# AnthonyMadia/lodestar

Hardware: AMD Instinct MI355X
Metric: verified signature sets/sec (node) at 8192-set batches (higher is better)
Workload: dtype u32 (28-bit-limb Montgomery Fp, v_mad_u64_u32)

## Files before the change

### lodestar_amd/csrc/bgv_api.cpp

```cpp
#include <hip/hip_runtime.h>
#include <stdio.h>
#include <stdlib.h>
#include <string.h>
#include <sys/mman.h>
#include <sys/random.h>

#include <algorithm>
#include <atomic>
#include <chrono>
#include <condition_variable>
#include <unordered_map>
#include <deque>
#include <map>
#include <memory>
#include <mutex>
#include <shared_mutex>
#include <unordered_set>
#include <thread>
#include <vector>

#include "../../include/blsgpu.h"
#include "bgv_launch.h"
#include "bgv_retry_plan.h"
#include "bls_field.h"
#include "bgv_shuffle.h"

#define BGV_MAX_BATCH_SLOTS 131072
#define BGV_DISPATCHERS 2

static size_t max_batch_slots() {
  static const size_t v = env_size("BGV_MAX_BATCH_SLOTS", BGV_MAX_BATCH_SLOTS, BGV_WAVE);
  return v;
}
#define BGV_COALESCE_US 500
static size_t coalesce_us() {
  static const size_t v = env_size("BGV_COALESCE_US", BGV_COALESCE_US, 0);
  return v;
}
#define BGV_IDLE_COALESCE_US 50
static size_t idle_coalesce_us() {
  static const size_t v = env_size("BGV_IDLE_COALESCE_US", BGV_IDLE_COALESCE_US, 0);
  return v;
}
#define BGV_SPLIT_MIN_SETS 4096
static size_t split_min_env() {
  static const size_t v = env_size("BGV_SPLIT_MIN", BGV_SPLIT_MIN_SETS, 0);
  return v == 1 ? 2 : v;
}
static int dispatchers_per_device() {
  static const int v = (int)env_size("BGV_DISPATCHERS", BGV_DISPATCHERS, 1);
  return v;
}
static int execs_per_device() {
  static const int v = (int)env_size("BGV_EXECS", 2 * BGV_DISPATCHERS, 1);
  return std::max(v, dispatchers_per_device());
}

static size_t retry_hold_max() {
  static const size_t v = env_size("BGV_RETRY_HOLD", 1, 1);
  return v;
}
static int retry_threads_per_device() {
  static const int v = (int)env_size("BGV_RETRY_THREADS", 1, 1);
  return v;
}

extern "C" int bgv_device_count(void) {
  int n = 0;
  if (hipGetDeviceCount(&n) != hipSuccess) return 0;
  return n;
}

namespace {

template <class T>
struct Pinned {
  T* p = nullptr;
  size_t cap = 0;
  hipError_t reserve(size_t n) {
    if (n <= cap) return hipSuccess;
    release();
    n = std::max(n, 2 * cap);
    hipError_t e = hipHostMalloc(reinterpret_cast<void**>(&p), std::max<size_t>(n, 1) * sizeof(T), 0);
    if (e != hipSuccess) {
      p = nullptr;
      return e;
    }
    cap = n;
    return hipSuccess;
  }
  void release() {
    if (p) (void)hipHostFree(p);
    p = nullptr;
    cap = 0;
  }
};

struct Exec {
  hipStream_t main = nullptr;
  hipStream_t close = nullptr;
  hipEvent_t ev0 = nullptr, ev1 = nullptr, ev_prep = nullptr, ev_sets = nullptr;
  hipEvent_t kev[2 * BGV_NKERNELS] = {};
  void* slot_mem = nullptr;
  uint32_t slot_cap = 0;
  void* group_mem = nullptr;
  uint32_t group_cap = 0;
  bgv_dslot* d_slots = nullptr;
  bgv_dgroup* d_groups = nullptr;
  uint32_t* d_idx = nullptr;
  size_t idx_cap = 0;
  uint8_t* d_pkb = nullptr;
  size_t pkb_cap = 0;
  Pinned<bgv_dslot> h_slots;
  Pinned<bgv_dgroup> h_groups;
  Pinned<uint32_t> h_idx;
  Pinned<uint8_t> h_pkb;
  Pinned<int32_t> h_ss, h_ps, h_verdict;
  fp12_t* d_gu1 = nullptr;
  size_t gu1_cap = 0;
  void* d_pscratch = nullptr;
  size_t pscratch_cap = 0;
  uint8_t* d_pout = nullptr;
  size_t pout_cap = 0;
  uint32_t* d_lines = nullptr;
  uint32_t lines_cap = 0;
};

struct FinalScratch {
  uint8_t* din = nullptr;
  void* vals = nullptr;
  void* one = nullptr;
  bgv_dgroup* dg = nullptr;
  int32_t* dst = nullptr;
  int32_t* dv = nullptr;
  size_t cap = 0;
};

static const uint32_t kComHandles = 2 * BGV_MAX_COMMITTEES;
static const size_t kComPoolInit = size_t(1) << 20;
struct ComPool {
  std::mutex mu;
  std::vector<uint32_t> free_handles;
  std::map<uint32_t, uint32_t> free_ranges;
  size_t cap = 0;
  bool alloc(uint32_t n, uint32_t* handle, uint32_t* off) {
    if (free_handles.empty()) return false;
    for (auto it = free_ranges.begin(); it != free_ranges.end(); ++it)
      if (it->second >= n) {
        *off = it->first;
        const uint32_t rest = it->second - n;
        free_ranges.erase(it);
        if (rest) free_ranges.emplace(*off + n, rest);
        *handle = free_handles.back();
        free_handles.pop_back();
        return true;
      }
    return false;
  }
  bool alloc_bulk(uint32_t n, uint32_t nh, std::vector<uint32_t>* handles, uint32_t* off) {
    if (free_handles.size() < nh) return false;
    for (auto it = free_ranges.begin(); it != free_ranges.end(); ++it)
      if (it->second >= n) {
        *off = it->first;
        const uint32_t rest = it->second - n;
        free_ranges.erase(it);
        if (rest) free_ranges.emplace(*off + n, rest);
        handles->assign(free_handles.end() - nh, free_handles.end());
        free_handles.resize(free_handles.size() - nh);
        return true;
      }
    return false;
  }
  void add_range(uint32_t off, uint32_t n) {
    auto nx = free_ranges.lower_bound(off);
    if (nx != free_ranges.begin()) {
      auto pv = std::prev(nx);
      if (pv->first + pv->second == off) {
        off = pv->first;
        n += pv->second;
        free_ranges.erase(pv);
      }
    }
    if (nx != free_ranges.end() && off + n == nx->first) {
      n += nx->second;
      free_ranges.erase(nx);
    }
    free_ranges.emplace(off, n);
  }
};
struct CommitteeRec {
  uint32_t handle = 0, off = 0;
  std::vector<uint32_t> idx;
  bool bad = false;
  std::shared_ptr<ComPool> pool;
  ~CommitteeRec() {
    if (!pool) return;
    std::lock_guard<std::mutex> lk(pool->mu);
    pool->free_handles.push_back(handle);
    pool->add_range(off, (uint32_t)idx.size());
  }
};

struct Call;
struct BatchState {
  std::chrono::steady_clock::time_point tb;
  double t_merge = 0, t_tok = 0, t_sets = 0, t_pass1 = 0, t_post = 0;
  uint32_t nslots = 0, ngroups = 0;
  std::vector<uint32_t> call_gb;
  bool want_gu = false;
  bool uniform = false;
  bool prof = false;
};
struct RetryJob {
  std::vector<Call*> calls;
  Exec* x = nullptr;
  std::shared_ptr<BatchState> st;
};
struct DevSched {
  std::mutex mu;
  std::condition_variable cv;
  std::deque<Exec*> free;
  std::deque<RetryJob> rq;
  bool stop = false;
  std::vector<std::thread> retry_threads;
  std::vector<hipStream_t> retries;
  std::vector<hipStream_t> dstreams;
};

struct Device {
  int id = 0;
  std::unique_ptr<DevSched> sched = std::make_unique<DevSched>();
  FinalScratch final_scratch;
  hipStream_t stream = nullptr;
  bgv_cache_entry* cache = nullptr;
  size_t cache_cap = 0;
  bgv_dcommittee* com_dir = nullptr;
  uint32_t* com_pool = nullptr;
  uint32_t* com_list = nullptr;
  uint32_t* shuf_buf = nullptr;
  size_t shuf_cap = 0;
  std::vector<Exec*> execs;
  std::unique_ptr<std::mutex> compute_mu = std::make_unique<std::mutex>();
};

struct Call : CallPlan {
  const bgv_set* sets = nullptr;
  const bgv_pkbits* pkbits = nullptr;
  std::vector<SetCommittee> setcom;
  std::vector<std::shared_ptr<CommitteeRec>> com_refs;
  int32_t* out = nullptr;
  bgv_stats* stats_out = nullptr;
  bgv_done_fn done = nullptr;
  void* user = nullptr;
  bool owned = false;
  std::chrono::steady_clock::time_point t0;
  int dev = -1;
  bgv_job pjob{};
  int32_t pcode = 0;
  int rc = BGV_OK;
  std::mutex mu;
  std::condition_variable cv;
  bool finished = false;
};

}

struct bgv_ctx {
  std::vector<Device> devs;
  std::atomic<size_t> n_pubkeys{0};
  std::mutex put_mu;
  std::unordered_set<uint32_t> bad_pk;
  std::atomic<bool> closed{false};
  std::mutex rng_mu;
  uint64_t rng_seed = 0, rng_state = 0;
  std::shared_mutex cache_mu;
  std::mutex util_mu;
  std::shared_mutex com_mu;
  std::unordered_map<uint32_t, std::shared_ptr<CommitteeRec>> committees;
  std::vector<std::weak_ptr<CommitteeRec>> retired;
  std::shared_ptr<ComPool> com_pool = std::make_shared<ComPool>();
  std::mutex prof_mu;
  bool profile = false;
  bool fault_inject = false;
  std::atomic<uint32_t> max_slots{BGV_MAX_BATCH_SLOTS};
  std::atomic<uint32_t> coalesce{BGV_COALESCE_US};
  std::atomic<uint32_t> idle_coalesce{BGV_IDLE_COALESCE_US};
  std::atomic<int> running{0};
  std::atomic<uint32_t> split_min{BGV_SPLIT_MIN_SETS};
  int split_inflight = 0;
  bool split_closing = false;
  std::mutex split_mu;
  std::condition_variable split_cv;
  double kernel_ms[BGV_NKERNELS] = {};
  uint64_t kernel_launches = 0;
  std::vector<std::thread> dispatchers;
  std::mutex qmu;
  std::condition_variable qcv;
  std::deque<Call*> queue;
  bool stop = false;
};

#define HIPCHK(x)                               \
  do {                                          \
    hipError_t e_ = (x);                        \
    if (e_ != hipSuccess) return -BGV_E_DEVICE; \
  } while (0)

static uint64_t splitmix64(uint64_t* s) {
  uint64_t z = (*s += 0x9E3779B97F4A7C15ull);
  z = (z ^ (z >> 30)) * 0xBF58476D1CE4E5B9ull;
  z = (z ^ (z >> 27)) * 0x94D049BB133111EBull;
  return z ^ (z >> 31);
}

static void fill_scalars(bgv_ctx* c, uint64_t* out, size_t n) {
  {
    std::lock_guard<std::mutex> lk(c->rng_mu);
    if (c->rng_seed) {
      for (size_t i = 0; i < n; ++i) {
        uint64_t v;
        do v = splitmix64(&c->rng_state);
        while (v == 0);
        out[i] = v;
      }
      return;
    }
  }
  par_ranges(n, [out](size_t lo, size_t hi) {
    size_t got = 0;
    uint8_t* p = reinterpret_cast<uint8_t*>(out + lo);
    while (got < (hi - lo) * 8) {
      const ssize_t r = getrandom(p + got, (hi - lo) * 8 - got, 0);
      if (r > 0) got += (size_t)r;
    }
    for (size_t i = lo; i < hi; ++i)
      if (out[i] == 0) out[i] = 1;
  });
}

template <class T>
static int grow(T** p, size_t* cap, size_t want) {
  if (want <= *cap) return BGV_OK;
  size_t n = std::max(want, *cap * 2);
  if (*p) (void)hipFree(*p);
  *p = nullptr;
  HIPCHK(hipMalloc(reinterpret_cast<void**>(p), n * sizeof(T)));
  *cap = n;
  return BGV_OK;
}

static int exec_reserve_slots(Exec& x, uint32_t slots) {
  if (slots <= x.slot_cap) return BGV_OK;
  uint32_t n = std::max<uint32_t>(slots, x.slot_cap * 2);
  if (x.slot_mem) (void)hipFree(x.slot_mem);
  if (x.d_slots) (void)hipFree(x.d_slots);
  x.slot_mem = nullptr;
  x.d_slots = nullptr;
  HIPCHK(hipMalloc(&x.slot_mem, bgv_slot_mem_bytes(n)));
  HIPCHK(hipMalloc(reinterpret_cast<void**>(&x.d_slots), sizeof(bgv_dslot) * n));
  x.slot_cap = n;
  return BGV_OK;
}

static int exec_reserve_groups(Exec& x, uint32_t groups) {
  if (groups <= x.group_cap) return BGV_OK;
  uint32_t n = std::max<uint32_t>(groups, x.group_cap * 2);
  if (x.group_mem) (void)hipFree(x.group_mem);
  if (x.d_groups) (void)hipFree(x.d_groups);
  x.group_mem = nullptr;
  x.d_groups = nullptr;
  HIPCHK(hipMalloc(&x.group_mem, bgv_group_bytes() * n));
  HIPCHK(hipMalloc(reinterpret_cast<void**>(&x.d_groups), sizeof(bgv_dgroup) * n));
  x.group_cap = n;
  return BGV_OK;
}

static uint32_t lines_keep_pairs(size_t slots) {
  return (uint32_t)((slots + slots / BGV_WAVE + 16383u) & ~(size_t)16383u);
}
static void exec_trim_lines(Exec& x, size_t max_slots) {
  if (x.lines_cap <= lines_keep_pairs(max_slots)) return;
  (void)hipFree(x.d_lines);
  x.d_lines = nullptr;
  x.lines_cap = 0;
}
static int exec_reserve_lines(Exec& x, bgv_dev_batch& b) {
  const uint32_t need = bgv_lines_pairs(b);
  if (need > x.lines_cap) {
    const uint32_t cap = (need + 16383u) & ~16383u;
    if (x.d_lines) (void)hipFree(x.d_lines);
    x.d_lines = nullptr;
    x.lines_cap = 0;
    HIPCHK(hipMalloc(reinterpret_cast<void**>(&x.d_lines), bgv_line_record_bytes() * cap));
    x.lines_cap = cap;
  }
  b.lines = x.d_lines;
  b.lines_cap = x.lines_cap;
  return BGV_OK;
}

static int exec_create(Exec* x) {
  HIPCHK(hipEventCreate(&x->ev0));
  HIPCHK(hipEventCreate(&x->ev1));
  HIPCHK(hipEventCreateWithFlags(&x->ev_sets, hipEventDisableTiming));
  HIPCHK(hipEventCreateWithFlags(&x->ev_prep, hipEventDisableTiming));
  for (auto& e : x->kev) HIPCHK(hipEventCreate(&e));
  return BGV_OK;
}

static void exec_destroy(Exec* x) {
  if (x->main) (void)hipStreamSynchronize(x->main);
  void* ptrs[] = {x->slot_mem, x->group_mem, x->d_slots,    x->d_groups, x->d_idx,
                  x->d_pkb,      x->d_pscratch, x->d_pout, x->d_lines};
  for (void* p : ptrs)
    if (p) (void)hipFree(p);
  x->h_slots.release();
  x->h_groups.release();
  x->h_idx.release();
  x->h_pkb.release();
  x->h_ss.release();
  x->h_ps.release();
  x->h_verdict.release();
  if (x->d_gu1) (void)hipFree(x->d_gu1);
  if (x->ev0) (void)hipEventDestroy(x->ev0);
  if (x->ev1) (void)hipEventDestroy(x->ev1);
  if (x->ev_sets) (void)hipEventDestroy(x->ev_sets);
  if (x->ev_prep) (void)hipEventDestroy(x->ev_prep);
  for (auto& e : x->kev)
    if (e) (void)hipEventDestroy(e);
  if (x->close) (void)hipStreamSynchronize(x->close);
  delete x;
}

static void prof_add(bgv_ctx* c, Exec& x, bool sets, bool groups) {
  std::lock_guard<std::mutex> lk(c->prof_mu);
  if (!c->profile) return;
  for (int k = 0; k < BGV_NKERNELS; ++k) {
    const bool is_set_kernel = k < BGV_NSETKERNELS;
    if ((is_set_kernel && !sets) || (!is_set_kernel && !groups)) continue;
    float km = 0;
    if (hipEventElapsedTime(&km, x.kev[2 * k], x.kev[2 * k + 1]) == hipSuccess) c->kernel_ms[k] += km;
  }
  if (sets) c->kernel_launches++;
}

static bgv_dev_batch make_batch(Device& d, Exec& x, uint32_t nslots, uint32_t ngroups) {
  bgv_dev_batch b;
  memset(&b, 0, sizeof(b));
  b.nslots = nslots;
  b.ngroups = ngroups;
  b.slots = x.d_slots;
  b.groups = x.d_groups;
  b.pk_idx = x.d_idx;
  b.cache_opaque = d.cache;
  b.pk_bytes = x.d_pkb;
  b.com_dir = d.com_dir;
  b.com_pool = d.com_pool;
  bgv_carve(&b, x.slot_mem, x.slot_cap, x.group_mem, x.group_cap);
  return b;
}

static void call_finish(Call* call) {
  for (size_t j = 0; j < call->njobs; ++j) call->out[j] = call->code[j] == 2 ? -BGV_E_DEVICE : call->code[j];
  call->st.wall_ms =
      std::chrono::duration<double, std::milli>(std::chrono::steady_clock::now() - call->t0).count();
  if (call->stats_out) *call->stats_out = call->st;
  if (call->done) call->done(call->user, call->rc);
  if (call->owned) {
    delete call;
    return;
  }
  {
    std::lock_guard<std::mutex> lk(call->mu);
    call->finished = true;
  }
  call->cv.notify_all();
}

static void call_fail(Call* call, int rc) {
  call->rc = rc;
  for (auto& x : call->code)
    if (x == 2) x = -BGV_E_DEVICE;
  call_finish(call);
}

static int host_job_code(bgv_ctx* c, const bgv_job& jb, const bgv_set* sets, int32_t* code,
                         const bgv_pkbits* pkbits = nullptr, Call* call = nullptr) {
  *code = 2;
  if (jb.n_sets == 0) {
    *code = -BGV_E_EMPTY_SET;
    return BGV_OK;
  }
  for (uint32_t k = 0; k < jb.n_sets && *code == 2; ++k) {
    const bgv_set& s = sets[jb.first_set + k];
    if (pkbits && pkbits[jb.first_set + k].committee != BGV_NO_COMMITTEE) {
      const bgv_pkbits& pb = pkbits[jb.first_set + k];
      if (!s.msg || (!s.sig && s.sig_len) || (!pb.bits && pb.n_bits)) return -BGV_E_ARG;
      const auto it = c->committees.find(pb.committee);
      const CommitteeRec* rec = it != c->committees.end() ? it->second.get() : nullptr;
      CommitteeInfo ci{};
      if (rec) ci = CommitteeInfo{rec->handle, (uint32_t)rec->idx.size(), rec->bad};
      SetCommittee sc;
      *code = committee_set_check(rec ? &ci : nullptr, pb, &sc);
      if (*code == 2 && call) {
        call->setcom[jb.first_set + k] = sc;
        if (call->com_refs.empty() || call->com_refs.back().get() != rec) call->com_refs.push_back(it->second);
      }
      continue;
    }
    if (s.n_pk == 0)
      *code = -BGV_E_EMPTY_AGGREGATE;
    else if (!s.msg || (!s.sig && s.sig_len) || (!s.pk_indices && !s.pk_bytes))
      return -BGV_E_ARG;
    else if (s.pk_indices)
      for (uint32_t q = 0; q < s.n_pk; ++q)
        if (s.pk_indices[q] >= c->n_pubkeys || (!c->bad_pk.empty() && c->bad_pk.count(s.pk_indices[q]))) {
          *code = -BGV_E_BAD_INDEX;
          break;
        }
  }
  return BGV_OK;
}

static void advise_huge(void* p, size_t bytes) {
  const uintptr_t a = ((uintptr_t)p + (2u << 20) - 1) & ~(uintptr_t)((2u << 20) - 1);
  const uintptr_t e = ((uintptr_t)p + bytes) & ~(uintptr_t)((2u << 20) - 1);
  if (e > a) (void)madvise(reinterpret_cast<void*>(a), e - a, MADV_HUGEPAGE);
}

static int call_submit(bgv_ctx* c, Call* call, const bgv_job* jobs, size_t njobs, const bgv_set* sets, size_t nsets,
                       int mode, int32_t* out, bgv_stats* stats, bgv_done_fn done, void* user, int dev = -1,
                       const bgv_pkbits* pkbits = nullptr) {
  call->t0 = std::chrono::steady_clock::now();
  call->dev = dev;
  if (c->closed) return -BGV_E_CLOSED;
  if ((njobs && (!jobs || !out)) || (nsets && !sets)) return -BGV_E_ARG;
  if (mode != BGV_MODE_WORKER && mode != BGV_MODE_PER_JOB) return -BGV_E_ARG;
  call->jobs = jobs;
  call->njobs = njobs;
  call->sets = sets;
  call->nsets = nsets;
  call->mode = mode;
  call->out = out;
  call->stats_out = stats;
  call->done = done;
  call->user = user;
  call->code.assign(njobs, 2);
  call->pkbits = pkbits;
  if (pkbits) call->setcom.assign(nsets, SetCommittee{});
  {
    std::shared_lock<std::shared_mutex> clk(c->cache_mu);
    std::shared_lock<std::shared_mutex> mlk(c->com_mu, std::defer_lock);
    if (pkbits) mlk.lock();
    for (size_t j = 0; j < njobs; ++j) {
      if ((size_t)jobs[j].first_set + jobs[j].n_sets > nsets) return -BGV_E_ARG;
      if (host_job_code(c, jobs[j], sets, &call->code[j], pkbits, call) != BGV_OK) return -BGV_E_ARG;
    }
  }
  const auto is_com = [pkbits](size_t i) { return pkbits && pkbits[i].committee != BGV_NO_COMMITTEE; };
  Layout& L = call->L;
  {
    size_t npk = 0;
    for (size_t i = 0; i < nsets; ++i)
      if (is_com(i))
        npk += 1 + pkb_nwords(call->setcom[i].n);
      else if (sets[i].pk_indices)
        npk += sets[i].n_pk;
    const size_t cap = nsets + nsets / 8 + BGV_WAVE;
    L.slots.reserve(cap);
    L.slot_set.reserve(cap);
    L.idx.reserve(npk);
    if (nsets >= (1u << 17)) {
      advise_huge(L.slots.data(), sizeof(bgv_dslot) * cap);
      advise_huge(L.slot_set.data(), 4 * cap);
      advise_huge(L.idx.data(), 4 * npk);
    }
  }
  layout_call(L, call->todo, jobs, njobs, sets, mode, call->code, pkbits ? call->setcom.data() : nullptr);
  call->set_sig.assign(nsets, 0);
  call->set_pk.assign(nsets, 0);
  if (L.slots.empty()) {
    call_finish(call);
    return BGV_OK;
  }
  {
    std::lock_guard<std::mutex> lk(c->qmu);
    if (c->stop) return -BGV_E_CLOSED;
    c->queue.push_back(call);
  }
  if (dev < 0)
    c->qcv.notify_one();
  else
    c->qcv.notify_all();
  return BGV_OK;
}

static double ms_since(std::chrono::steady_clock::time_point t) {
  return std::chrono::duration<double, std::milli>(std::chrono::steady_clock::now() - t).count();
}

static bool needs_retry(const std::vector<Call*>& calls) {
  for (const Call* call : calls)
    if (!call->units.empty()) return true;
  return false;
}

static int run_pass1(bgv_ctx* c, Device& d, Exec& x, std::vector<Call*>& calls, BatchState& bs) {
  const auto tb = std::chrono::steady_clock::now();
  bs.tb = tb;
  double t_merge = 0, t_tok = 0, t_sets = 0, t_pass1 = 0, t_post = 0;
  uint32_t nslots = 0, ngroups = 0;
  size_t nidx = 0, npkb = 0, nuniq = 0, ncom_team = 0, ncom_wave = 0;
  bool any_uniform = false;
  for (Call* call : calls) {
    call->slot_base = nslots;
    nslots += (uint32_t)call->L.slots.size();
    ngroups += (uint32_t)call->L.groups.size();
    nidx += call->L.idx.size();
    npkb += call->L.pkb.size();
    nuniq += call->L.uniq.size();
    ncom_team += call->L.com_team.size();
    ncom_wave += call->L.com_wave.size();
    for (char u : call->L.group_uniform) any_uniform = any_uniform || u;
  }
  const size_t ncom = ncom_team + ncom_wave, nlist = nuniq + ncom;
  const bool bulk = nslots + ngroups > bgv_fold_pairs_max();
  const bool uniform = uniform_enabled() && any_uniform && bulk && !bgv_single_pass_miller();
  HIPCHK(hipSetDevice(d.id));
  int rc;
  if ((rc = exec_reserve_slots(x, nslots)) || (rc = exec_reserve_groups(x, ngroups)) ||
      (rc = grow(&x.d_idx, &x.idx_cap, std::max<size_t>(nidx + nlist, 1))) ||
      (rc = grow(&x.d_pkb, &x.pkb_cap, std::max<size_t>(npkb, 1))))
    return rc;
  HIPCHK(x.h_slots.reserve(nslots));
  HIPCHK(x.h_groups.reserve(std::max<size_t>(ngroups, 1)));
  HIPCHK(x.h_idx.reserve(nidx + nlist));
  HIPCHK(x.h_pkb.reserve(npkb));
  HIPCHK(x.h_ss.reserve(nslots));
  HIPCHK(x.h_ps.reserve(nslots));
  HIPCHK(x.h_verdict.reserve(std::max<size_t>(ngroups, 1)));
  bgv_dslot* slots = x.h_slots.p;
  bgv_dgroup* groups = x.h_groups.p;
  uint32_t max_npk = 0;
  {
    size_t ns = 0, ng = 0, ni = 0, npb = 0;
    for (Call* call : calls) {
      const uint32_t ib = (uint32_t)ni, pb = (uint32_t)(npb / 96), gb = (uint32_t)ng;
      if (ns == 0 && ib == 0 && pb == 0 && gb == 0) {
        const bgv_dslot* src = call->L.slots.data();
        std::atomic<uint32_t> mx{0};
        par_ranges(call->L.slots.size(), [&](size_t lo, size_t hi) {
          memcpy(slots + lo, src + lo, sizeof(bgv_dslot) * (hi - lo));
          uint32_t m = 0;
          for (size_t i = lo; i < hi; ++i)
            if (!(src[i].flags & BGV_SLOT_PK_COMMITTEE)) m = std::max(m, src[i].n_pk);
          uint32_t cur = mx.load();
          while (m > cur && !mx.compare_exchange_weak(cur, m)) {
          }
        });
        max_npk = std::max(max_npk, mx.load());
        ns = call->L.slots.size();
      } else {
        for (const bgv_dslot& s0 : call->L.slots) {
          const bgv_dslot s = rebase_slot(s0, call->slot_base, ib, pb, gb);
          if (!(s.flags & BGV_SLOT_PK_COMMITTEE)) max_npk = std::max(max_npk, s.n_pk);
          slots[ns++] = s;
        }
      }
      for (size_t gi = 0; gi < call->L.groups.size(); ++gi) {
        const bgv_dgroup& g = call->L.groups[gi];
        groups[ng++] = bgv_dgroup{g.first_slot + call->slot_base, g.n_slots, g.mask, 0,
                                  uniform && call->L.group_uniform[gi] ? BGV_GROUP_UNIFORM : 0u};
      }
      if (!call->L.idx.empty()) memcpy(x.h_idx.p + ni, call->L.idx.data(), 4 * call->L.idx.size());
      ni += call->L.idx.size();
      if (!call->L.pkb.empty()) memcpy(x.h_pkb.p + npb, call->L.pkb.data(), call->L.pkb.size());
      npb += call->L.pkb.size();
    }
    uint32_t* u = x.h_idx.p + nidx;
    for (Call* call : calls)
      for (uint32_t v : call->L.uniq) *u++ = v + call->slot_base;
    for (Call* call : calls)
      for (uint32_t v : call->L.com_team) *u++ = v + call->slot_base;
    for (Call* call : calls)
      for (uint32_t v : call->L.com_wave) *u++ = v + call->slot_base;
  }
  std::vector<uint64_t> sc(nslots);
  fill_scalars(c, sc.data(), nslots);
  par_ranges(nslots, [&](size_t lo, size_t hi) {
    for (size_t i = lo; i < hi; ++i) slots[i].scalar = sc[i];
  });

  bool prof;
  {
    std::lock_guard<std::mutex> lk(c->prof_mu);
    prof = c->profile;
  }
  t_merge = ms_since(tb);
  if (c->fault_inject) HIPCHK(hipErrorLaunchFailure);
  HIPCHK(hipMemcpyAsync(x.d_slots, slots, sizeof(bgv_dslot) * nslots, hipMemcpyHostToDevice, x.main));
  HIPCHK(hipMemcpyAsync(x.d_groups, groups, sizeof(bgv_dgroup) * ngroups, hipMemcpyHostToDevice, x.main));
  if (nidx + nlist) HIPCHK(hipMemcpyAsync(x.d_idx, x.h_idx.p, 4 * (nidx + nlist), hipMemcpyHostToDevice, x.main));
  if (npkb) HIPCHK(hipMemcpyAsync(x.d_pkb, x.h_pkb.p, npkb, hipMemcpyHostToDevice, x.main));
  bgv_dev_batch b = make_batch(d, x, nslots, ngroups);
  b.max_npk = max_npk;
  b.uniform = uniform;
  bs.uniform = uniform;
  b.uniq = x.d_idx + nidx;
  b.nuniq = (uint32_t)nuniq;
  b.com = x.d_idx + nidx + nuniq;
  b.ncom_team = (uint32_t)ncom_team;
  b.ncom_wave = (uint32_t)ncom_wave;
  if (int lrc = exec_reserve_lines(x, b)) return lrc;
  bgv_streams S{x.main, prof ? x.kev : nullptr};
  int32_t *ss = x.h_ss.p, *ps = x.h_ps.p, *verdict = x.h_verdict.p;
  {
    const auto tt = std::chrono::steady_clock::now();
    std::unique_lock<std::mutex> tok(*d.compute_mu);
    t_tok = ms_since(tt);
    HIPCHK(hipEventRecord(x.ev0, x.main));
    HIPCHK(bgv_launch_prep(b, S));
    HIPCHK(hipEventRecord(x.ev_prep, x.main));
    HIPCHK(bgv_launch_miller(b, S));
    HIPCHK(hipEventRecord(x.ev_sets, x.main));
    HIPCHK(hipEventSynchronize(x.ev_prep));
    t_sets = ms_since(tt) - t_tok;
  }
  const auto tg = std::chrono::steady_clock::now();
  HIPCHK(bgv_launch_groups(b, S, false));
  HIPCHK(hipEventRecord(x.ev1, x.main));
  HIPCHK(hipMemcpyAsync(ss, b.sig_status, 4ull * nslots, hipMemcpyDeviceToHost, x.main));
  HIPCHK(hipMemcpyAsync(ps, b.pk_status, 4ull * nslots, hipMemcpyDeviceToHost, x.main));
  HIPCHK(hipMemcpyAsync(verdict, b.verdict, 4ull * ngroups, hipMemcpyDeviceToHost, x.main));
  HIPCHK(hipStreamSynchronize(x.main));
  float ms = 0;
  HIPCHK(hipEventElapsedTime(&ms, x.ev0, x.ev1));
  exec_trim_lines(x, c->max_slots.load());
  if (prof) prof_add(c, x, true, true);
  t_pass1 = ms_since(tg);
  const auto tp = std::chrono::steady_clock::now();
  std::vector<uint32_t>& call_gb = bs.call_gb;
  bool& want_gu = bs.want_gu;
  {
    uint32_t gb = 0;
    for (Call* call : calls) {
      call->st.device_ms += ms;
      call->after_pass1(ss + call->slot_base, ps + call->slot_base, verdict + gb);
      call_gb.push_back(gb);
      gb += (uint32_t)call->L.groups.size();
      want_gu = want_gu || call->any_pattern_eligible();
    }
  }
  if (want_gu) {
    if ((rc = grow(&x.d_gu1, &x.gu1_cap, ngroups))) return rc;
    HIPCHK(hipMemcpyAsync(x.d_gu1, b.gu, sizeof(fp12_t) * ngroups, hipMemcpyDeviceToDevice, x.main));
  }
  {
    uint32_t gb = 0, np = 0, maxg = 0;
    for (Call* call : calls) {
      if (call->partial_out) {
        ++np;
        maxg = std::max<uint32_t>(maxg, (uint32_t)call->L.groups.size());
      }
    }
    if (np) {
      if ((rc = grow(reinterpret_cast<uint8_t**>(&x.d_pscratch), &x.pscratch_cap,
                     bgv_fp12_bytes() * (maxg / 32 + 4))) ||
          (rc = grow(&x.d_pout, &x.pout_cap, 576)))
        return rc;
      for (Call* call : calls) {
        const uint32_t ng = (uint32_t)call->L.groups.size();
        if (call->partial_out) {
          HIPCHK(bgv_launch_partial(b, gb, ng, x.d_pscratch, x.d_pout, x.main));
          HIPCHK(hipMemcpyAsync(call->partial_out, x.d_pout, 576, hipMemcpyDeviceToHost, x.main));
          HIPCHK(hipStreamSynchronize(x.main));
        }
        gb += ng;
      }
    }
  }
  HIPCHK(hipStreamSynchronize(x.main));
  t_post = ms_since(tp);
  bs.t_merge = t_merge;
  bs.t_tok = t_tok;
  bs.t_sets = t_sets;
  bs.t_pass1 = t_pass1;
  bs.t_post = t_post;
  bs.nslots = nslots;
  bs.ngroups = ngroups;
  bs.prof = prof;
  if (trace_on() && !needs_retry(calls))
    fprintf(stderr,
            "[bgv] dev %d calls %zu slots %u groups %u | submit..dispatch %.1f | merge %.1f tokwait %.1f sets %.1f "
            "groups %.1f post %.1f total %.1f ms\n",
            d.id, calls.size(), nslots, ngroups,
            std::chrono::duration<double, std::milli>(tb - calls.front()->t0).count(), t_merge, t_tok, t_sets,
            t_pass1, t_post, ms_since(tb));
  return BGV_OK;
}

struct RetryRun {
  RetryJob job;
  int rounds = 0;
  uint32_t nrg = 0;
  double t_build = 0;
  std::chrono::steady_clock::time_point tr;
};

static int retry_launch(Device& d, RetryRun& r, bool* more) {
  Exec& x = *r.job.x;
  std::vector<Call*>& calls = r.job.calls;
  BatchState& bs = *r.job.st;
  const auto th = std::chrono::steady_clock::now();
  std::vector<bgv_dgroup> rg;
  for (size_t k = 0; k < calls.size(); ++k)
    calls[k]->build_parts(rg, bs.want_gu ? (int64_t)bs.call_gb[k] : -1, bs.uniform);
  *more = !rg.empty();
  r.nrg = 0;
  if (rg.empty()) return BGV_OK;
  ++r.rounds;
  const uint32_t nrg = (uint32_t)rg.size();
  std::vector<uint32_t> upk;
  if (bs.uniform)
    for (uint32_t t = 0; t < nrg; ++t)
      if (rg[t].flags & BGV_GROUP_UNIFORM) upk.push_back(t);
  const uint32_t per = (uint32_t)(sizeof(bgv_dgroup) / sizeof(uint32_t));
  const uint32_t nlist = ((uint32_t)upk.size() + per - 1) / per;
  int rc;
  if ((rc = exec_reserve_groups(x, nrg + nlist))) return rc;
  HIPCHK(x.h_groups.reserve(nrg + nlist));
  HIPCHK(x.h_verdict.reserve(nrg));
  memcpy(x.h_groups.p, rg.data(), sizeof(bgv_dgroup) * nrg);
  if (!upk.empty()) memcpy(x.h_groups.p + nrg, upk.data(), 4 * upk.size());
  HIPCHK(hipMemcpyAsync(x.d_groups, x.h_groups.p, sizeof(bgv_dgroup) * (nrg + nlist), hipMemcpyHostToDevice,
                        x.close));
  bgv_dev_batch b = make_batch(d, x, bs.nslots, nrg);
  b.uniform = !upk.empty();
  b.upk = reinterpret_cast<const uint32_t*>(b.groups + nrg);
  b.npk = (uint32_t)upk.size();
  for (const bgv_dgroup& t : rg) b.weighted = b.weighted || (t.flags & BGV_GROUP_WEIGHTED);
  bool pattern = false;
  for (Call* call : calls) pattern = pattern || !call->punits.empty();
  if (pattern) b.gu1 = x.d_gu1;
  r.t_build = ms_since(th);
  bgv_streams SC{x.close, bs.prof ? x.kev : nullptr};
  HIPCHK(hipEventRecord(x.ev0, x.close));
  HIPCHK(bgv_launch_groups(b, SC, true));
  HIPCHK(hipEventRecord(x.ev1, x.close));
  HIPCHK(hipMemcpyAsync(x.h_verdict.p, b.verdict, 4ull * nrg, hipMemcpyDeviceToHost, x.close));
  r.nrg = nrg;
  return BGV_OK;
}

static int retry_complete(bgv_ctx* c, RetryRun& r, double t_wait) {
  Exec& x = *r.job.x;
  float ms = 0;
  HIPCHK(hipEventElapsedTime(&ms, x.ev0, x.ev1));
  if (r.job.st->prof) prof_add(c, x, false, true);
  if (trace_on()) {
    size_t npt = 0;
    for (Call* call : r.job.calls)
      for (const PatternUnit& pu : call->punits) npt += pu.tests.size();
    fprintf(stderr,
            "[bgv]  round %d: %u groups (%zu tests with a reference), host %.2f, launch..verdicts %.2f, device %.2f ms, "
            "since round start %.1f ms\n",
            r.rounds, r.nrg, npt, r.t_build, t_wait, ms, ms_since(r.tr));
  }
  for (Call* call : r.job.calls) {
    call->st.device_ms += ms;
    call->after_round(x.h_verdict.p);
  }
  r.nrg = 0;
  return BGV_OK;
}

static void retry_trace_done(const Device& d, const RetryRun& r) {
  if (!trace_on()) return;
  const BatchState& bs = *r.job.st;
  fprintf(stderr,
          "[bgv] dev %d calls %zu slots %u groups %u | merge %.1f tokwait %.1f sets %.1f groups %.1f post %.1f "
          "retry(%d) %.1f total %.1f ms\n",
          d.id, r.job.calls.size(), bs.nslots, bs.ngroups, bs.t_merge, bs.t_tok, bs.t_sets, bs.t_pass1, bs.t_post,
          r.rounds, ms_since(r.tr), ms_since(bs.tb));
}

static Exec* exec_acquire(Device& d) {
  DevSched& s = *d.sched;
  std::unique_lock<std::mutex> lk(s.mu);
  s.cv.wait(lk, [&s] { return !s.free.empty(); });
  Exec* x = s.free.back();
  s.free.pop_back();
  return x;
}

static void exec_release(Device& d, Exec* x) {
  DevSched& s = *d.sched;
  {
    std::lock_guard<std::mutex> lk(s.mu);
    s.free.push_back(x);
  }
  s.cv.notify_all();
}

static void finish_calls(std::vector<Call*>& calls, int rc) {
  for (Call* call : calls) {
    if (rc != BGV_OK)
      call_fail(call, rc);
    else
      call_finish(call);
  }
}

static void retry_loop(bgv_ctx* c, Device* d, int k) {
  DevSched& s = *d->sched;
  (void)hipSetDevice(d->id);
  hipStream_t st = s.retries[k];
  std::vector<RetryRun> held;
  auto leave = [&](size_t i, int rc) {
    finish_calls(held[i].job.calls, rc);
    exec_release(*d, held[i].job.x);
    c->running.fetch_sub(1);
    held.erase(held.begin() + (std::ptrdiff_t)i);
  };
  for (;;) {
    {
      std::unique_lock<std::mutex> lk(s.mu);
      if (held.empty()) s.cv.wait(lk, [&s] { return s.stop || !s.rq.empty(); });
      if (held.empty() && s.rq.empty()) return;
      while (!s.rq.empty() && held.size() < retry_hold_max()) {
        RetryRun r;
        r.job = std::move(s.rq.front());
        s.rq.pop_front();
        r.job.x->close = st;
        r.tr = std::chrono::steady_clock::now();
        c->running.fetch_add(1);
        held.push_back(std::move(r));
      }
    }
    (void)hipSetDevice(d->id);
    for (size_t i = 0; i < held.size();) {
      bool more = false;
      const int rc = retry_launch(*d, held[i], &more);
      if (rc != BGV_OK) {
        (void)hipStreamSynchronize(st);
        leave(i, rc);
      } else if (!more) {
        retry_trace_done(*d, held[i]);
        leave(i, BGV_OK);
      } else {
        ++i;
      }
    }
    if (held.empty()) continue;
    const auto tl = std::chrono::steady_clock::now();
    const hipError_t e = hipStreamSynchronize(st);
    const double t_wait = ms_since(tl);
    for (size_t i = 0; i < held.size();) {
      const int rc = e == hipSuccess ? retry_complete(c, held[i], t_wait) : -BGV_E_DEVICE;
      if (rc != BGV_OK)
        leave(i, rc);
      else
        ++i;
    }
  }
}

static void dispatcher_loop(bgv_ctx* c, Device* d, hipStream_t stream) {
  (void)hipSetDevice(d->id);
  const int di = (int)(d - c->devs.data());
  auto mine = [di](const Call* q) { return q->dev < 0 || q->dev == di; };
  auto any_mine = [c, &mine] {
    for (Call* q : c->queue)
      if (mine(q)) return true;
    return false;
  };
  for (;;) {
    std::vector<Call*> calls;
    {
      std::unique_lock<std::mutex> lk(c->qmu);
      c->qcv.wait(lk, [c, &any_mine] { return c->stop || any_mine(); });
      if (!any_mine()) return;
      auto queued_slots = [c, &mine] {
        size_t n = 0;
        for (Call* q : c->queue)
          if (mine(q)) n += q->L.slots.size();
        return n;
      };
      const size_t cap = c->max_slots.load();
      const size_t win = c->running.load() > 0 ? c->coalesce.load()
                                               : std::min<size_t>(c->coalesce.load(), c->idle_coalesce.load());
      const auto until = std::chrono::steady_clock::now() + std::chrono::microseconds(win);
      while (!c->stop && queued_slots() < cap &&
             c->qcv.wait_until(lk, until) != std::cv_status::timeout) {
      }
      if (!any_mine()) continue;
      size_t slots = 0;
      for (auto it = c->queue.begin(); it != c->queue.end();) {
        Call* call = *it;
        if (!mine(call)) {
          ++it;
          continue;
        }
        const size_t n = call->L.slots.size();
        if (!calls.empty() && slots + n > cap) break;
        calls.push_back(call);
        slots += n;
        it = c->queue.erase(it);
      }
      if (!c->queue.empty()) c->qcv.notify_all();
    }
    Exec* x = exec_acquire(*d);
    x->main = stream;
    auto bs = std::make_shared<BatchState>();
    int rc;
    {
      std::shared_lock<std::shared_mutex> clk(c->cache_mu);
      c->running.fetch_add(1);
      rc = run_pass1(c, *d, *x, calls, *bs);
      c->running.fetch_sub(1);
    }
    if (rc == BGV_OK && needs_retry(calls)) {
      DevSched& s = *d->sched;
      {
        std::lock_guard<std::mutex> lk(s.mu);
        s.rq.push_back(RetryJob{std::move(calls), x, bs});
      }
      s.cv.notify_all();
      continue;
    }
    finish_calls(calls, rc);
    exec_release(*d, x);
  }
}

extern "C" {

static void ctx_free_devices(bgv_ctx* c) {
  for (Device& d : c->devs) {
    if (!d.stream) continue;
    (void)hipSetDevice(d.id);
    for (Exec* x : d.execs) exec_destroy(x);
    d.execs.clear();
    d.sched->free.clear();
    for (hipStream_t st : d.sched->dstreams) (void)hipStreamDestroy(st);
    d.sched->dstreams.clear();
    for (hipStream_t st : d.sched->retries) (void)hipStreamDestroy(st);
    d.sched->retries.clear();
    if (d.stream) (void)hipStreamSynchronize(d.stream);
    if (d.cache) (void)hipFree(d.cache);
    d.cache = nullptr;
    {
      void* cbufs[] = {d.com_dir, d.com_pool, d.com_list, d.shuf_buf};
      for (void* q : cbufs)
        if (q) (void)hipFree(q);
      d.shuf_buf = nullptr;
      d.shuf_cap = 0;
      d.com_dir = nullptr;
      d.com_pool = nullptr;
      d.com_list = nullptr;
    }
    {
      FinalScratch& fs = d.final_scratch;
      void* bufs[] = {fs.din, fs.vals, fs.one, fs.dg, fs.dst, fs.dv};
      for (void* q : bufs)
        if (q) (void)hipFree(q);
      fs = FinalScratch{};
    }
    if (d.stream) (void)hipStreamDestroy(d.stream);
    d.stream = nullptr;
  }
}

int bgv_init(const int* devices, int ndev, bgv_ctx** out) {
  if (!out) return -BGV_E_ARG;
  *out = nullptr;
  int avail = bgv_device_count();
  if (avail <= 0) return -BGV_E_DEVICE;
  bgv_ctx* c = new bgv_ctx();
  {
    const char* fi = getenv("BGV_FAULT_INJECT");
    c->fault_inject = fi && atoi(fi) > 0;
  }
  c->max_slots = (uint32_t)max_batch_slots();
  c->coalesce = (uint32_t)coalesce_us();
  c->idle_coalesce = (uint32_t)idle_coalesce_us();
  c->split_min = (uint32_t)split_min_env();
  const int n = (devices && ndev > 0) ? ndev : 1;
  c->devs.resize(n);
  for (int i = 0; i < n; ++i) {
    Device& d = c->devs[i];
    d.id = (devices && ndev > 0) ? devices[i] : 0;
    bool ok = d.id >= 0 && d.id < avail && hipSetDevice(d.id) == hipSuccess &&
              hipStreamCreateWithFlags(&d.stream, hipStreamNonBlocking) == hipSuccess;
    int least = 0, greatest = 0;
    ok = ok && hipDeviceGetStreamPriorityRange(&least, &greatest) == hipSuccess;
    for (int k = 0; ok && k < retry_threads_per_device(); ++k) {
      hipStream_t st = nullptr;
      ok = hipStreamCreateWithPriority(&st, hipStreamNonBlocking, greatest) == hipSuccess;
      if (ok) d.sched->retries.push_back(st);
    }
    for (int k = 0; ok && k < dispatchers_per_device(); ++k) {
      hipStream_t st = nullptr;
      ok = hipStreamCreateWithFlags(&st, hipStreamNonBlocking) == hipSuccess;
      if (ok) d.sched->dstreams.push_back(st);
    }
    ok = ok && hipMalloc(reinterpret_cast<void**>(&d.com_dir), sizeof(bgv_dcommittee) * kComHandles) == hipSuccess &&
         hipMalloc(reinterpret_cast<void**>(&d.com_pool), 4 * kComPoolInit) == hipSuccess &&
         hipMalloc(reinterpret_cast<void**>(&d.com_list), 4 * (size_t)kComHandles) == hipSuccess;
    for (int k = 0; ok && k < execs_per_device(); ++k) {
      Exec* x = new Exec();
      d.execs.push_back(x);
      ok = exec_create(x) == BGV_OK;
      if (ok) d.sched->free.push_back(x);
    }
    if (!ok) {
      ctx_free_devices(c);
      delete c;
      (void)hipGetLastError();
      return d.id < 0 || d.id >= avail ? -BGV_E_ARG : -BGV_E_DEVICE;
    }
  }
  c->com_pool->cap = kComPoolInit;
  c->com_pool->free_ranges.emplace(0u, (uint32_t)kComPoolInit);
  for (uint32_t h = kComHandles; h-- > 0;) c->com_pool->free_handles.push_back(h);
  for (Device& d : c->devs) {
    for (hipStream_t st : d.sched->dstreams) c->dispatchers.emplace_back(dispatcher_loop, c, &d, st);
    for (int k = 0; k < (int)d.sched->retries.size(); ++k) d.sched->retry_threads.emplace_back(retry_loop, c, &d, k);
  }
  *out = c;
  return BGV_OK;
}

int bgv_close(bgv_ctx* c) {
  if (!c) return -BGV_E_ARG;
  {
    std::unique_lock<std::mutex> lk(c->split_mu);
    c->split_closing = true;
    c->split_cv.wait(lk, [c] { return c->split_inflight == 0; });
  }
  {
    std::lock_guard<std::mutex> lk(c->qmu);
    c->stop = true;
  }
  c->qcv.notify_all();
  for (auto& w : c->dispatchers)
    if (w.joinable()) w.join();
  c->dispatchers.clear();
  for (Device& d : c->devs) {
    {
      std::lock_guard<std::mutex> lk(d.sched->mu);
      d.sched->stop = true;
    }
    d.sched->cv.notify_all();
    for (auto& t : d.sched->retry_threads)
      if (t.joinable()) t.join();
    d.sched->retry_threads.clear();
  }
  std::unique_lock<std::shared_mutex> lk(c->cache_mu);
  if (c->closed.exchange(true)) return BGV_OK;
  ctx_free_devices(c);
  return BGV_OK;
}

int bgv_destroy(bgv_ctx* c) {
  if (!c) return -BGV_E_ARG;
  bgv_close(c);
  delete c;
  return BGV_OK;
}

int bgv_set_batching(bgv_ctx* c, uint32_t max_batch_slots, uint32_t coalesce_us, uint32_t idle_coalesce_us) {
  if (!c) return -BGV_E_ARG;
  if (max_batch_slots) c->max_slots = std::max<uint32_t>(max_batch_slots, BGV_WAVE);
  if (coalesce_us != UINT32_MAX) c->coalesce = coalesce_us;
  if (idle_coalesce_us != UINT32_MAX) c->idle_coalesce = idle_coalesce_us;
  return BGV_OK;
}

int bgv_set_rng_seed(bgv_ctx* c, uint64_t seed) {
  if (!c) return -BGV_E_ARG;
  std::lock_guard<std::mutex> lk(c->rng_mu);
  c->rng_seed = seed;
  c->rng_state = seed;
  return BGV_OK;
}

size_t bgv_pubkeys_count(const bgv_ctx* c) { return c ? c->n_pubkeys.load() : 0; }

static int cache_reserve(bgv_ctx* c, size_t need) {
  const size_t esz = bgv_cache_entry_bytes();
  for (Device& d : c->devs) {
    HIPCHK(hipSetDevice(d.id));
    if (need <= d.cache_cap) continue;
    size_t cap = std::max(need, d.cache_cap * 2);
    void* p = nullptr;
    HIPCHK(hipMalloc(&p, esz * cap));
    if (d.cache) {
      HIPCHK(hipMemcpyAsync(p, d.cache, esz * c->n_pubkeys, hipMemcpyDeviceToDevice, d.stream));
      HIPCHK(hipStreamSynchronize(d.stream));
      HIPCHK(hipFree(d.cache));
    }
    d.cache = static_cast<bgv_cache_entry*>(p);
    d.cache_cap = cap;
  }
  return BGV_OK;
}

static int committee_totals(bgv_ctx* c, const std::vector<uint32_t>& handles) {
  if (handles.empty()) return BGV_OK;
  for (Device& d : c->devs) {
    HIPCHK(hipSetDevice(d.id));
    HIPCHK(hipMemcpyAsync(d.com_list, handles.data(), 4 * handles.size(), hipMemcpyHostToDevice, d.stream));
    HIPCHK(bgv_launch_committee_totals(d.com_dir, d.com_list, (uint32_t)handles.size(), d.com_pool, d.cache, d.stream));
    HIPCHK(hipStreamSynchronize(d.stream));
  }
  return BGV_OK;
}

static int committees_refresh(bgv_ctx* c, uint32_t first, size_t n) {
  std::vector<uint32_t> handles;
  {
    std::unique_lock<std::shared_mutex> lk(c->com_mu);
    std::vector<std::shared_ptr<CommitteeRec>> recs;
    for (auto& kv : c->committees) recs.push_back(kv.second);
    for (auto& w : c->retired)
      if (auto sp = w.lock()) recs.push_back(std::move(sp));
    for (auto& sp : recs) {
      CommitteeRec& r = *sp;
      bool touched = false, bad = false;
      for (uint32_t i : r.idx) {
        touched = touched || (i >= first && (size_t)i < (size_t)first + n);
        bad = bad || (!c->bad_pk.empty() && c->bad_pk.count(i));
      }
      if (!touched) continue;
      r.bad = bad;
      handles.push_back(r.handle);
    }
  }
  return committee_totals(c, handles);
}

static int com_pool_grow(bgv_ctx* c, size_t need) {
  ComPool& P = *c->com_pool;
  const size_t old = P.cap, cap = std::max(2 * old, old + need);
  if (cap > (size_t)UINT32_MAX) return -BGV_E_NOMEM;
  for (Device& d : c->devs) {
    HIPCHK(hipSetDevice(d.id));
    uint32_t* p = nullptr;
    HIPCHK(hipMalloc(reinterpret_cast<void**>(&p), 4 * cap));
    HIPCHK(hipMemcpyAsync(p, d.com_pool, 4 * old, hipMemcpyDeviceToDevice, d.stream));
    HIPCHK(hipStreamSynchronize(d.stream));
    HIPCHK(hipFree(d.com_pool));
    d.com_pool = p;
  }
  std::lock_guard<std::mutex> lk(P.mu);
  P.add_range((uint32_t)old, (uint32_t)(cap - old));
  P.cap = cap;
  return BGV_OK;
}

int bgv_committee_put(bgv_ctx* c, uint32_t id, const uint32_t* indices, size_t n) {
  if (!c || id >= BGV_MAX_COMMITTEES || !indices || n < 1 || n > 65536) return -BGV_E_ARG;
  std::lock_guard<std::mutex> plk(c->put_mu);
  auto rec = std::make_shared<CommitteeRec>();
  auto checks = [&]() -> int {
    if (c->closed) return -BGV_E_CLOSED;
    {
      std::shared_lock<std::shared_mutex> lk(c->com_mu);
      if (c->committees.count(id)) return -BGV_E_ARG;
    }
    for (size_t i = 0; i < n; ++i)
      if (indices[i] >= c->n_pubkeys || (!c->bad_pk.empty() && c->bad_pk.count(indices[i]))) return -BGV_E_BAD_INDEX;
    return BGV_OK;
  };
  auto take = [&]() -> bool {
    std::lock_guard<std::mutex> lk(c->com_pool->mu);
    if (!c->com_pool->alloc((uint32_t)n, &rec->handle, &rec->off)) return false;
    rec->pool = c->com_pool;
    return true;
  };
  auto upload = [&]() -> int {
    rec->idx.assign(indices, indices + n);
    const bgv_dcommittee head{rec->off, (uint32_t)n, {}};
    std::lock_guard<std::mutex> ulk(c->util_mu);
    for (Device& d : c->devs) {
      HIPCHK(hipSetDevice(d.id));
      HIPCHK(hipMemcpyAsync(d.com_pool + rec->off, indices, 4 * n, hipMemcpyHostToDevice, d.stream));
      HIPCHK(hipMemcpyAsync(d.com_dir + rec->handle, &head, sizeof(head), hipMemcpyHostToDevice, d.stream));
      HIPCHK(hipStreamSynchronize(d.stream));
    }
    const int rc = committee_totals(c, {rec->handle});
    if (rc) return rc;
    std::unique_lock<std::shared_mutex> lk(c->com_mu);
    c->committees.emplace(id, rec);
    return BGV_OK;
  };
  {
    std::shared_lock<std::shared_mutex> clk(c->cache_mu);
    if (int rc = checks()) return rc;
    if (take()) return upload();
    std::lock_guard<std::mutex> lk(c->com_pool->mu);
    if (c->com_pool->free_handles.empty()) return -BGV_E_NOMEM;
  }
  std::unique_lock<std::shared_mutex> clk(c->cache_mu);
  if (int rc = checks()) return rc;
  {
    std::lock_guard<std::mutex> ulk(c->util_mu);
    if (int rc = com_pool_grow(c, n)) return rc;
  }
  if (!take()) return -BGV_E_NOMEM;
  return upload();
}

int bgv_committee_drop(bgv_ctx* c, uint32_t id) {
  if (!c) return -BGV_E_ARG;
  std::lock_guard<std::mutex> plk(c->put_mu);
  if (c->closed) return -BGV_E_CLOSED;
  std::shared_ptr<CommitteeRec> rec;
  std::unique_lock<std::shared_mutex> lk(c->com_mu);
  auto it = c->committees.find(id);
  if (it == c->committees.end()) return -BGV_E_BAD_INDEX;
  rec = std::move(it->second);
  c->committees.erase(it);
  c->retired.erase(std::remove_if(c->retired.begin(), c->retired.end(),
                                  [](const std::weak_ptr<CommitteeRec>& w) { return w.expired(); }),
                   c->retired.end());
  c->retired.push_back(rec);
  return BGV_OK;
}

int bgv_shuffling_put(bgv_ctx* c, uint32_t first_id, const uint8_t seed[32], const uint32_t* active, size_t n_active,
                      uint32_t slots, uint32_t committees_per_slot, uint32_t rounds, uint32_t* out_shuffling) {
  if (!c || !seed || !active || n_active < 1 || n_active > BGV_SHUFFLE_MAX_N || !slots || !committees_per_slot ||
      rounds > BGV_SHUFFLE_MAX_ROUNDS)
    return -BGV_E_ARG;
  const uint64_t count64 = (uint64_t)slots * committees_per_slot;
  if (first_id > BGV_MAX_COMMITTEES || count64 > BGV_MAX_COMMITTEES - first_id) return -BGV_E_ARG;
  const uint32_t n = (uint32_t)n_active, count = (uint32_t)count64, m = shuf_nonempty(n, count);
  if (shuf_longest(n, count) > 65536) return -BGV_E_ARG;
  std::lock_guard<std::mutex> plk(c->put_mu);
  std::vector<std::shared_ptr<CommitteeRec>> recs;
  std::vector<uint32_t> ks, handles;
  uint32_t base = 0;
  auto checks = [&]() -> int {
    if (c->closed) return -BGV_E_CLOSED;
    {
      std::shared_lock<std::shared_mutex> lk(c->com_mu);
      for (uint32_t k = 0; k < count; ++k)
        if (c->committees.count(first_id + k)) return -BGV_E_ARG;
    }
    const size_t npk = c->n_pubkeys;
    const bool marks = !c->bad_pk.empty();
    for (size_t i = 0; i < n; ++i)
      if (active[i] >= npk || (marks && c->bad_pk.count(active[i]))) return -BGV_E_BAD_INDEX;
    return BGV_OK;
  };
  auto take = [&]() -> bool {
    std::lock_guard<std::mutex> lk(c->com_pool->mu);
    if (!c->com_pool->alloc_bulk(n, m, &handles, &base)) return false;
    for (uint32_t j = 0; j < m; ++j) {
      uint32_t lo, hi;
      ks.push_back(shuf_nonempty_k(n, count, j, &lo, &hi));
      auto rec = std::make_shared<CommitteeRec>();
      rec->handle = handles[j];
      rec->off = base + lo;
      rec->idx.resize(hi - lo);
      rec->pool = c->com_pool;
      recs.push_back(std::move(rec));
    }
    return true;
  };
  auto run = [&]() -> int {
    std::vector<uint32_t> shuf(n);
    {
      std::lock_guard<std::mutex> ulk(c->util_mu);
      const size_t words = bgv_shuffle_scratch_words(n, rounds);
      bool first = true;
      for (Device& d : c->devs) {
        HIPCHK(hipSetDevice(d.id));
        if (d.shuf_cap < words) {
          uint32_t* p = nullptr;
          HIPCHK(hipMalloc(reinterpret_cast<void**>(&p), 4 * words));
          if (d.shuf_buf) (void)hipFree(d.shuf_buf);
          d.shuf_buf = p;
          d.shuf_cap = words;
        }
        HIPCHK(hipMemcpyAsync(d.shuf_buf, active, 4 * (size_t)n, hipMemcpyHostToDevice, d.stream));
        HIPCHK(hipMemcpyAsync(d.com_list, handles.data(), 4 * (size_t)m, hipMemcpyHostToDevice, d.stream));
        HIPCHK(bgv_launch_shuffle(seed, n, rounds, d.shuf_buf, d.com_pool + base, d.stream));
        HIPCHK(bgv_launch_shuffle_dir(d.com_dir, d.com_list, m, base, n, count, d.stream));
        HIPCHK(bgv_launch_committee_totals(d.com_dir, d.com_list, m, d.com_pool, d.cache, d.stream));
        if (first)
          HIPCHK(hipMemcpyAsync(shuf.data(), d.com_pool + base, 4 * (size_t)n, hipMemcpyDeviceToHost, d.stream));
        first = false;
        HIPCHK(hipStreamSynchronize(d.stream));
      }
    }
    for (uint32_t j = 0; j < m; ++j) {
      CommitteeRec& r = *recs[j];
      std::copy_n(shuf.begin() + (r.off - base), r.idx.size(), r.idx.begin());
    }
    if (out_shuffling) memcpy(out_shuffling, shuf.data(), 4 * (size_t)n);
    std::unique_lock<std::shared_mutex> lk(c->com_mu);
    for (uint32_t j = 0; j < m; ++j) c->committees.emplace(first_id + ks[j], recs[j]);
    return BGV_OK;
  };
  {
    std::shared_lock<std::shared_mutex> clk(c->cache_mu);
    if (int rc = checks()) return rc;
    if (take()) return run();
    std::lock_guard<std::mutex> lk(c->com_pool->mu);
    if (c->com_pool->free_handles.size() < m) return -BGV_E_NOMEM;
  }
  std::unique_lock<std::shared_mutex> clk(c->cache_mu);
  if (int rc = checks()) return rc;
  {
    std::lock_guard<std::mutex> ulk(c->util_mu);
    if (int rc = com_pool_grow(c, n)) return rc;
  }
  if (!take()) return -BGV_E_NOMEM;
  return run();
}

int bgv_committee_drop_range(bgv_ctx* c, uint32_t first_id, uint32_t count) {
  if (!c || first_id > BGV_MAX_COMMITTEES || count > BGV_MAX_COMMITTEES - first_id) return -BGV_E_ARG;
  std::lock_guard<std::mutex> plk(c->put_mu);
  if (c->closed) return -BGV_E_CLOSED;
  std::vector<std::shared_ptr<CommitteeRec>> recs;
  std::unique_lock<std::shared_mutex> lk(c->com_mu);
  c->retired.erase(std::remove_if(c->retired.begin(), c->retired.end(),
                                  [](const std::weak_ptr<CommitteeRec>& w) { return w.expired(); }),
                   c->retired.end());
  for (uint32_t id = first_id; id < first_id + count; ++id) {
    auto it = c->committees.find(id);
    if (it == c->committees.end()) continue;
    c->retired.push_back(it->second);
    recs.push_back(std::move(it->second));
    c->committees.erase(it);
  }
  return (int)recs.size();
}

int bgv_pubkeys_put(bgv_ctx* c, uint32_t first, const uint8_t* keys, size_t n, int fmt) {
  if (!c || (n && !keys) || (fmt != BGV_PK_COMPRESSED && fmt != BGV_PK_UNCOMPRESSED)) return -BGV_E_ARG;
  std::lock_guard<std::mutex> plk(c->put_mu);
  const size_t esz = bgv_cache_entry_bytes();
  std::vector<void*> staged(c->devs.size(), nullptr);
  std::vector<int32_t> status(n, 0);
  auto free_staged = [&] {
    for (size_t di = 0; di < staged.size(); ++di)
      if (staged[di]) {
        (void)hipSetDevice(c->devs[di].id);
        (void)hipFree(staged[di]);
      }
  };
  {
    std::shared_lock<std::shared_mutex> clk(c->cache_mu);
    if (c->closed) return -BGV_E_CLOSED;
    if ((size_t)first > c->n_pubkeys) return -BGV_E_ARG;
    if (n == 0) return BGV_OK;
    std::lock_guard<std::mutex> ulk(c->util_mu);
    for (size_t di = 0; di < c->devs.size(); ++di) {
      Device& d = c->devs[di];
      if (hipSetDevice(d.id) != hipSuccess || hipMalloc(&staged[di], esz * n) != hipSuccess ||
          hipMemsetAsync(staged[di], 0, esz * n, d.stream) != hipSuccess) {
        free_staged();
        return -BGV_E_DEVICE;
      }
      const size_t chunk = 1 << 20;
      uint8_t* dk = nullptr;
      int32_t* dst = nullptr;
      int rc = BGV_OK;
      if (hipMalloc(reinterpret_cast<void**>(&dk), (size_t)fmt * std::min(n, chunk) + 1) != hipSuccess ||
          hipMalloc(reinterpret_cast<void**>(&dst), 4 * std::min(n, chunk) + 4) != hipSuccess)
        rc = -BGV_E_DEVICE;
      for (size_t off = 0; rc == BGV_OK && off < n; off += chunk) {
        const size_t m = std::min(chunk, n - off);
        bgv_cache_entry* out =
            reinterpret_cast<bgv_cache_entry*>(static_cast<uint8_t*>(staged[di]) + esz * off);
        if (hipMemcpyAsync(dk, keys + (size_t)fmt * off, (size_t)fmt * m, hipMemcpyHostToDevice, d.stream) !=
                hipSuccess ||
            bgv_launch_cache_put(dk, (uint32_t)m, fmt, out, dst, d.stream) != hipSuccess ||
            (di == 0 && hipMemcpyAsync(status.data() + off, dst, 4 * m, hipMemcpyDeviceToHost, d.stream) !=
                            hipSuccess) ||
            hipStreamSynchronize(d.stream) != hipSuccess)
          rc = -BGV_E_DEVICE;
      }
      if (dk) (void)hipFree(dk);
      if (dst) (void)hipFree(dst);
      if (rc) {
        free_staged();
        return rc;
      }
    }
  }
  int first_err = BGV_OK;
  std::vector<uint32_t> bad;
  for (size_t i = 0; i < n; ++i)
    if (status[i]) {
      if (first_err == BGV_OK) first_err = status[i];
      bad.push_back(first + (uint32_t)i);
    }
  const size_t need = (size_t)first + n;
  auto copy_in = [&]() -> int {
    for (size_t di = 0; di < c->devs.size(); ++di) {
      Device& d = c->devs[di];
      HIPCHK(hipSetDevice(d.id));
      HIPCHK(hipMemcpyAsync(reinterpret_cast<uint8_t*>(d.cache) + esz * first, staged[di], esz * n,
                            hipMemcpyDeviceToDevice, d.stream));
      HIPCHK(hipStreamSynchronize(d.stream));
    }
    return BGV_OK;
  };
  int rc = BGV_OK;
  bool done = false;
  {
    std::shared_lock<std::shared_mutex> clk(c->cache_mu);
    if (c->closed) {
      rc = -BGV_E_CLOSED;
      done = true;
    } else if (first == c->n_pubkeys && bad.empty()) {
      bool fits = true;
      for (const Device& d : c->devs) fits = fits && need <= d.cache_cap;
      if (fits) {
        std::lock_guard<std::mutex> ulk(c->util_mu);
        rc = copy_in();
        if (rc == BGV_OK) c->n_pubkeys.store(need);
        done = true;
      }
    }
  }
  if (!done) {
    std::unique_lock<std::shared_mutex> clk(c->cache_mu);
    if (c->closed) {
      rc = -BGV_E_CLOSED;
    } else {
      std::lock_guard<std::mutex> ulk(c->util_mu);
      rc = cache_reserve(c, need);
      const uint32_t old_n = (uint32_t)c->n_pubkeys.load();
      for (size_t di = 0; rc == BGV_OK && di < c->devs.size(); ++di) {
        Device& d = c->devs[di];
        if (hipSetDevice(d.id) != hipSuccess) rc = -BGV_E_DEVICE;
        for (uint32_t i : bad)
          if (rc == BGV_OK && i < old_n &&
              hipMemcpyAsync(static_cast<uint8_t*>(staged[di]) + esz * (i - first),
                             reinterpret_cast<const uint8_t*>(d.cache) + esz * i, esz, hipMemcpyDeviceToDevice,
                             d.stream) != hipSuccess)
            rc = -BGV_E_DEVICE;
      }
      if (rc == BGV_OK) rc = copy_in();
      if (rc == BGV_OK) {
        for (uint32_t i = first; i < need; ++i) c->bad_pk.erase(i);
        for (uint32_t i : bad) c->bad_pk.insert(i);
        c->n_pubkeys.store(std::max(c->n_pubkeys.load(), need));
        if (first < old_n) rc = committees_refresh(c, first, n);
      }
    }
  }
  free_staged();
  if (rc) return rc;
  return first_err ? -first_err : BGV_OK;
}

static void fp12_one_bytes(uint8_t out[576]) {
  memset(out, 0, 576);
  out[47] = 1;
}

static int partial_submit(bgv_ctx* c, Call* call, const bgv_set* sets, size_t nsets, uint8_t* out576,
                          int32_t* out_codes, int dev, const bgv_pkbits* pkbits = nullptr) {
  out_codes[0] = out_codes[1] = 0;
  fp12_one_bytes(out576);
  call->partial_out = out576;
  call->partial_codes = out_codes;
  call->pjob = bgv_job{0, (uint32_t)nsets, 0};
  return call_submit(c, call, &call->pjob, 1, sets, nsets, BGV_MODE_PER_JOB, &call->pcode, nullptr, nullptr, nullptr,
                     dev, pkbits);
}

static int call_wait(Call* call) {
  std::unique_lock<std::mutex> lk(call->mu);
  call->cv.wait(lk, [call] { return call->finished; });
  return call->rc;
}

static int partial_finish(Call* call, int rc, int32_t* out_codes) {
  if (rc == BGV_OK) rc = call_wait(call);
  if (rc == BGV_OK && call->pcode < 0 && call->pcode != -BGV_E_DEVICE) out_codes[0] = call->pcode;
  return rc;
}

static size_t split_min_sets(const bgv_ctx* c) {
  return c->split_min.load();
}

static void stats_add(bgv_stats* a, const bgv_stats& b) {
  a->batch_retries += b.batch_retries;
  a->batch_sigs_success += b.batch_sigs_success;
  a->device_groups += b.device_groups;
  a->sets_verified += b.sets_verified;
  a->device_ms = std::max(a->device_ms, b.device_ms);
}

static bool split_wanted(const bgv_ctx* c, size_t nsets) {
  return c->devs.size() > 1 && split_min_sets(c) > 0 && nsets >= split_min_sets(c);
}

static bool split_enter(bgv_ctx* c) {
  std::lock_guard<std::mutex> lk(c->split_mu);
  if (c->split_closing) return false;
  ++c->split_inflight;
  return true;
}

static void split_leave(bgv_ctx* c) {
  std::lock_guard<std::mutex> lk(c->split_mu);
  --c->split_inflight;
  c->split_cv.notify_all();
}

static int verify_split(bgv_ctx* c, const bgv_job* jobs, size_t njobs, const bgv_set* sets, size_t nsets,
                        const bgv_pkbits* pkbits, int mode, int32_t* out, bgv_stats* stats) {
  const auto t0 = std::chrono::steady_clock::now();
  const size_t K = c->devs.size(), big = split_min_sets(c);
  struct Shard {
    Call call;
    size_t job;
    uint8_t part[576];
    int32_t codes[2] = {0, 0};
    int rc = BGV_OK;
  };
  struct Child {
    Call call;
    std::vector<bgv_job> jobs;
    std::vector<int32_t> out;
    bgv_stats st{};
    size_t j0 = 0;
    int rc = BGV_OK;
  };
  std::vector<std::unique_ptr<Shard>> shards;
  std::vector<std::unique_ptr<Child>> kids;
  std::vector<size_t> small;
  size_t small_sets = 0;
  std::vector<int32_t> pre(njobs, 2);
  {
    std::shared_lock<std::shared_mutex> clk(c->cache_mu);
    std::shared_lock<std::shared_mutex> mlk(c->com_mu, std::defer_lock);
    if (pkbits) mlk.lock();
    for (size_t j = 0; j < njobs; ++j) {
      if ((size_t)jobs[j].first_set + jobs[j].n_sets > nsets) return -BGV_E_ARG;
      if (jobs[j].n_sets >= big && host_job_code(c, jobs[j], sets, &pre[j], pkbits) != BGV_OK) return -BGV_E_ARG;
    }
  }
  for (size_t j = 0; j < njobs; ++j) {
    if (jobs[j].n_sets >= big) continue;
    small.push_back(j);
    small_sets += jobs[j].n_sets;
  }
  int rc = BGV_OK;
  {
    size_t i = 0, acc = 0;
    for (size_t d = 0; d < K && i < small.size(); ++d) {
      const size_t target = (small_sets * (d + 1) + K - 1) / K;
      auto kid = std::make_unique<Child>();
      kid->j0 = i;
      while (i < small.size() && (acc < target || kid->jobs.empty())) {
        kid->jobs.push_back(jobs[small[i]]);
        acc += jobs[small[i]].n_sets;
        ++i;
      }
      if (d == K - 1)
        while (i < small.size()) {
          kid->jobs.push_back(jobs[small[i]]);
          ++i;
        }
      kid->out.assign(kid->jobs.size(), 0);
      kid->rc = call_submit(c, &kid->call, kid->jobs.data(), kid->jobs.size(), sets, nsets, mode, kid->out.data(),
                            &kid->st, nullptr, nullptr, (int)d, pkbits);
      if (kid->rc != BGV_OK && rc == BGV_OK) rc = kid->rc;
      kids.push_back(std::move(kid));
    }
  }
  for (size_t j = 0; j < njobs; ++j) {
    const uint32_t n = jobs[j].n_sets;
    if (n < big || pre[j] != 2) continue;
    for (size_t d = 0; d < K; ++d) {
      const size_t lo = n * d / K, hi = n * (d + 1) / K;
      if (hi <= lo) continue;
      auto sh = std::make_unique<Shard>();
      sh->job = j;
      sh->rc = partial_submit(c, &sh->call, sets + jobs[j].first_set + lo, hi - lo, sh->part, sh->codes, (int)d,
                              pkbits ? pkbits + jobs[j].first_set + lo : nullptr);
      if (sh->rc != BGV_OK && rc == BGV_OK) rc = sh->rc;
      shards.push_back(std::move(sh));
    }
  }
  for (auto& k : kids)
    if (k->rc == BGV_OK) {
      k->rc = call_wait(&k->call);
      if (k->rc != BGV_OK && rc == BGV_OK) rc = k->rc;
    }
  for (auto& sh : shards)
    if (sh->rc == BGV_OK) {
      sh->rc = partial_finish(&sh->call, BGV_OK, sh->codes);
      if (sh->rc != BGV_OK && rc == BGV_OK) rc = sh->rc;
    }
  if (rc != BGV_OK) return rc;
  bgv_stats st{};
  for (auto& k : kids) {
    for (size_t q = 0; q < k->jobs.size(); ++q) out[small[k->j0 + q]] = k->out[q];
    stats_add(&st, k->st);
  }
  for (size_t j = 0; j < njobs; ++j) {
    if (jobs[j].n_sets < big) continue;
    if (pre[j] != 2) {
      out[j] = pre[j];
      continue;
    }
    int32_t code = 0;
    bool decided = false;
    std::vector<uint8_t> parts;
    for (auto& sh : shards)
      if (sh->job == j && sh->codes[0] && !decided) {
        code = sh->codes[0];
        decided = true;
      }
    for (auto& sh : shards)
      if (sh->job == j && sh->codes[1] && !decided) {
        code = sh->codes[1] == 1 ? -BGV_BLST_PK_IS_INFINITY : sh->codes[1];
        decided = true;
      }
    if (!decided) {
      for (auto& sh : shards)
        if (sh->job == j) parts.insert(parts.end(), sh->part, sh->part + 576);
      int32_t v = 0;
      const int frc = bgv_final_verify(c, parts.data(), parts.size() / 576, &v);
      if (frc != BGV_OK) return frc;
      code = v ? 1 : 0;
    }
    out[j] = code;
    st.sets_verified += jobs[j].n_sets;
    st.device_groups += 1;
  }
  st.wall_ms = std::chrono::duration<double, std::milli>(std::chrono::steady_clock::now() - t0).count();
  if (stats) *stats = st;
  return BGV_OK;
}

int bgv_set_split(bgv_ctx* c, uint32_t min_sets) {
  if (!c) return -BGV_E_ARG;
  c->split_min = min_sets == 1 ? 2 : min_sets;
  return BGV_OK;
}

int bgv_verify(bgv_ctx* c, const bgv_job* jobs, size_t njobs, const bgv_set* sets, size_t nsets, int mode,
               int32_t* out, bgv_stats* stats) {
  return bgv_verify_bits(c, jobs, njobs, sets, nsets, nullptr, mode, out, stats);
}

int bgv_verify_async(bgv_ctx* c, const bgv_job* jobs, size_t njobs, const bgv_set* sets, size_t nsets, int mode,
                     int32_t* out, bgv_stats* stats, bgv_done_fn done, void* user) {
  return bgv_verify_bits_async(c, jobs, njobs, sets, nsets, nullptr, mode, out, stats, done, user);
}

int bgv_verify_bits(bgv_ctx* c, const bgv_job* jobs, size_t njobs, const bgv_set* sets, size_t nsets,
                    const bgv_pkbits* pkbits, int mode, int32_t* out, bgv_stats* stats) {
  if (!c) return -BGV_E_ARG;
  if (split_wanted(c, nsets)) {
    if (c->closed) return -BGV_E_CLOSED;
    if ((njobs && (!jobs || !out)) || (nsets && !sets)) return -BGV_E_ARG;
    if (mode != BGV_MODE_WORKER && mode != BGV_MODE_PER_JOB) return -BGV_E_ARG;
    if (!split_enter(c)) return -BGV_E_CLOSED;
    const int rc = verify_split(c, jobs, njobs, sets, nsets, pkbits, mode, out, stats);
    split_leave(c);
    return rc;
  }
  Call* call = new Call();
  int rc = call_submit(c, call, jobs, njobs, sets, nsets, mode, out, stats, nullptr, nullptr, -1, pkbits);
  if (rc == BGV_OK) {
    std::unique_lock<std::mutex> lk(call->mu);
    call->cv.wait(lk, [call] { return call->finished; });
    rc = call->rc;
  }
  delete call;
  return rc;
}

int bgv_verify_bits_async(bgv_ctx* c, const bgv_job* jobs, size_t njobs, const bgv_set* sets, size_t nsets,
                          const bgv_pkbits* pkbits, int mode, int32_t* out, bgv_stats* stats, bgv_done_fn done,
                          void* user) {
  if (!c) return -BGV_E_ARG;
  if (split_wanted(c, nsets)) {
    if (c->closed) return -BGV_E_CLOSED;
    if ((njobs && (!jobs || !out)) || (nsets && !sets)) return -BGV_E_ARG;
    if (mode != BGV_MODE_WORKER && mode != BGV_MODE_PER_JOB) return -BGV_E_ARG;
    if (!split_enter(c)) return -BGV_E_CLOSED;
    std::thread([=] {
      const int rc = verify_split(c, jobs, njobs, sets, nsets, pkbits, mode, out, stats);
      if (done) done(user, rc);
      split_leave(c);
    }).detach();
    return BGV_OK;
  }
  Call* call = new Call();
  call->owned = true;
  int rc = call_submit(c, call, jobs, njobs, sets, nsets, mode, out, stats, done, user, -1, pkbits);
  if (rc != BGV_OK) delete call;
  return rc;
}

int bgv_verify_partial(bgv_ctx* c, const bgv_set* sets, size_t nsets, uint8_t out576[576], int32_t out_codes[2]) {
  if (!c || !out576 || !out_codes || (nsets && !sets)) return -BGV_E_ARG;
  out_codes[0] = out_codes[1] = 0;
  fp12_one_bytes(out576);
  if (nsets == 0) return c->closed ? -BGV_E_CLOSED : BGV_OK;
  Call* call = new Call();
  const int rc = partial_finish(call, partial_submit(c, call, sets, nsets, out576, out_codes, -1), out_codes);
  delete call;
  return rc;
}

int bgv_final_verify(bgv_ctx* c, const uint8_t* partials, size_t n, int32_t* out_verdict) {
  if (!c || !out_verdict || (n && !partials) || n > (1u << 20)) return -BGV_E_ARG;
  std::shared_lock<std::shared_mutex> clk(c->cache_mu);
  if (c->closed) return -BGV_E_CLOSED;
  std::lock_guard<std::mutex> lk(c->util_mu);
  Device& d = c->devs[0];
  HIPCHK(hipSetDevice(d.id));
  const size_t m = std::max<size_t>(n, 1);
  std::vector<uint8_t> in(576 * m);
  if (n) memcpy(in.data(), partials, 576 * n);
  else fp12_one_bytes(in.data());
  FinalScratch& fs = d.final_scratch;
  if (m > fs.cap) {
    void* bufs[] = {fs.din, fs.vals, fs.one, fs.dg, fs.dst, fs.dv};
    for (void* q : bufs)
      if (q) (void)hipFree(q);
    fs = FinalScratch{};
    const size_t cap = std::max<size_t>(m, 8);
    HIPCHK(hipMalloc(reinterpret_cast<void**>(&fs.din), 576 * cap));
    HIPCHK(hipMalloc(&fs.vals, bgv_fp12_bytes() * cap));
    HIPCHK(hipMalloc(&fs.one, bgv_fp12_bytes()));
    HIPCHK(hipMalloc(reinterpret_cast<void**>(&fs.dg), sizeof(bgv_dgroup)));
    HIPCHK(hipMalloc(reinterpret_cast<void**>(&fs.dst), 4 * cap));
    HIPCHK(hipMalloc(reinterpret_cast<void**>(&fs.dv), 4));
    fs.cap = cap;
  }
  const bgv_dgroup g{0, (uint32_t)m, BGV_ALL_SLOTS};
  HIPCHK(hipMemcpyAsync(fs.din, in.data(), 576 * m, hipMemcpyHostToDevice, d.stream));
  HIPCHK(hipMemcpyAsync(fs.dg, &g, sizeof(g), hipMemcpyHostToDevice, d.stream));
  HIPCHK(bgv_launch_final_verify(fs.din, (uint32_t)m, fs.vals, fs.one, fs.dg, fs.dst, fs.dv, d.stream));
  std::vector<int32_t> st(m);
  int32_t v = 0;
  HIPCHK(hipMemcpyAsync(st.data(), fs.dst, 4 * m, hipMemcpyDeviceToHost, d.stream));
  HIPCHK(hipMemcpyAsync(&v, fs.dv, 4, hipMemcpyDeviceToHost, d.stream));
  HIPCHK(hipStreamSynchronize(d.stream));
  for (int32_t x : st)
    if (x) return -BGV_E_ARG;
  *out_verdict = v;
  return BGV_OK;
}

int bgv_debug_prepare(bgv_ctx* c, const bgv_set* sets, size_t nsets, int path, uint64_t seed, uint8_t* out_h192,
                      uint8_t* out_f576, int32_t* out_status) {
  if (!c || (nsets && (!sets || !out_h192 || !out_f576 || !out_status)) ||
      (path != BGV_PATH_BULK && path != BGV_PATH_LATENCY))
    return -BGV_E_ARG;
  if (nsets == 0) return BGV_OK;
  std::shared_lock<std::shared_mutex> clk(c->cache_mu);
  if (c->closed) return -BGV_E_CLOSED;
  std::vector<bgv_dslot> slots;
  std::vector<bgv_dgroup> groups;
  std::vector<uint32_t> idx;
  uint64_t state = seed;
  uint32_t max_npk = 0;
  for (size_t i = 0; i < nsets; ++i) {
    const bgv_set& st = sets[i];
    if (!st.pk_indices || st.n_pk == 0 || !st.msg || (st.sig_len && !st.sig)) return -BGV_E_ARG;
    for (uint32_t q = 0; q < st.n_pk; ++q)
      if (st.pk_indices[q] >= c->n_pubkeys || c->bad_pk.count(st.pk_indices[q])) return -BGV_E_BAD_INDEX;
    bgv_dslot s;
    memset(&s, 0, sizeof(s));
    s.flags = BGV_SLOT_PK_CACHED;
    s.n_pk = st.n_pk;
    s.sig_len = st.sig_len;
    s.pk_off = (uint32_t)idx.size();
    idx.insert(idx.end(), st.pk_indices, st.pk_indices + st.n_pk);
    memcpy(s.msg, st.msg, 32);
    if (st.sig_len == 96) memcpy(s.sig, st.sig, 96);
    s.group = (uint32_t)(i / BGV_WAVE);
    s.hsrc = (uint32_t)i;
    do s.scalar = splitmix64(&state);
    while (s.scalar == 0);
    max_npk = std::max(max_npk, st.n_pk);
    slots.push_back(s);
  }
  while (slots.size() % BGV_WAVE) {
    bgv_dslot s;
    memset(&s, 0, sizeof(s));
    s.flags = BGV_SLOT_PAD;
    s.hsrc = (uint32_t)slots.size();
    slots.push_back(s);
  }
  for (size_t g = 0; g * BGV_WAVE < nsets; ++g)
    groups.push_back(bgv_dgroup{(uint32_t)(g * BGV_WAVE), (uint32_t)std::min<size_t>(BGV_WAVE, nsets - g * BGV_WAVE),
                                BGV_ALL_SLOTS});
  const uint32_t nslots = (uint32_t)slots.size(), ngroups = (uint32_t)groups.size();
  std::lock_guard<std::mutex> lk(c->util_mu);
  Device& d = c->devs[0];
  HIPCHK(hipSetDevice(d.id));
  Exec* x = new Exec();
  uint8_t *dh = nullptr, *df = nullptr;
  int rc = exec_create(x);
  hipStream_t dstream = nullptr;
  if (!rc && hipStreamCreateWithFlags(&dstream, hipStreamNonBlocking) != hipSuccess) rc = -BGV_E_DEVICE;
  x->main = dstream;
  if (!rc) rc = exec_reserve_slots(*x, nslots);
  if (!rc) rc = exec_reserve_groups(*x, ngroups);
  if (!rc) rc = grow(&x->d_idx, &x->idx_cap, idx.size());
  if (!rc && (hipMalloc(reinterpret_cast<void**>(&dh), 192ull * nslots) != hipSuccess ||
              hipMalloc(reinterpret_cast<void**>(&df), 576ull * nslots) != hipSuccess))
    rc = -BGV_E_DEVICE;
  std::vector<int32_t> ss(nslots), ps(nslots);
  if (!rc) {
    bgv_dev_batch b = make_batch(d, *x, nslots, ngroups);
    b.max_npk = max_npk;
    b.path = path;
    rc = exec_reserve_lines(*x, b);
    bgv_streams S{x->main, nullptr};
    const bool ok = rc == BGV_OK &&
        hipMemcpyAsync(x->d_slots, slots.data(), sizeof(bgv_dslot) * nslots, hipMemcpyHostToDevice, x->main) ==
            hipSuccess &&
        hipMemcpyAsync(x->d_groups, groups.data(), sizeof(bgv_dgroup) * ngroups, hipMemcpyHostToDevice, x->main) ==
            hipSuccess &&
        hipMemcpyAsync(x->d_idx, idx.data(), 4 * idx.size(), hipMemcpyHostToDevice, x->main) == hipSuccess &&
        bgv_launch_sets(b, S) == hipSuccess && bgv_launch_debug_out(b, dh, df, x->main) == hipSuccess &&
        hipMemcpyAsync(out_h192, dh, 192 * nsets, hipMemcpyDeviceToHost, x->main) == hipSuccess &&
        hipMemcpyAsync(out_f576, df, 576 * nsets, hipMemcpyDeviceToHost, x->main) == hipSuccess &&
        hipMemcpyAsync(ss.data(), b.sig_status, 4ull * nslots, hipMemcpyDeviceToHost, x->main) == hipSuccess &&
        hipMemcpyAsync(ps.data(), b.pk_status, 4ull * nslots, hipMemcpyDeviceToHost, x->main) == hipSuccess &&
        hipStreamSynchronize(x->main) == hipSuccess;
    if (!ok) rc = -BGV_E_DEVICE;
  }
  if (dh) (void)hipFree(dh);
  if (df) (void)hipFree(df);
  exec_destroy(x);
  if (dstream) (void)hipStreamDestroy(dstream);
  if (rc) return rc;
  for (size_t i = 0; i < nsets; ++i) {
    out_status[2 * i] = ss[i];
    out_status[2 * i + 1] = ps[i];
  }
  return BGV_OK;
}

int bgv_debug_uniform(bgv_ctx* c, const bgv_set* sets, size_t nsets, uint64_t seed, const uint64_t* test_masks,
                      const uint32_t* test_weighted, size_t ntests, uint8_t* out_first576, uint8_t* out_pk576,
                      uint8_t* out_sig576) {
  if (!c || nsets < 2 || nsets > BGV_WAVE || !sets || !out_first576 || ntests > BGV_WAVE ||
      (ntests && (!test_masks || !test_weighted || !out_pk576 || !out_sig576)))
    return -BGV_E_ARG;
  std::shared_lock<std::shared_mutex> clk(c->cache_mu);
  if (c->closed) return -BGV_E_CLOSED;
  std::vector<bgv_dslot> slots;
  std::vector<uint32_t> idx;
  uint64_t state = seed;
  uint32_t max_npk = 0;
  for (size_t i = 0; i < nsets; ++i) {
    const bgv_set& st = sets[i];
    if (!st.pk_indices || st.n_pk == 0 || !st.msg || st.sig_len != 96 || !st.sig ||
        memcmp(st.msg, sets[0].msg, 32) != 0)
      return -BGV_E_ARG;
    for (uint32_t q = 0; q < st.n_pk; ++q)
      if (st.pk_indices[q] >= c->n_pubkeys || c->bad_pk.count(st.pk_indices[q])) return -BGV_E_BAD_INDEX;
    bgv_dslot s;
    memset(&s, 0, sizeof(s));
    s.flags = BGV_SLOT_PK_CACHED;
    s.n_pk = st.n_pk;
    s.sig_len = st.sig_len;
    s.pk_off = (uint32_t)idx.size();
    idx.insert(idx.end(), st.pk_indices, st.pk_indices + st.n_pk);
    memcpy(s.msg, st.msg, 32);
    memcpy(s.sig, st.sig, 96);
    s.group = 0;
    s.hsrc = 0;
    do s.scalar = splitmix64(&state);
    while (s.scalar == 0);
    max_npk = std::max(max_npk, st.n_pk);
    slots.push_back(s);
  }
  while (slots.size() % BGV_WAVE) {
    bgv_dslot s;
    memset(&s, 0, sizeof(s));
    s.flags = BGV_SLOT_PAD;
    s.hsrc = (uint32_t)slots.size();
    slots.push_back(s);
  }
  const uint32_t nslots = (uint32_t)slots.size(), nt = (uint32_t)ntests;
  const bgv_dgroup first{0u, (uint32_t)nsets, BGV_ALL_SLOTS, 0u, BGV_GROUP_UNIFORM};
  const uint32_t per = (uint32_t)(sizeof(bgv_dgroup) / sizeof(uint32_t));
  const uint32_t nlist = (nt + per - 1) / per;
  std::vector<bgv_dgroup> tg(nt + nlist);
  bool weighted = false;
  for (uint32_t t = 0; t < nt; ++t) {
    tg[t] = bgv_dgroup{0u, (uint32_t)nsets, test_masks[t], 0u,
                       BGV_GROUP_UNIFORM | (test_weighted[t] ? BGV_GROUP_WEIGHTED : 0u)};
    weighted = weighted || test_weighted[t];
    reinterpret_cast<uint32_t*>(tg.data() + nt)[t] = t;
  }
  std::lock_guard<std::mutex> lk(c->util_mu);
  Device& d = c->devs[0];
  HIPCHK(hipSetDevice(d.id));
  Exec* x = new Exec();
  uint8_t* dout = nullptr;
  int rc = exec_create(x);
  hipStream_t dstream = nullptr;
  if (!rc && hipStreamCreateWithFlags(&dstream, hipStreamNonBlocking) != hipSuccess) rc = -BGV_E_DEVICE;
  x->main = dstream;
  if (!rc) rc = exec_reserve_slots(*x, nslots);
  if (!rc) rc = exec_reserve_groups(*x, std::max<uint32_t>(1, nt + nlist));
  if (!rc) rc = grow(&x->d_idx, &x->idx_cap, idx.size());
  if (!rc && hipMalloc(reinterpret_cast<void**>(&dout), 576ull * (1 + 2 * nt)) != hipSuccess) rc = -BGV_E_DEVICE;
  if (!rc) {
    bgv_dev_batch b = make_batch(d, *x, nslots, 1);
    b.max_npk = max_npk;
    b.path = BGV_PATH_BULK;
    b.uniform = true;
    rc = exec_reserve_lines(*x, b);
    bgv_streams S{x->main, nullptr};
    bool ok = rc == BGV_OK &&
        hipMemcpyAsync(x->d_slots, slots.data(), sizeof(bgv_dslot) * nslots, hipMemcpyHostToDevice, x->main) ==
            hipSuccess &&
        hipMemcpyAsync(x->d_groups, &first, sizeof(bgv_dgroup), hipMemcpyHostToDevice, x->main) == hipSuccess &&
        hipMemcpyAsync(x->d_idx, idx.data(), 4 * idx.size(), hipMemcpyHostToDevice, x->main) == hipSuccess &&
        bgv_launch_sets(b, S) == hipSuccess &&
        bgv_launch_fp12_bytes(b.gpkp, 1, dout, x->main) == hipSuccess;
    if (ok && nt) {
      bgv_dev_batch t = make_batch(d, *x, nslots, nt);
      t.max_npk = max_npk;
      t.path = BGV_PATH_BULK;
      t.uniform = true;
      t.upk = reinterpret_cast<const uint32_t*>(t.groups + nt);
      t.npk = nt;
      t.weighted = weighted;
      ok = hipMemcpyAsync(x->d_groups, tg.data(), sizeof(bgv_dgroup) * tg.size(), hipMemcpyHostToDevice, x->main) ==
               hipSuccess &&
           bgv_launch_gpairs(t, x->main) == hipSuccess &&
           bgv_launch_fp12_bytes(t.gpkp, nt, dout + 576, x->main) == hipSuccess &&
           bgv_launch_fp12_bytes(t.gpair, nt, dout + 576ull * (1 + nt), x->main) == hipSuccess &&
           hipMemcpyAsync(out_pk576, dout + 576, 576ull * nt, hipMemcpyDeviceToHost, x->main) == hipSuccess &&
           hipMemcpyAsync(out_sig576, dout + 576ull * (1 + nt), 576ull * nt, hipMemcpyDeviceToHost, x->main) ==
               hipSuccess;
    }
    ok = ok && hipMemcpyAsync(out_first576, dout, 576, hipMemcpyDeviceToHost, x->main) == hipSuccess &&
         hipStreamSynchronize(x->main) == hipSuccess;
    if (!ok) rc = -BGV_E_DEVICE;
  }
  if (dout) (void)hipFree(dout);
  exec_destroy(x);
  if (dstream) (void)hipStreamDestroy(dstream);
  return rc;
}

int bgv_aggregate_pubkeys(bgv_ctx* c, const uint32_t* idx, size_t n, uint8_t out96[96]) {
  if (!c || !out96 || (n && !idx)) return -BGV_E_ARG;
  if (n == 0) return -BGV_E_EMPTY_AGGREGATE;
  std::shared_lock<std::shared_mutex> clk(c->cache_mu);
  if (c->closed) return -BGV_E_CLOSED;
  for (size_t i = 0; i < n; ++i)
    if (idx[i] >= c->n_pubkeys || c->bad_pk.count(idx[i])) return -BGV_E_BAD_INDEX;
  std::lock_guard<std::mutex> lk(c->util_mu);
  Device& d = c->devs[0];
  HIPCHK(hipSetDevice(d.id));
  bgv_dslot s;
  memset(&s, 0, sizeof(s));
  s.flags = BGV_SLOT_PK_CACHED;
  s.n_pk = (uint32_t)n;
  uint32_t* di = nullptr;
  uint8_t* dout = nullptr;
  bgv_dslot* ds = nullptr;
  void* dagg = nullptr;
  HIPCHK(hipMalloc(reinterpret_cast<void**>(&di), 4 * n));
  HIPCHK(hipMalloc(reinterpret_cast<void**>(&dout), 96));
  HIPCHK(hipMalloc(reinterpret_cast<void**>(&ds), sizeof(bgv_dslot)));
  HIPCHK(hipMalloc(&dagg, bgv_g1_point_bytes()));
  HIPCHK(hipMemcpyAsync(di, idx, 4 * n, hipMemcpyHostToDevice, d.stream));
  HIPCHK(hipMemcpyAsync(ds, &s, sizeof(s), hipMemcpyHostToDevice, d.stream));
  HIPCHK(bgv_launch_aggregate(ds, di, (uint32_t)n, d.cache, dagg, dout, d.stream));
  HIPCHK(hipMemcpyAsync(out96, dout, 96, hipMemcpyDeviceToHost, d.stream));
  HIPCHK(hipStreamSynchronize(d.stream));
  void* bufs[] = {di, dout, ds, dagg};
  for (void* p : bufs) (void)hipFree(p);
  return BGV_OK;
}

int bgv_aggregate_committee_bits(bgv_ctx* c, uint32_t id, const uint8_t* bits, uint32_t n_bits, uint8_t out96[96]) {
  if (!c || !out96 || (n_bits && !bits)) return -BGV_E_ARG;
  std::shared_lock<std::shared_mutex> clk(c->cache_mu);
  if (c->closed) return -BGV_E_CLOSED;
  const uint8_t zero[96] = {0};
  bgv_set st{};
  st.sig_len = 96;
  st.msg = zero;
  st.sig = zero;
  const bgv_pkbits pb{id, n_bits, bits};
  const bgv_job jb{0, 1, 0};
  Call call;
  call.setcom.assign(1, SetCommittee{});
  int32_t code = 2;
  {
    std::shared_lock<std::shared_mutex> mlk(c->com_mu);
    if (host_job_code(c, jb, &st, &code, &pb, &call) != BGV_OK) return -BGV_E_ARG;
  }
  if (code != 2) return code;
  Layout L;
  std::vector<size_t> todo;
  layout_call(L, todo, &jb, 1, &st, BGV_MODE_PER_JOB, {2}, call.setcom.data());
  const uint32_t list = 0;
  std::lock_guard<std::mutex> lk(c->util_mu);
  Device& d = c->devs[0];
  HIPCHK(hipSetDevice(d.id));
  uint32_t* di = nullptr;
  uint8_t* dout = nullptr;
  bgv_dslot* ds = nullptr;
  void* dagg = nullptr;
  const bool ok =
      hipMalloc(reinterpret_cast<void**>(&di), 4 * (L.idx.size() + 1)) == hipSuccess &&
      hipMalloc(reinterpret_cast<void**>(&dout), 96) == hipSuccess &&
      hipMalloc(reinterpret_cast<void**>(&ds), sizeof(bgv_dslot)) == hipSuccess &&
      hipMalloc(&dagg, bgv_g1_point_bytes()) == hipSuccess &&
      hipMemcpyAsync(di, L.idx.data(), 4 * L.idx.size(), hipMemcpyHostToDevice, d.stream) == hipSuccess &&
      hipMemcpyAsync(di + L.idx.size(), &list, 4, hipMemcpyHostToDevice, d.stream) == hipSuccess &&
      hipMemcpyAsync(ds, L.slots.data(), sizeof(bgv_dslot), hipMemcpyHostToDevice, d.stream) == hipSuccess &&
      bgv_launch_aggregate_bits(ds, di, di + L.idx.size(), !L.com_team.empty(), d.com_dir, d.com_pool, d.cache, dagg,
                                dout, d.stream) == hipSuccess &&
      hipMemcpyAsync(out96, dout, 96, hipMemcpyDeviceToHost, d.stream) == hipSuccess;
  const bool done = hipStreamSynchronize(d.stream) == hipSuccess;
  void* bufs[] = {di, dout, ds, dagg};
  for (void* p : bufs)
    if (p) (void)hipFree(p);
  return ok && done ? BGV_OK : -BGV_E_DEVICE;
}

int bgv_hash_to_g2(bgv_ctx* c, const uint8_t* msgs, const uint32_t* lens, size_t n, uint8_t* out192) {
  if (!c || (n && (!lens || !out192))) return -BGV_E_ARG;
  std::shared_lock<std::shared_mutex> clk(c->cache_mu);
  if (c->closed) return -BGV_E_CLOSED;
  if (n == 0) return BGV_OK;
  std::vector<uint32_t> offs(n);
  size_t tot = 0;
  for (size_t i = 0; i < n; ++i) {
    if (lens[i] > 1024) return -BGV_E_ARG;
    offs[i] = (uint32_t)tot;
    tot += lens[i];
  }
  if (tot && !msgs) return -BGV_E_ARG;
  std::lock_guard<std::mutex> lk(c->util_mu);
  Device& d = c->devs[0];
  HIPCHK(hipSetDevice(d.id));
  uint8_t *dm = nullptr, *dout = nullptr;
  uint32_t *doff = nullptr, *dlen = nullptr;
  HIPCHK(hipMalloc(reinterpret_cast<void**>(&dm), tot + 1));
  HIPCHK(hipMalloc(reinterpret_cast<void**>(&doff), 4 * n));
  HIPCHK(hipMalloc(reinterpret_cast<void**>(&dlen), 4 * n));
  HIPCHK(hipMalloc(reinterpret_cast<void**>(&dout), 192 * n));
  if (tot) HIPCHK(hipMemcpyAsync(dm, msgs, tot, hipMemcpyHostToDevice, d.stream));
  HIPCHK(hipMemcpyAsync(doff, offs.data(), 4 * n, hipMemcpyHostToDevice, d.stream));
  HIPCHK(hipMemcpyAsync(dlen, lens, 4 * n, hipMemcpyHostToDevice, d.stream));
  HIPCHK(bgv_launch_hash(dm, doff, dlen, (uint32_t)n, dout, d.stream));
  HIPCHK(hipMemcpyAsync(out192, dout, 192 * n, hipMemcpyDeviceToHost, d.stream));
  HIPCHK(hipStreamSynchronize(d.stream));
  (void)hipFree(dm);
  (void)hipFree(doff);
  (void)hipFree(dlen);
  (void)hipFree(dout);
  return BGV_OK;
}

int bgv_pubkeys_validate(bgv_ctx* c, const uint8_t* keys48, size_t n, int32_t* out_status, uint8_t* out96) {
  if (!c || (n && (!keys48 || !out_status))) return -BGV_E_ARG;
  std::shared_lock<std::shared_mutex> clk(c->cache_mu);
  if (c->closed) return -BGV_E_CLOSED;
  if (n == 0) return BGV_OK;
  std::lock_guard<std::mutex> lk(c->util_mu);
  Device& d = c->devs[0];
  HIPCHK(hipSetDevice(d.id));
  uint8_t *dk = nullptr, *dout = nullptr;
  int32_t* dst = nullptr;
  HIPCHK(hipMalloc(reinterpret_cast<void**>(&dk), 48 * n));
  HIPCHK(hipMalloc(reinterpret_cast<void**>(&dout), 96 * n));
  HIPCHK(hipMalloc(reinterpret_cast<void**>(&dst), 4 * n));
  HIPCHK(hipMemcpyAsync(dk, keys48, 48 * n, hipMemcpyHostToDevice, d.stream));
  HIPCHK(bgv_launch_pk_validate(dk, (uint32_t)n, dst, dout, d.stream));
  HIPCHK(hipMemcpyAsync(out_status, dst, 4 * n, hipMemcpyDeviceToHost, d.stream));
  if (out96) HIPCHK(hipMemcpyAsync(out96, dout, 96 * n, hipMemcpyDeviceToHost, d.stream));
  HIPCHK(hipStreamSynchronize(d.stream));
  (void)hipFree(dk);
  (void)hipFree(dout);
  (void)hipFree(dst);
  for (size_t i = 0; i < n; ++i) out_status[i] = -out_status[i];
  return BGV_OK;
}

int bgv_aggregate_signatures(bgv_ctx* c, const uint8_t* sigs96, const uint32_t* lens, const uint32_t* counts,
                             size_t naggs, uint8_t* out96, int32_t* out_status) {
  if (!c || (naggs && (!counts || !out96 || !out_status))) return -BGV_E_ARG;
  std::shared_lock<std::shared_mutex> clk(c->cache_mu);
  if (c->closed) return -BGV_E_CLOSED;
  if (naggs == 0) return BGV_OK;
  std::vector<uint32_t> first(naggs);
  size_t n = 0;
  for (size_t a = 0; a < naggs; ++a) {
    first[a] = (uint32_t)n;
    n += counts[a];
  }
  if (n && (!sigs96 || !lens)) return -BGV_E_ARG;
  std::vector<int32_t> st(n);
  std::lock_guard<std::mutex> lk(c->util_mu);
  Device& d = c->devs[0];
  HIPCHK(hipSetDevice(d.id));
  uint8_t *ds = nullptr, *dout = nullptr;
  uint32_t *dl = nullptr, *df = nullptr, *dc = nullptr;
  int32_t* dst = nullptr;
  void* pts = nullptr;
  HIPCHK(hipMalloc(reinterpret_cast<void**>(&ds), 96 * n + 1));
  HIPCHK(hipMalloc(reinterpret_cast<void**>(&dl), 4 * n + 4));
  HIPCHK(hipMalloc(reinterpret_cast<void**>(&dst), 4 * n + 4));
  HIPCHK(hipMalloc(&pts, bgv_g2_point_bytes() * n + 1));
  HIPCHK(hipMalloc(reinterpret_cast<void**>(&df), 4 * naggs));
  HIPCHK(hipMalloc(reinterpret_cast<void**>(&dc), 4 * naggs));
  HIPCHK(hipMalloc(reinterpret_cast<void**>(&dout), 96 * naggs));
  if (n) {
    HIPCHK(hipMemcpyAsync(ds, sigs96, 96 * n, hipMemcpyHostToDevice, d.stream));
    HIPCHK(hipMemcpyAsync(dl, lens, 4 * n, hipMemcpyHostToDevice, d.stream));
  }
  HIPCHK(hipMemcpyAsync(df, first.data(), 4 * naggs, hipMemcpyHostToDevice, d.stream));
  HIPCHK(hipMemcpyAsync(dc, counts, 4 * naggs, hipMemcpyHostToDevice, d.stream));
  HIPCHK(bgv_launch_sig_aggregate(ds, dl, (uint32_t)n, df, dc, (uint32_t)naggs, pts, dst, dout, d.stream));
  if (n) HIPCHK(hipMemcpyAsync(st.data(), dst, 4 * n, hipMemcpyDeviceToHost, d.stream));
  HIPCHK(hipMemcpyAsync(out96, dout, 96 * naggs, hipMemcpyDeviceToHost, d.stream));
  HIPCHK(hipStreamSynchronize(d.stream));
  void* bufs[] = {ds, dl, dst, pts, df, dc, dout};
  for (void* b : bufs) (void)hipFree(b);
  for (size_t a = 0; a < naggs; ++a) {
    int32_t code = counts[a] ? BGV_OK : -BGV_E_EMPTY_AGGREGATE;
    for (uint32_t k = 0; k < counts[a] && code == BGV_OK; ++k)
      if (st[first[a] + k] != BGV_OK) code = -st[first[a] + k];
    out_status[a] = code;
    if (code != BGV_OK) memset(out96 + 96 * a, 0, 96);
  }
  return BGV_OK;
}

int bgv_deposits_verify(bgv_ctx* c, const uint8_t* keys48, const uint8_t* msgs32, const uint8_t* sigs96, size_t n,
                        int32_t* out_valid) {
  if (!c || (n && (!keys48 || !msgs32 || !sigs96 || !out_valid))) return -BGV_E_ARG;
  if (n == 0) return BGV_OK;
  std::vector<int32_t> ks(n);
  std::vector<uint8_t> pk96(96 * n);
  int rc = bgv_pubkeys_validate(c, keys48, n, ks.data(), pk96.data());
  if (rc) return rc;
  std::vector<bgv_set> sets;
  std::vector<bgv_job> jobs;
  std::vector<size_t> which;
  for (size_t i = 0; i < n; ++i) {
    out_valid[i] = 0;
    if (ks[i] != BGV_OK) continue;
    bgv_set st{};
    st.n_pk = 1;
    st.sig_len = 96;
    st.pk_bytes = pk96.data() + 96 * i;
    st.msg = msgs32 + 32 * i;
    st.sig = sigs96 + 96 * i;
    jobs.push_back(bgv_job{(uint32_t)sets.size(), 1, 0});
    sets.push_back(st);
    which.push_back(i);
  }
  if (jobs.empty()) return BGV_OK;
  std::vector<int32_t> codes(jobs.size());
  rc = bgv_verify(c, jobs.data(), jobs.size(), sets.data(), sets.size(), BGV_MODE_PER_JOB, codes.data(), nullptr);
  if (rc) return rc;
  for (size_t k = 0; k < which.size(); ++k) out_valid[which[k]] = codes[k] == 1 ? 1 : 0;
  return BGV_OK;
}

int bgv_keygen(bgv_ctx* c, const uint8_t* sks, size_t n, int64_t cache_first, uint8_t* out48) {
  if (!c || (n && !sks)) return -BGV_E_ARG;
  std::lock_guard<std::mutex> plk(c->put_mu);
  std::unique_lock<std::shared_mutex> clk(c->cache_mu);
  if (c->closed) return -BGV_E_CLOSED;
  if (cache_first > (int64_t)c->n_pubkeys) return -BGV_E_ARG;
  if (n == 0) return BGV_OK;
  if (cache_first >= 0) {
    int rc = cache_reserve(c, (size_t)cache_first + n);
    if (rc) return rc;
  }
  const size_t esz = bgv_cache_entry_bytes();
  for (size_t di = 0; di < c->devs.size(); ++di) {
    Device& d = c->devs[di];
    if (cache_first < 0 && di > 0) break;
    HIPCHK(hipSetDevice(d.id));
    uint8_t *dsk = nullptr, *dout = nullptr;
    HIPCHK(hipMalloc(reinterpret_cast<void**>(&dsk), 32 * n));
    HIPCHK(hipMalloc(reinterpret_cast<void**>(&dout), 48 * n));
    HIPCHK(hipMemcpyAsync(dsk, sks, 32 * n, hipMemcpyHostToDevice, d.stream));
    bgv_cache_entry* dst =
        cache_first >= 0 ? reinterpret_cast<bgv_cache_entry*>(reinterpret_cast<uint8_t*>(d.cache) + esz * cache_first)
                         : nullptr;
    HIPCHK(bgv_launch_keygen(dsk, (uint32_t)n, dst, dout, d.stream));
    if (out48 && di == 0) HIPCHK(hipMemcpyAsync(out48, dout, 48 * n, hipMemcpyDeviceToHost, d.stream));
    HIPCHK(hipStreamSynchronize(d.stream));
    (void)hipFree(dsk);
    (void)hipFree(dout);
  }
  if (cache_first >= 0) {
    const size_t old_n = c->n_pubkeys.load();
    for (size_t i = 0; i < n; ++i) c->bad_pk.erase((uint32_t)(cache_first + i));
    c->n_pubkeys.store(std::max(old_n, (size_t)cache_first + n));
    if ((size_t)cache_first < old_n) return committees_refresh(c, (uint32_t)cache_first, n);
  }
  return BGV_OK;
}

int bgv_sign(bgv_ctx* c, const uint8_t* sks, const uint8_t* msgs, size_t n, uint8_t* out96) {
  if (!c || (n && (!sks || !msgs || !out96))) return -BGV_E_ARG;
  std::shared_lock<std::shared_mutex> clk(c->cache_mu);
  if (c->closed) return -BGV_E_CLOSED;
  if (n == 0) return BGV_OK;
  std::lock_guard<std::mutex> lk(c->util_mu);
  Device& d = c->devs[0];
  HIPCHK(hipSetDevice(d.id));
  uint8_t *dsk = nullptr, *dm = nullptr, *dout = nullptr;
  HIPCHK(hipMalloc(reinterpret_cast<void**>(&dsk), 32 * n));
  HIPCHK(hipMalloc(reinterpret_cast<void**>(&dm), 32 * n));
  HIPCHK(hipMalloc(reinterpret_cast<void**>(&dout), 96 * n));
  HIPCHK(hipMemcpyAsync(dsk, sks, 32 * n, hipMemcpyHostToDevice, d.stream));
  HIPCHK(hipMemcpyAsync(dm, msgs, 32 * n, hipMemcpyHostToDevice, d.stream));
  HIPCHK(bgv_launch_sign(dsk, dm, (uint32_t)n, dout, d.stream));
  HIPCHK(hipMemcpyAsync(out96, dout, 96 * n, hipMemcpyDeviceToHost, d.stream));
  HIPCHK(hipStreamSynchronize(d.stream));
  (void)hipFree(dsk);
  (void)hipFree(dm);
  (void)hipFree(dout);
  return BGV_OK;
}

int bgv_profile(bgv_ctx* c, int enable, double* kernel_ms, const char** names, int n, uint64_t* launches) {
  if (!c) return -BGV_E_ARG;
  std::lock_guard<std::mutex> lk(c->prof_mu);
  for (int k = 0; k < n && k < BGV_NKERNELS; ++k) {
    if (kernel_ms) kernel_ms[k] = c->kernel_ms[k];
    if (names) names[k] = BGV_KERNEL_NAMES[k];
  }
  if (launches) *launches = c->kernel_launches;
  if (enable >= 0) {
    c->profile = enable != 0;
    for (double& v : c->kernel_ms) v = 0;
    c->kernel_launches = 0;
  }
  return BGV_NKERNELS;
}

const char* bgv_strerror(int code) {
  if (code < 0) code = -code;
  switch (code) {
    case BGV_OK: return "BLST_SUCCESS";
    case BGV_BLST_BAD_ENCODING: return "BLST_BAD_ENCODING";
    case BGV_BLST_POINT_NOT_ON_CURVE: return "BLST_POINT_NOT_ON_CURVE";
    case BGV_BLST_POINT_NOT_IN_GROUP: return "BLST_POINT_NOT_IN_GROUP";
    case BGV_BLST_AGGR_TYPE_MISMATCH: return "BLST_AGGR_TYPE_MISMATCH";
    case BGV_BLST_VERIFY_FAIL: return "BLST_VERIFY_FAIL";
    case BGV_BLST_PK_IS_INFINITY: return "BLST_PK_IS_INFINITY";
    case BGV_BLST_BAD_SCALAR: return "BLST_BAD_SCALAR";
    case BGV_BLST_INVALID_SIZE: return "BLST_INVALID_SIZE";
    case BGV_E_EMPTY_AGGREGATE: return "EMPTY_AGGREGATE_ARRAY";
    case BGV_E_EMPTY_SET: return "Empty signature set";
    case BGV_E_BAD_INDEX: return "BGV_E_BAD_INDEX: validator index not in the device pubkey cache";
    case BGV_E_ARG: return "BGV_E_ARG: invalid argument";
    case BGV_E_DEVICE: return "BGV_E_DEVICE: HIP device error";
    case BGV_E_NOMEM: return "BGV_E_NOMEM";
    case BGV_E_CLOSED: return "QUEUE_ABORTED";
    default: return "BGV_E_UNKNOWN";
  }
}

}
```

### lodestar_amd/csrc/bgv_device.h

```cpp
#pragma once
#include <stdlib.h>
#include "bgv_layout.h"
#define BGV_KERNEL_SIDE 1
#include "bls_hash.h"
#include "bls_pairing.h"
#include "bls_team.h"

#ifndef BGV_WPE
#define BGV_WPE 1
#endif
#ifndef BGV_WPE_PREP
#define BGV_WPE_PREP 1
#endif
#ifndef BGV_PK_TREE_MIN
#define BGV_PK_TREE_MIN 16
#endif
#ifndef BGV_PK_TEAM_MAX
#define BGV_PK_TEAM_MAX 256
#endif
#define BGV_KATTR __launch_bounds__(64) __attribute__((amdgpu_waves_per_eu(BGV_WPE, BGV_WPE)))
#define BGV_KATTR_PREP __launch_bounds__(64) __attribute__((amdgpu_waves_per_eu(BGV_WPE_PREP, BGV_WPE_PREP)))

template <int M>
__device__ __forceinline__ uint32_t lane_xor(uint32_t v) {
  if constexpr (M == 32)
    return (uint32_t)__builtin_amdgcn_ds_bpermute((int)((threadIdx.x ^ 32u) << 2), (int)v);
  else
    return (uint32_t)__builtin_amdgcn_ds_swizzle((int)v, 0x1f | (M << 10));
}

template <int M, class P>
__device__ __forceinline__ P point_xor(const P& p) {
  constexpr int W = (int)(sizeof(P) / 4);
  P r;
  const uint32_t* a = reinterpret_cast<const uint32_t*>(&p);
  uint32_t* o = reinterpret_cast<uint32_t*>(&r);
  BGV_UNROLL for (int i = 0; i < W; ++i) o[i] = lane_xor<M>(a[i]);
  return r;
}



__device__ __forceinline__ bool grp_has(const bgv_dgroup& g, uint32_t k) {
  return k < g.n_slots && (k >= 64 || ((g.mask >> k) & 1));
}

__device__ __forceinline__ bool slot_live(const bgv_dslot& d, int32_t ss, int32_t ps) {
  return !(d.flags & BGV_SLOT_PAD) && (ss == BGV_ST_OK || ss == BGV_ST_INFINITY) && ps == BGV_ST_OK;
}

#include "bgv_launch.h"

static inline unsigned nblk(uint32_t n, unsigned t) { return (n + t - 1) / t; }

#define BGV_PREP_WIDE_MAX 340
#define BGV_MILLER_WIDE_MAX 1024

static inline uint32_t bgv_latency_max() {
  static const uint32_t v = [] {
    const char* e = getenv("BGV_LATENCY_MAX");
    return e ? (uint32_t)strtoul(e, nullptr, 10) : 16384u;
  }();
  return v;
}

static inline bool bgv_use_latency(const bgv_dev_batch& b, uint32_t pairs) {
  return b.path == BGV_PATH_LATENCY || (b.path == BGV_PATH_AUTO && pairs <= bgv_latency_max());
}

#define BGV_MARK(i) \
  if (s.kev) (void)hipEventRecord(s.kev[i], s.main)
```

### lodestar_amd/csrc/bgv_host_layout.h

```cpp
#pragma once
#include <stdint.h>
#include <stdlib.h>
#include <string.h>

#include <algorithm>
#include <memory>
#include <thread>
#include <unordered_map>
#include <utility>
#include <vector>

#include "../../include/blsgpu.h"
#include "bgv_layout.h"
#include "bgv_pk_bits.h"

namespace {

inline size_t env_size(const char* name, size_t dflt, size_t lo) {
  const char* e = getenv(name);
  long n = e ? atol(e) : 0;
  return n >= (long)lo ? (size_t)n : dflt;
}
#define BGV_GROUP_SLOTS 64
inline uint32_t group_slots() {
  static const uint32_t v = [] {
    size_t n = env_size("BGV_GROUP_SLOTS", BGV_GROUP_SLOTS, 1);
    uint32_t p = 1;
    while (p * 2 <= n && p * 2 <= BGV_WAVE) p *= 2;
    return p;
  }();
  return v;
}
inline bool uniform_enabled() {
  static const bool v = [] {
    const char* e = getenv("BGV_UNIFORM");
    return !(e && atoi(e) == 0);
  }();
  return v;
}
#define BGV_UNIFORM_MIN_JOBS 1024
static const size_t kUniformAlignMin = 32;

template <class F>
inline void par_ranges(size_t n, F fn) {
  const size_t kMin = size_t(1) << 17;
  const unsigned nt = n >= kMin ? std::min<unsigned>(8u, std::max(1u, std::thread::hardware_concurrency())) : 1u;
  if (nt <= 1) {
    fn(size_t(0), n);
    return;
  }
  std::vector<std::thread> th;
  for (unsigned t = 1; t < nt; ++t) th.emplace_back(fn, n * t / nt, n * (t + 1) / nt);
  fn(size_t(0), n / nt);
  for (auto& t : th) t.join();
}

template <class T>
struct uninit_alloc : std::allocator<T> {
  template <class U>
  struct rebind {
    using other = uninit_alloc<U>;
  };
  uninit_alloc() = default;
  template <class U>
  uninit_alloc(const uninit_alloc<U>&) {}
  template <class U>
  void construct(U* p) noexcept {
    ::new (static_cast<void*>(p)) U;
  }
  template <class U, class... A>
  void construct(U* p, A&&... a) {
    ::new (static_cast<void*>(p)) U(std::forward<A>(a)...);
  }
};

struct CommitteeInfo {
  uint32_t handle;
  uint32_t n;
  bool bad;
};
struct SetCommittee {
  uint32_t handle = BGV_NO_COMMITTEE;
  uint32_t n = 0;
  uint32_t k = 0;
  const uint8_t* bits = nullptr;
};
inline int32_t committee_set_check(const CommitteeInfo* ci, const bgv_pkbits& pb, SetCommittee* out) {
  if (!ci) return -BGV_E_BAD_INDEX;
  if (pb.n_bits != ci->n) return -BGV_E_ARG;
  const uint32_t nbytes = (pb.n_bits + 7u) / 8u;
  if ((pb.n_bits & 7u) && (pb.bits[nbytes - 1] >> (pb.n_bits & 7u))) return -BGV_E_ARG;
  uint32_t k = 0;
  for (uint32_t i = 0; i < nbytes; ++i) k += (uint32_t)__builtin_popcount(pb.bits[i]);
  if (k == 0) return -BGV_E_EMPTY_AGGREGATE;
  if (ci->bad) return -BGV_E_BAD_INDEX;
  *out = SetCommittee{ci->handle, ci->n, k, pb.bits};
  return 2;
}

struct Layout {
  std::vector<bgv_dslot, uninit_alloc<bgv_dslot>> slots;
  std::vector<bgv_dgroup> groups;
  std::vector<int32_t> slot_set;
  std::vector<std::vector<uint32_t>> job_groups;
  std::vector<uint32_t> job_first_slot;
  std::vector<char> group_shared;
  std::vector<char> group_uniform;
  std::vector<uint32_t> idx;
  std::vector<uint8_t> pkb;
  std::vector<uint32_t> uniq;
  std::vector<uint32_t> com_team, com_wave;
};

inline bgv_dslot rebase_slot(bgv_dslot s, uint32_t slot_base, uint32_t ib, uint32_t pb, uint32_t gb) {
  s.hsrc += slot_base;
  if (s.flags & (BGV_SLOT_PK_CACHED | BGV_SLOT_PK_COMMITTEE)) s.pk_off += ib;
  if (s.flags & BGV_SLOT_PK_BYTES) s.pk_off += pb;
  if (!(s.flags & BGV_SLOT_PAD)) s.group += gb;
  return s;
}

struct RootIndex {
  std::unordered_map<uint64_t, uint32_t> first;
  template <class MsgOf>
  uint32_t source(uint32_t self, const uint8_t* msg, const uint8_t* prev_msg, uint32_t prev_src, MsgOf msg_of) {
    if (prev_msg && memcmp(prev_msg, msg, 32) == 0) return prev_src;
    uint64_t key;
    memcpy(&key, msg, 8);
    auto it = first.find(key);
    if (it == first.end()) it = first.emplace(key, self).first;
    return it->second != self && memcmp(msg_of(it->second), msg, 32) == 0 ? it->second : self;
  }
};

struct Builder {
  Layout& L;
  bool open = false;
  uint32_t open_group = 0;
  int open_job = -1;
  RootIndex roots;
  explicit Builder(Layout& l) : L(l) {}

  void close_group() { open = false; }
  void new_group() {
    uint32_t first = (uint32_t)L.slots.size();
    const uint32_t gs = group_slots();
    uint32_t aligned = (first + gs - 1) / gs * gs;
    while (L.slots.size() < aligned) pad();
    L.groups.push_back(bgv_dgroup{aligned, 0, BGV_ALL_SLOTS});
    L.group_shared.push_back(0);
    L.group_uniform.push_back(1);
    open_group = (uint32_t)L.groups.size() - 1;
    open = true;
    open_job = -1;
  }
  void pad() {
    bgv_dslot s;
    memset(&s, 0, sizeof(s));
    s.flags = BGV_SLOT_PAD;
    s.hsrc = (uint32_t)L.slots.size();
    L.slots.push_back(s);
    L.slot_set.push_back(-1);
  }
  void pad_to_wave() {
    while (L.slots.size() % BGV_WAVE) pad();
  }
  void add(int job, uint32_t set_index, const bgv_set& st, bool first_of_job, const SetCommittee* sc = nullptr) {
    if (!open || L.groups[open_group].n_slots == group_slots()) new_group();
    bgv_dgroup& g = L.groups[open_group];
    if (open_job >= 0 && open_job != job) L.group_shared[open_group] = 1;
    open_job = job;
    std::vector<uint32_t>& jg = L.job_groups[job];
    if (jg.empty() || jg.back() != open_group) jg.push_back(open_group);
    if (first_of_job) L.job_first_slot[job] = (uint32_t)L.slots.size();
    bgv_dslot s;
    memset(&s, 0, sizeof(s));
    s.n_pk = st.n_pk;
    s.sig_len = st.sig_len;
    s.group = open_group;
    if (sc && sc->handle != BGV_NO_COMMITTEE) {
      const bool comp = pkb_use_complement(sc->n, sc->k);
      s.flags = BGV_SLOT_PK_COMMITTEE | (comp ? BGV_SLOT_PK_COMPLEMENT : 0u);
      s.n_pk = sc->k;
      s.pk_off = (uint32_t)L.idx.size();
      L.idx.push_back(sc->handle);
      const uint32_t nbytes = (sc->n + 7u) / 8u;
      for (uint32_t w = 0; w < pkb_nwords(sc->n); ++w) {
        uint32_t v = 0;
        for (uint32_t q = 0; q < 4 && 4 * w + q < nbytes; ++q) v |= (uint32_t)sc->bits[4 * w + q] << (8 * q);
        L.idx.push_back(v);
      }
      (pkb_terms(sc->n, sc->k, comp) <= BGV_PK_TEAM_MAX ? L.com_team : L.com_wave).push_back((uint32_t)L.slots.size());
    } else if (st.pk_indices) {
      s.flags = BGV_SLOT_PK_CACHED;
      s.pk_off = (uint32_t)L.idx.size();
      L.idx.insert(L.idx.end(), st.pk_indices, st.pk_indices + st.n_pk);
    } else {
      s.flags = BGV_SLOT_PK_BYTES;
      s.pk_off = (uint32_t)(L.pkb.size() / 96);
      L.pkb.insert(L.pkb.end(), st.pk_bytes, st.pk_bytes + 96ull * st.n_pk);
    }
    memcpy(s.msg, st.msg, 32);
    if (st.sig_len == 96) memcpy(s.sig, st.sig, 96);
    const uint32_t self = (uint32_t)L.slots.size();
    const bgv_dslot* prev = self > 0 && !(L.slots[self - 1].flags & BGV_SLOT_PAD) ? &L.slots[self - 1] : nullptr;
    s.hsrc = roots.source(self, st.msg, prev ? prev->msg : nullptr, prev ? prev->hsrc : 0,
                          [&](uint32_t i) { return L.slots[i].msg; });
    if (s.hsrc == self) L.uniq.push_back(self);
    if (g.n_slots > 0 && L.slots[g.first_slot].hsrc != s.hsrc) L.group_uniform[open_group] = 0;
    L.slots.push_back(s);
    L.slot_set.push_back((int32_t)set_index);
    g.n_slots++;
  }
};

inline bool layout_one_job_fast(Layout& L, const bgv_job& jb, const bgv_set* sets, const SetCommittee* sc = nullptr) {
  const uint32_t n = jb.n_sets, gs = group_slots();
  const bgv_set* S = sets + jb.first_set;
  if (n < (1u << 17)) return false;
  for (uint32_t i = 0; i < n; ++i)
    if (!S[i].pk_indices || (sc && sc[jb.first_set + i].handle != BGV_NO_COMMITTEE)) return false;
  std::vector<uint32_t> hsrc(n), pk_off(n);
  RootIndex roots;
  uint32_t npk = 0;
  for (uint32_t i = 0; i < n; ++i) {
    pk_off[i] = npk;
    npk += S[i].n_pk;
    hsrc[i] = roots.source(i, S[i].msg, i > 0 ? S[i - 1].msg : nullptr, i > 0 ? hsrc[i - 1] : 0,
                           [&](uint32_t q) { return S[q].msg; });
    if (hsrc[i] == i) L.uniq.push_back(i);
  }
  const uint32_t nslots = (n + BGV_WAVE - 1) / BGV_WAVE * BGV_WAVE, ng = (n + gs - 1) / gs;
  L.slots.resize(nslots);
  L.slot_set.resize(nslots);
  L.idx.resize(npk);
  par_ranges(nslots, [&](size_t lo, size_t hi) {
    for (size_t i = lo; i < hi; ++i) {
      bgv_dslot& s = L.slots[i];
      memset(&s, 0, sizeof(s));
      if (i >= n) {
        s.flags = BGV_SLOT_PAD;
        s.hsrc = (uint32_t)i;
        L.slot_set[i] = -1;
        continue;
      }
      const bgv_set& st = S[i];
      s.n_pk = st.n_pk;
      s.sig_len = st.sig_len;
      s.group = (uint32_t)(i / gs);
      s.flags = BGV_SLOT_PK_CACHED;
      s.pk_off = pk_off[i];
      memcpy(L.idx.data() + pk_off[i], st.pk_indices, 4ull * st.n_pk);
      memcpy(s.msg, st.msg, 32);
      if (st.sig_len == 96) memcpy(s.sig, st.sig, 96);
      s.hsrc = hsrc[i];
      L.slot_set[i] = (int32_t)(jb.first_set + i);
    }
  });
  L.groups.resize(ng);
  L.group_shared.assign(ng, 0);
  L.group_uniform.assign(ng, 1);
  for (uint32_t g = 0; g < ng; ++g) {
    const uint32_t f = g * gs, m = std::min(gs, n - f);
    L.groups[g] = bgv_dgroup{f, m, BGV_ALL_SLOTS};
    for (uint32_t k = 1; k < m; ++k)
      if (hsrc[f + k] != hsrc[f]) {
        L.group_uniform[g] = 0;
        break;
      }
  }
  L.job_groups[0].resize(ng);
  for (uint32_t g = 0; g < ng; ++g) L.job_groups[0][g] = g;
  L.job_first_slot[0] = 0;
  return true;
}

inline void layout_call(Layout& L, std::vector<size_t>& todo, const bgv_job* jobs, size_t njobs, const bgv_set* sets,
                        int mode, const std::vector<int32_t>& code, const SetCommittee* sc = nullptr) {
  auto shared_job = [&](size_t j) { return mode == BGV_MODE_WORKER && jobs[j].batchable; };
  L.job_groups.resize(njobs);
  L.job_first_slot.assign(njobs, 0);
  Builder B(L);
  for (size_t j = 0; j < njobs; ++j)
    if (code[j] == 2) todo.push_back(j);
  const bool fast = njobs == 1 && todo.size() == 1 && !shared_job(0) && layout_one_job_fast(L, jobs[0], sets, sc);
  auto add_job = [&](size_t j) {
    for (uint32_t k = 0; k < jobs[j].n_sets; ++k)
      B.add((int)j, jobs[j].first_set + k, sets[jobs[j].first_set + k], k == 0,
            sc ? sc + jobs[j].first_set + k : nullptr);
  };
  for (size_t j : todo) {
    if (shared_job(j) || fast) continue;
    B.close_group();
    add_job(j);
    B.close_group();
  }
  B.close_group();
  std::vector<size_t> shared_order;
  std::vector<size_t> breaks;
  size_t n_one = 0;
  for (size_t j : todo)
    if (shared_job(j) && jobs[j].n_sets == 1) ++n_one;
  if (uniform_enabled() && n_one >= BGV_UNIFORM_MIN_JOBS) {
    std::unordered_map<uint64_t, uint32_t> bucket_of;
    bucket_of.reserve(2 * n_one);
    std::vector<std::vector<size_t>> buckets;
    std::vector<const uint8_t*> broot;
    bool grouped = false;
    uint32_t last = UINT32_MAX;
    for (size_t j : todo) {
      if (!shared_job(j) || jobs[j].n_sets != 1) continue;
      const uint8_t* m = sets[jobs[j].first_set].msg;
      uint64_t key;
      memcpy(&key, m, 8);
      auto it = bucket_of.find(key);
      uint32_t b;
      if (it != bucket_of.end() && memcmp(broot[it->second], m, 32) == 0) {
        b = it->second;
      } else {
        b = (uint32_t)buckets.size();
        buckets.emplace_back();
        broot.push_back(m);
        if (it == bucket_of.end()) bucket_of.emplace(key, b);
      }
      grouped = grouped || (b != last && !buckets[b].empty());
      last = b;
      buckets[b].push_back(j);
    }
    if (grouped) {
      for (const auto& bk : buckets)
        if (bk.size() >= kUniformAlignMin) {
          breaks.push_back(shared_order.size());
          shared_order.insert(shared_order.end(), bk.begin(), bk.end());
        }
      breaks.push_back(shared_order.size());
      for (const auto& bk : buckets)
        if (bk.size() < kUniformAlignMin) shared_order.insert(shared_order.end(), bk.begin(), bk.end());
      for (size_t j : todo)
        if (shared_job(j) && jobs[j].n_sets != 1) shared_order.push_back(j);
    }
  }
  if (shared_order.empty())
    for (size_t j : todo)
      if (shared_job(j)) shared_order.push_back(j);
  size_t bi = 0;
  for (size_t q = 0; q < shared_order.size(); ++q) {
    if (bi < breaks.size() && breaks[bi] == q) B.close_group();
    while (bi < breaks.size() && breaks[bi] <= q) ++bi;
    add_job(shared_order[q]);
  }
  B.pad_to_wave();
  for (size_t j : todo)
    if (L.job_groups[j].size() > 1 && shared_job(j))
      for (uint32_t g : L.job_groups[j]) L.group_uniform[g] = 0;
}

}
```

### lodestar_amd/csrc/bgv_k_prep.hip

```cpp
#include "bgv_k_lat.h"
#include "bgv_pk_bits.h"
#include "bgv_team_dev.h"
#include "bgv_tcurve.h"
#include "bgv_tg1.h"
#include "bgv_tround_dev.h"

static __constant__ uint8_t kTcProg[TCP_TABLE_BYTES] = TCP_TABLE_INIT;
static __constant__ uint8_t kTg1Prog[TG1_TABLE_BYTES] = TG1_TABLE_INIT;

struct tc_dev_engine {
  const uint8_t* prog;
  fp_t* S;
  int c;
  bool bad;
  __device__ void run(int off) {
    int pos = off;
    const int nr = prog[pos++];
    for (int r = 0; r < nr; ++r) {
      const int T = prog[pos], M = prog[pos + 1];
      pos += 2;
      const int rb = tmp_rec_bytes(T, M);
      int out;
      const fp_t v = tmp_lane_any(S, prog + pos + c * rb, T, M, &out);
      S[out] = v;
      __syncthreads();
      pos += BGV_TEAM * rb;
    }
  }
  __device__ void copy(int dst, int src) {
    if (c < 6 && dst != src) S[TCP_BANK(dst) + c] = S[TCP_BANK(src) + c];
    __syncthreads();
  }
  __device__ void neg_y(int b) {
    if (c == 2 || c == 3) S[TCP_BANK(b) + c] = fp_neg(S[TCP_BANK(b) + c]);
    __syncthreads();
  }
  __device__ void check_add() {
    if (c == 0) {
      const auto z2 = [&](int s) { return fp_is_zero(S[s]) && fp_is_zero(S[s + 1]); };
      bad = bad || z2(TC_CHK_A) || z2(TC_CHK_B);
    }
  }
};

#ifndef BGV_WPE_AGG
#define BGV_WPE_AGG 2
#endif

static_assert(sizeof(g1_jac) == sizeof(bgv_dcommittee::total), "bgv_dcommittee keeps a Jacobian G1 point");
template <int T>
__device__ __forceinline__ g1_jac pk_bits_sum(bool act, uint32_t l, const uint32_t* __restrict__ words,
                                              const uint32_t* __restrict__ members, uint32_t n, bool comp,
                                              const g1_aff* __restrict__ cache) {
  g1_jac acc = jac_infinity<fp_t>();
  if (act) {
    pkb_cursor c = pkb_begin(l);
    uint32_t pos;
    if (pkb_next(c, words, n, comp, T, &pos)) {
      acc = jac_from_aff(cache[members[pos]]);
      bool have = pkb_next(c, words, n, comp, T, &pos);
      g1_aff cur = cache[members[have ? pos : 0]];
      while (have) {
        uint32_t pn;
        const bool hn = pkb_next(c, words, n, comp, T, &pn);
        const g1_aff nxt = cache[members[hn ? pn : pos]];
        acc = jac_add_aff(acc, cur);
        cur = nxt;
        pos = hn ? pn : pos;
        have = hn;
      }
    }
  }
  if constexpr (T == 64) {
    acc = jac_add(acc, point_xor<32>(acc));
    acc = jac_add(acc, point_xor<16>(acc));
  }
  acc = jac_add(acc, point_xor<8>(acc));
  acc = jac_add(acc, point_xor<4>(acc));
  acc = jac_add(acc, point_xor<2>(acc));
  acc = jac_add(acc, point_xor<1>(acc));
  return acc;
}

template <int T>
__device__ __forceinline__ void pk_bits_slot(bool act, uint32_t s, uint32_t l, const bgv_dslot* __restrict__ slots,
                                             const uint32_t* __restrict__ pk_idx,
                                             const bgv_dcommittee* __restrict__ dir,
                                             const uint32_t* __restrict__ pool, const g1_aff* __restrict__ cache,
                                             g1_jac* __restrict__ pk_agg, bool writer) {
  const uint32_t* words = nullptr;
  const uint32_t* members = nullptr;
  const bgv_dcommittee* cm = nullptr;
  uint32_t n = 0;
  bool comp = false;
  if (act) {
    const bgv_dslot& d = slots[s];
    cm = dir + pk_idx[d.pk_off];
    words = pk_idx + d.pk_off + 1;
    members = pool + cm->off;
    n = cm->n;
    comp = (d.flags & BGV_SLOT_PK_COMPLEMENT) != 0;
  }
  g1_jac acc = pk_bits_sum<T>(act, l, words, members, n, comp, cache);
  if (act && writer) {
    if (comp) acc = jac_add(*reinterpret_cast<const g1_jac*>(cm->total), jac_neg(acc));
    pk_agg[s] = acc;
  }
}

extern "C" {

__device__ __forceinline__ void pk_aggw_body(const bgv_dslot* __restrict__ slots, uint32_t s,
                                             const uint32_t* __restrict__ pk_idx, const g1_aff* __restrict__ cache,
                                             g1_jac* __restrict__ pk_agg) {
  const bgv_dslot& d = slots[s];
  if ((d.flags & BGV_SLOT_PAD) || !(d.flags & BGV_SLOT_PK_CACHED) || d.n_pk <= BGV_PK_TEAM_MAX) return;
  const uint32_t l = threadIdx.x;
  g1_jac acc = jac_infinity<fp_t>();
  for (uint32_t k = l; k < d.n_pk; k += 64) acc = jac_add_aff(acc, cache[pk_idx[d.pk_off + k]]);
  acc = jac_add(acc, point_xor<32>(acc));
  acc = jac_add(acc, point_xor<16>(acc));
  acc = jac_add(acc, point_xor<8>(acc));
  acc = jac_add(acc, point_xor<4>(acc));
  acc = jac_add(acc, point_xor<2>(acc));
  acc = jac_add(acc, point_xor<1>(acc));
  if (l == 0) pk_agg[s] = acc;
}

__device__ __forceinline__ void pk_agg16_body(const bgv_dslot* __restrict__ slots, uint32_t nslots, uint32_t blk,
                                              const uint32_t* __restrict__ pk_idx, const g1_aff* __restrict__ cache,
                                              g1_jac* __restrict__ pk_agg) {
  const uint32_t s = blk * (64 / 16) + threadIdx.x / 16;
  const uint32_t l = threadIdx.x % 16;
  const bgv_dslot* d = s < nslots ? &slots[s] : nullptr;
  const bool act = d && !(d->flags & BGV_SLOT_PAD) && (d->flags & BGV_SLOT_PK_CACHED) &&
                   d->n_pk >= BGV_PK_TREE_MIN && d->n_pk <= BGV_PK_TEAM_MAX;
  g1_jac acc = jac_infinity<fp_t>();
  if (act) {
    const uint32_t* idx = pk_idx + d->pk_off;
    const uint32_t n = d->n_pk;
    acc = jac_from_aff(cache[idx[l]]);
    uint32_t k = l + 16;
    g1_aff cur = cache[idx[k < n ? k : l]];
    for (; k < n; k += 16) {
      const uint32_t kn = k + 16 < n ? k + 16 : k;
      const g1_aff nxt = cache[idx[kn]];
      acc = jac_add_aff(acc, cur);
      cur = nxt;
    }
  }
  acc = jac_add(acc, point_xor<8>(acc));
  acc = jac_add(acc, point_xor<4>(acc));
  acc = jac_add(acc, point_xor<2>(acc));
  acc = jac_add(acc, point_xor<1>(acc));
  if (act && l == 0) pk_agg[s] = acc;
}

__device__ __forceinline__ void pk_agg_one(const bgv_dslot* __restrict__ slots, uint32_t s,
                                           const uint32_t* __restrict__ pk_idx, const g1_aff* __restrict__ cache,
                                           g1_jac* __restrict__ pk_agg) {
  const bgv_dslot& d = slots[s];
  if ((d.flags & BGV_SLOT_PAD) || !(d.flags & BGV_SLOT_PK_CACHED) || d.n_pk < BGV_PK_TREE_MIN) return;
  if (d.n_pk > BGV_PK_TEAM_MAX) {
    pk_aggw_body(slots, s, pk_idx, cache, pk_agg);
    return;
  }
  const uint32_t l = threadIdx.x % 16;
  const uint32_t* idx = pk_idx + d.pk_off;
  const uint32_t n = d.n_pk;
  g1_jac acc = jac_from_aff(cache[idx[l]]);
  for (uint32_t k = l + 16; k < n; k += 16) acc = jac_add_aff(acc, cache[idx[k]]);
  acc = jac_add(acc, point_xor<8>(acc));
  acc = jac_add(acc, point_xor<4>(acc));
  acc = jac_add(acc, point_xor<2>(acc));
  acc = jac_add(acc, point_xor<1>(acc));
  if (threadIdx.x == 0) pk_agg[s] = acc;
}

#ifndef BGV_WPE_BITS
#define BGV_WPE_BITS 1
#endif
__global__ void __launch_bounds__(64) __attribute__((amdgpu_waves_per_eu(BGV_WPE_BITS, BGV_WPE_BITS)))
k_pk_agg_bits(const bgv_dslot* __restrict__ slots, const uint32_t* __restrict__ com, uint32_t nteam, uint32_t nwave,
              const uint32_t* __restrict__ pk_idx, const bgv_dcommittee* __restrict__ dir,
              const uint32_t* __restrict__ pool, const g1_aff* __restrict__ cache, g1_jac* __restrict__ pk_agg) {
  const uint32_t nb_team = (nteam + 3) / 4;
  if (blockIdx.x < nb_team) {
    const uint32_t q = blockIdx.x * 4 + threadIdx.x / 16, l = threadIdx.x % 16;
    const bool act = q < nteam;
    pk_bits_slot<16>(act, act ? com[q] : 0u, l, slots, pk_idx, dir, pool, cache, pk_agg, l == 0);
  } else {
    const uint32_t q = nteam + (blockIdx.x - nb_team);
    const bool act = q < nteam + nwave;
    pk_bits_slot<64>(act, act ? com[q] : 0u, threadIdx.x, slots, pk_idx, dir, pool, cache, pk_agg, threadIdx.x == 0);
  }
}

#define BGV_PK_ONE_WAVE_MIN 49
__device__ __noinline__ void pk_bits_one(const bgv_dslot* __restrict__ slots, uint32_t s,
                                            const uint32_t* __restrict__ pk_idx,
                                            const bgv_dcommittee* __restrict__ dir,
                                            const uint32_t* __restrict__ pool, const g1_aff* __restrict__ cache,
                                            g1_jac* __restrict__ pk_agg) {
  const bgv_dslot& d = slots[s];
  if ((d.flags & BGV_SLOT_PAD) || !(d.flags & BGV_SLOT_PK_COMMITTEE)) return;
  const uint32_t n = dir[pk_idx[d.pk_off]].n;
  if (pkb_terms(n, d.n_pk, (d.flags & BGV_SLOT_PK_COMPLEMENT) != 0) < BGV_PK_ONE_WAVE_MIN)
    pk_bits_slot<16>(true, s, threadIdx.x % 16, slots, pk_idx, dir, pool, cache, pk_agg, threadIdx.x == 0);
  else
    pk_bits_slot<64>(true, s, threadIdx.x, slots, pk_idx, dir, pool, cache, pk_agg, threadIdx.x == 0);
}

__global__ void __launch_bounds__(64) k_committee_total(bgv_dcommittee* __restrict__ dir,
                                                        const uint32_t* __restrict__ handles, uint32_t nh,
                                                        const uint32_t* __restrict__ pool,
                                                        const g1_aff* __restrict__ cache) {
  if (blockIdx.x >= nh) return;
  bgv_dcommittee* cm = dir + handles[blockIdx.x];
  const g1_jac acc = pk_bits_sum<64>(true, threadIdx.x, nullptr, pool + cm->off, cm->n, false, cache);
  if (threadIdx.x == 0) *reinterpret_cast<g1_jac*>(cm->total) = acc;
}

__global__ void __launch_bounds__(64) k_pk_agg(const bgv_dslot* __restrict__ slots, uint32_t nslots,
                                               const uint32_t* __restrict__ pk_idx,
                                               const g1_aff* __restrict__ cache, g1_jac* __restrict__ pk_agg) {
  if (blockIdx.x < nslots) pk_aggw_body(slots, blockIdx.x, pk_idx, cache, pk_agg);
}

__global__ void BGV_KATTR_PREP k_prep_a(const bgv_dslot* __restrict__ slots, uint32_t nslots, g2_jac* __restrict__ h,
                                        fp12_t* __restrict__ f, int32_t* __restrict__ sig_status,
                                        const uint32_t* __restrict__ pk_idx, const g1_aff* __restrict__ cache,
                                        const uint8_t* __restrict__ pk_bytes, g1_jac* __restrict__ rpk,
                                        int32_t* __restrict__ pk_status, g1_jac* __restrict__ pk_agg) {
  const uint32_t s = blockIdx.x * blockDim.x + threadIdx.x;
  if (s >= nslots) return;
  if (blockIdx.y == 0)
    task_map_t<bgv_pow_lane>(s, 0, slots, h + s, true);
  else if (blockIdx.y == 1)
    task_map_t<bgv_pow_lane>(s, 1, slots, split_q1(f, s), true);
  else if (blockIdx.y == 2)
    task_sig_decode_t<bgv_pow_lane>(s, slots, split_sig(f, s), sig_status, true);
  else
    task_pk(s, slots, pk_idx, cache, pk_bytes, rpk, pk_status, pk_agg);
}

__global__ void __launch_bounds__(64) k_prep_team(const bgv_dslot* __restrict__ slots, uint32_t nslots,
                                                  g2_jac* __restrict__ h, fp12_t* __restrict__ f,
                                                  g2_jac* __restrict__ rsig, int32_t* __restrict__ sig_status) {
  if (blockIdx.y == 2) {
    const uint32_t s = blockIdx.x * blockDim.x + threadIdx.x;
    if (s >= nslots || (slots[s].flags & BGV_SLOT_PAD) || sig_status[s] != BGV_ST_OK) return;
    if (!g2_in_subgroup(jac_from_aff(*split_sig(f, s)))) sig_status[s] = BGV_POINT_NOT_IN_GROUP;
    return;
  }
  __shared__ uint8_t prog[TCP_TABLE_BYTES];
  __shared__ fp_t Sall[BGV_FINAL_TEAMS][TCP_NSLOT];
  __shared__ int flags[BGV_FINAL_TEAMS];
  for (int i = threadIdx.x; i < TCP_TABLE_BYTES; i += 64) prog[i] = kTcProg[i];
  const int team = threadIdx.x / BGV_TEAM, c = threadIdx.x % BGV_TEAM;
  const uint32_t u = blockIdx.x * BGV_FINAL_TEAMS + team;
  const uint32_t uu = u < nslots ? u : nslots - 1;
  const bgv_dslot& d = slots[uu];
  const bool real = u < nslots && !(d.flags & BGV_SLOT_PAD);
  fp_t* S = Sall[team];
  if (c == 6) {
    S[TCP_S_ONE] = fp_one();
  } else if (c >= 7 && c < 11) {
    const fp2_t cx = BGV_PSI_CX, cy = BGV_PSI_CY;
    const fp2_t& v = c < 9 ? cx : cy;
    S[c < 9 ? TCP_S_PSI_CX + (c - 7) : TCP_S_PSI_CY + (c - 9)] = (c & 1) ? v.c0 : v.c1;
  } else if (c == 11) {
    S[TCP_S_PSI2_CX] = fp_t{BGV_PSI2_CX};
  } else if (c == 12) {
    S[TCP_S_PSI2_CY] = fp_t{BGV_PSI2_CY};
  }
  for (int i = c; i < TC_ISO_NCONST; i += BGV_TEAM) S[TCP_S_ISO + i] = tc_iso_const(i);
  tc_dev_engine e{prog, S, c, false};
  if (blockIdx.y == 0) {
    if (c < 6) {
      S[TCP_BANK(1) + c] = reinterpret_cast<const fp_t*>(h + uu)[c];
      S[TCP_BANK(2) + c] = reinterpret_cast<const fp_t*>(split_q1(f, uu))[c];
    }
    __syncthreads();
    tc_clear_cofactor(e);
    if (c == 0) flags[team] = e.bad ? 1 : 0;
    __syncthreads();
    if (real) {
      if (!flags[team]) {
        if (c < 6) reinterpret_cast<fp_t*>(h + uu)[c] = S[TCP_BANK(3) + c];
      } else if (c == 0) {
        h[uu] = g2_clear_cofactor(jac_add(iso_map_g2_jac(h[uu]), iso_map_g2_jac(*split_q1(f, uu))));
      }
    }
  } else {
    const bool ok = sig_status[uu] == BGV_ST_OK;
    if (c < 4)
      S[TCP_BANK(1) + c] = reinterpret_cast<const fp_t*>(split_sig(f, uu))[c];
    else if (c < 6)
      S[TCP_BANK(1) + c] = c == 4 ? fp_one() : fp_zero();
    __syncthreads();
    tc_mul_glv(e, d.scalar);
    if (real && ok && c < 6) reinterpret_cast<fp_t*>(rsig + uu)[c] = S[TCP_BANK(4) + c];
  }
}

struct tc_wide_engine : tr_wide_engine {
  __device__ void copy(int dst, int src) {
    if (q == 0 && c < 6 && dst != src) S[TCP_BANK(dst) + c] = S[TCP_BANK(src) + c];
    __syncthreads();
  }
  __device__ void neg_y(int b) {
    if (q == 0 && (c == 2 || c == 3)) S[TCP_BANK(b) + c] = fp_neg(S[TCP_BANK(b) + c]);
    __syncthreads();
  }
  __device__ void check_add() {
    if (q == 0 && c == 0) {
      const auto z2 = [&](int s) { return fp_is_zero(S[s]) && fp_is_zero(S[s + 1]); };
      bad = bad || z2(TC_CHK_A) || z2(TC_CHK_B);
    }
  }
};

struct tg1_wide_engine : tr_wide_engine {
  __device__ void copy(int dst, int src) {
    if (q == 0 && c < 3 && dst != src) S[TG1_BANK(dst) + c] = S[TG1_BANK(src) + c];
    __syncthreads();
  }
};

__global__ void __launch_bounds__(64) k_prep_wide(const bgv_dslot* __restrict__ slots, uint32_t nslots,
                                                  g2_jac* __restrict__ h, fp12_t* __restrict__ f,
                                                  g2_jac* __restrict__ rsig, int32_t* __restrict__ sig_status,
                                                  const uint32_t* __restrict__ pk_idx,
                                                  const g1_aff* __restrict__ cache, const uint8_t* __restrict__ pk_bytes,
                                                  g1_jac* __restrict__ rpk, int32_t* __restrict__ pk_status,
                                                  g1_jac* __restrict__ pk_agg,
                                                  const bgv_dcommittee* __restrict__ com_dir,
                                                  const uint32_t* __restrict__ com_pool) {
  static_assert(TG1_TABLE_BYTES <= TCP_TABLE_BYTES && TG1_NSLOT <= TCP_NSLOT, "plane 3 reuses the G2 buffers");
  __shared__ uint8_t prog[TCP_TABLE_BYTES];
  __shared__ fp_t S[TCP_NSLOT];
  __shared__ fp_t RP[64];
  __shared__ int flag;
  if (blockIdx.y == 3) {
    const uint32_t s = blockIdx.x;
    if (pk_agg) pk_agg_one(slots, s, pk_idx, cache, pk_agg);
    if (pk_agg) pk_bits_one(slots, s, pk_idx, com_dir, com_pool, cache, pk_agg);
    if (threadIdx.x == 0) {
      g1_jac acc;
      const bool go = task_pk_sum(s, slots, pk_idx, cache, pk_bytes, pk_status, pk_agg, &acc);
      flag = go ? 1 : 0;
      if (go) {
        S[TG1_BANK(1)] = acc.x;
        S[TG1_BANK(1) + 1] = acc.y;
        S[TG1_BANK(1) + 2] = acc.z;
      }
      S[TG1_S_ONE] = fp_one();
      S[TG1_S_BETA] = fp_t{BGV_BETA_MX2};
    }
    for (int i = threadIdx.x; i < TG1_TABLE_BYTES; i += 64) prog[i] = kTg1Prog[i];
    __syncthreads();
    if (!flag) return;
    const int lane = threadIdx.x;
    tg1_wide_engine e{{prog, S, RP, tr_wide_lane_c(lane), tr_wide_lane_q(lane), false}};
    tg1_mul_glv(e, slots[s].scalar);
    if (lane < 3) reinterpret_cast<fp_t*>(rpk + s)[lane] = S[TG1_BANK(4) + lane];
    if (lane == 0) pk_status[s] = BGV_ST_OK;
    return;
  }
  const uint32_t uu = blockIdx.x;
  const int lane = threadIdx.x, c = lane % BGV_TEAM, q = lane / BGV_TEAM;
  const bgv_dslot& d = slots[uu];
  const bool real = !(d.flags & BGV_SLOT_PAD);
  if (blockIdx.y == 2 && (!real || sig_status[uu] != BGV_ST_OK)) return;
  for (int i = lane; i < TCP_TABLE_BYTES; i += 64) prog[i] = kTcProg[i];
  if (q == 0) {
    if (c == 6) {
      S[TCP_S_ONE] = fp_one();
    } else if (c >= 7 && c < 11) {
      const fp2_t cx = BGV_PSI_CX, cy = BGV_PSI_CY;
      const fp2_t& v = c < 9 ? cx : cy;
      S[c < 9 ? TCP_S_PSI_CX + (c - 7) : TCP_S_PSI_CY + (c - 9)] = (c & 1) ? v.c0 : v.c1;
    } else if (c == 11) {
      S[TCP_S_PSI2_CX] = fp_t{BGV_PSI2_CX};
    } else if (c == 12) {
      S[TCP_S_PSI2_CY] = fp_t{BGV_PSI2_CY};
    }
  }
  for (int i = lane; i < TC_ISO_NCONST; i += 64) S[TCP_S_ISO + i] = tc_iso_const(i);
  tc_wide_engine e{{prog, S, RP, tr_wide_lane_c(lane), tr_wide_lane_q(lane), false}};
  if (blockIdx.y == 0) {
    if (q == 0 && c < 6) {
      S[TCP_BANK(1) + c] = reinterpret_cast<const fp_t*>(h + uu)[c];
      S[TCP_BANK(2) + c] = reinterpret_cast<const fp_t*>(split_q1(f, uu))[c];
    }
    __syncthreads();
    tc_clear_cofactor(e);
    if (lane == 0) flag = e.bad ? 1 : 0;
    __syncthreads();
    if (real) {
      if (!flag) {
        if (q == 0 && c < 6) reinterpret_cast<fp_t*>(h + uu)[c] = S[TCP_BANK(3) + c];
      } else if (lane == 0) {
        h[uu] = g2_clear_cofactor(jac_add(iso_map_g2_jac(h[uu]), iso_map_g2_jac(*split_q1(f, uu))));
      }
    }
  } else if (blockIdx.y == 1) {
    const bool ok = sig_status[uu] == BGV_ST_OK;
    if (q == 0) {
      if (c < 4)
        S[TCP_BANK(1) + c] = reinterpret_cast<const fp_t*>(split_sig(f, uu))[c];
      else if (c < 6)
        S[TCP_BANK(1) + c] = c == 4 ? fp_one() : fp_zero();
    }
    __syncthreads();
    tc_mul_glv(e, d.scalar);
    if (real && ok && q == 0 && c < 6) reinterpret_cast<fp_t*>(rsig + uu)[c] = S[TCP_BANK(4) + c];
  } else {
    if (q == 0 && c < 6) {
      const fp_t v = c < 4 ? reinterpret_cast<const fp_t*>(split_sig(f, uu))[c] : (c == 4 ? fp_one() : fp_zero());
      S[TCP_BANK(0) + c] = v;
      S[TCP_BANK(4) + c] = v;
    }
    __syncthreads();
    const int a = tc_to_jac(e, tc_mul_x_abs(e));
    if (lane == 0) {
      const g2_jac p = jac_from_aff(*split_sig(f, uu));
      bool in;
      if (e.bad) {
        in = g2_in_subgroup(p);
      } else {
        const fp_t* B = S + TCP_BANK(a);
        const g2_jac xp = {{B[0], B[1]}, {B[2], B[3]}, {B[4], B[5]}};
        in = jac_eq(g2_psi(p), jac_neg(xp));
      }
      if (!in) sig_status[uu] = BGV_POINT_NOT_IN_GROUP;
    }
  }
}

__global__ void __launch_bounds__(64) __attribute__((amdgpu_waves_per_eu(BGV_WPE_AGG, BGV_WPE_AGG)))
k_pk_agg16(const bgv_dslot* __restrict__ slots, uint32_t nslots, const uint32_t* __restrict__ pk_idx,
           const g1_aff* __restrict__ cache, g1_jac* __restrict__ pk_agg) {
  pk_agg16_body(slots, nslots, blockIdx.x, pk_idx, cache, pk_agg);
}

__global__ void k_pk_sum_out(const bgv_dslot* __restrict__ slot, const uint32_t* __restrict__ idx,
                             const g1_aff* __restrict__ cache, const g1_jac* __restrict__ pk_agg,
                             uint8_t* __restrict__ out96) {
  if (blockIdx.x != 0 || threadIdx.x != 0) return;
  int32_t st = BGV_OK;
  const g1_jac acc = pk_sum(slot[0], idx, cache, nullptr, pk_agg, 0, &st);
  g1_aff a;
  const bool fin = jac_to_aff(&a, acc);
  uint8_t b[96];
  g1_serialize(b, a, !fin);
  for (int i = 0; i < 96; ++i) out96[i] = b[i];
}

}

hipError_t bgv_launch_prep(const bgv_dev_batch& b, const bgv_streams& s) {
  const uint32_t n = b.nslots;
  if (n == 0) return hipSuccess;
  BGV_MARK(0);
  const bool tree = b.max_npk >= BGV_PK_TREE_MIN;
  const uint32_t ncom = b.ncom_team + b.ncom_wave;
  const bool agg = tree || ncom > 0;
  const bool wide = bgv_use_latency(b, n + b.ngroups) && n <= BGV_PREP_WIDE_MAX;
  if (wide) {
    const g1_aff* cache = reinterpret_cast<const g1_aff*>(b.cache_opaque);
    const hipError_t e = bgv_launch_prep_wave(b, s.main);
    if (e != hipSuccess) return e;
    hipLaunchKernelGGL(k_prep_wide, dim3(n, 4), dim3(64), 0, s.main, b.slots, n, b.h, b.f, b.rsig, b.sig_status,
                       b.pk_idx, cache, b.pk_bytes, b.rpk, b.pk_status, agg ? b.pk_agg : nullptr, b.com_dir, b.com_pool);
    BGV_MARK(1);
    return hipGetLastError();
  }
  if (ncom)
    hipLaunchKernelGGL(k_pk_agg_bits, dim3(nblk(b.ncom_team, 4) + b.ncom_wave), dim3(64), 0, s.main, b.slots, b.com,
                       b.ncom_team, b.ncom_wave, b.pk_idx, b.com_dir, b.com_pool,
                       reinterpret_cast<const g1_aff*>(b.cache_opaque), b.pk_agg);
  if (tree)
    hipLaunchKernelGGL(k_pk_agg16, dim3(nblk(n, 4)), dim3(64), 0, s.main, b.slots, n, b.pk_idx,
                       reinterpret_cast<const g1_aff*>(b.cache_opaque), b.pk_agg);
  if (b.max_npk > BGV_PK_TEAM_MAX)
    hipLaunchKernelGGL(k_pk_agg, dim3(n), dim3(64), 0, s.main, b.slots, n, b.pk_idx,
                       reinterpret_cast<const g1_aff*>(b.cache_opaque), b.pk_agg);
  if (bgv_use_latency(b, n + b.ngroups)) {
    hipLaunchKernelGGL(k_prep_a, dim3(nblk(n, 64), 4), dim3(64), 0, s.main, b.slots, n, b.h, b.f, b.sig_status,
                       b.pk_idx, reinterpret_cast<const g1_aff*>(b.cache_opaque), b.pk_bytes, b.rpk, b.pk_status,
                       agg ? b.pk_agg : nullptr);
    hipLaunchKernelGGL(k_prep_team, dim3(nblk(n, BGV_FINAL_TEAMS), 3), dim3(64), 0, s.main, b.slots, n, b.h, b.f,
                       b.rsig, b.sig_status);
  } else {
    const hipError_t e = bgv_launch_prep_bulk(b, s, agg);
    if (e != hipSuccess) return e;
  }
  BGV_MARK(1);
  return hipGetLastError();
}

hipError_t bgv_launch_aggregate(const bgv_dslot* slot, const uint32_t* idx, uint32_t n, const bgv_cache_entry* cache,
                                void* agg, uint8_t* out96, hipStream_t st) {
  const g1_aff* c = reinterpret_cast<const g1_aff*>(cache);
  g1_jac* a = reinterpret_cast<g1_jac*>(agg);
  const bool tree = n >= BGV_PK_TREE_MIN;
  if (tree && n <= BGV_PK_TEAM_MAX) hipLaunchKernelGGL(k_pk_agg16, dim3(1), dim3(64), 0, st, slot, 1u, idx, c, a);
  if (tree && n > BGV_PK_TEAM_MAX) hipLaunchKernelGGL(k_pk_agg, dim3(1), dim3(64), 0, st, slot, 1u, idx, c, a);
  hipLaunchKernelGGL(k_pk_sum_out, dim3(1), dim3(64), 0, st, slot, idx, c, tree ? a : nullptr, out96);
  return hipGetLastError();
}

hipError_t bgv_launch_aggregate_bits(const bgv_dslot* slot, const uint32_t* idx, const uint32_t* list, bool team,
                                     const bgv_dcommittee* dir, const uint32_t* pool, const bgv_cache_entry* cache,
                                     void* agg, uint8_t* out96, hipStream_t st) {
  const g1_aff* c = reinterpret_cast<const g1_aff*>(cache);
  g1_jac* a = reinterpret_cast<g1_jac*>(agg);
  hipLaunchKernelGGL(k_pk_agg_bits, dim3(1), dim3(64), 0, st, slot, list, team ? 1u : 0u, team ? 0u : 1u, idx, dir, pool,
                     c, a);
  hipLaunchKernelGGL(k_pk_sum_out, dim3(1), dim3(64), 0, st, slot, idx, c, a, out96);
  return hipGetLastError();
}

hipError_t bgv_launch_committee_totals(bgv_dcommittee* dir, const uint32_t* handles, uint32_t nh, const uint32_t* pool,
                                       const bgv_cache_entry* cache, hipStream_t st) {
  if (nh == 0) return hipSuccess;
  hipLaunchKernelGGL(k_committee_total, dim3(nh), dim3(64), 0, st, dir, handles, nh, pool,
                     reinterpret_cast<const g1_aff*>(cache));
  return hipGetLastError();
}
```

### lodestar_amd/csrc/bgv_k_prep_bulk.hip

```cpp
#ifndef BGV_LZ2_CLASSIC
#define BGV_LZ2_WIDE 1
#define BGV_LZ2_WIDE_STRICT 1
#endif
#include "bgv_k_tasks.h"

#ifndef BGV_WPE_BULK
#define BGV_WPE_BULK 1
#endif
#define BGV_KATTR_BULK __launch_bounds__(64) __attribute__((amdgpu_waves_per_eu(BGV_WPE_BULK, BGV_WPE_BULK)))

extern "C" {

__global__ void BGV_KATTR_BULK k_prep(const bgv_dslot* __restrict__ slots, uint32_t nslots, g2_jac* __restrict__ rsig,
                                      int32_t* __restrict__ sig_status, g2_jac* __restrict__ h,
                                      const uint32_t* __restrict__ pk_idx, const g1_aff* __restrict__ cache,
                                      const uint8_t* __restrict__ pk_bytes, g1_jac* __restrict__ rpk,
                                      int32_t* __restrict__ pk_status, const g1_jac* __restrict__ pk_agg,
                                      const uint32_t* __restrict__ uniq, uint32_t nuniq, uint32_t task0) {
  const uint32_t s = blockIdx.x * blockDim.x + threadIdx.x;
  const uint32_t task = blockIdx.y + task0;
  if (task == 0) {
    if (uniq) {
      if (s < nuniq) task_hash(uniq[s], slots, h);
    } else if (s < nslots) {
      task_hash(s, slots, h);
    }
    return;
  }
  if (s >= nslots) return;
  if (task == 1)
    task_sig(s, slots, rsig, sig_status);
  else
    task_pk(s, slots, pk_idx, cache, pk_bytes, rpk, pk_status, pk_agg);
}

}

hipError_t bgv_launch_prep_bulk(const bgv_dev_batch& b, const bgv_streams& s, bool tree) {
  static const bool split = [] {
    const char* e = getenv("BGV_PREP_SPLIT");
    return e && atoi(e) > 0;
  }();
  for (uint32_t t0 = 0; t0 < 3; t0 += split ? 1 : 3) {
    hipLaunchKernelGGL(k_prep, dim3(nblk(b.nslots, 64), split ? 1 : 3), dim3(64), 0, s.main, b.slots, b.nslots, b.rsig,
                       b.sig_status, b.h, b.pk_idx, reinterpret_cast<const g1_aff*>(b.cache_opaque), b.pk_bytes, b.rpk,
                       b.pk_status, tree ? b.pk_agg : nullptr, b.uniq, b.nuniq, t0);
  }
  return hipGetLastError();
}
```

### lodestar_amd/csrc/bgv_k_tasks.h

```cpp
#pragma once
#include "bgv_device.h"

static __device__ __noinline__ void task_sig(uint32_t s, const bgv_dslot* __restrict__ slots, g2_jac* __restrict__ rsig,
                                      int32_t* __restrict__ sig_status) {
  const bgv_dslot& d = slots[s];
  int32_t st = BGV_ST_OK;
  if (d.flags & BGV_SLOT_PAD) {
    st = BGV_ST_INFINITY;
  } else if (d.sig_len != 96) {
    st = BGV_INVALID_SIZE;
  } else {
    uint8_t b[96];
    for (int i = 0; i < 96; ++i) b[i] = d.sig[i];
    g2_aff a;
    bool inf;
    st = g2_decompress(&a, &inf, b);
    if (st == BGV_OK) {
      if (inf) {
        st = BGV_ST_INFINITY;
      } else {
        const g2_jac j = jac_from_aff(a);
        if (!g2_in_subgroup(j))
          st = BGV_POINT_NOT_IN_GROUP;
        else
          rsig[s] = jac_mul_glv(j, d.scalar);
      }
    }
  }
  sig_status[s] = st;
}

static __device__ __noinline__ void task_hash(uint32_t s, const bgv_dslot* __restrict__ slots, g2_jac* __restrict__ h) {
  const bgv_dslot& d = slots[s];
  if (d.flags & BGV_SLOT_PAD) return;
  uint8_t msg[32];
  for (int i = 0; i < 32; ++i) msg[i] = d.msg[i];
  h[s] = hash_to_g2(msg, 32);
}

__device__ __noinline__ static g1_jac pk_sum(const bgv_dslot& d, const uint32_t* __restrict__ pk_idx,
                                      const g1_aff* __restrict__ cache, const uint8_t* __restrict__ pk_bytes,
                                      const g1_jac* __restrict__ pk_agg, uint32_t s, int32_t* st) {
  if (d.flags & BGV_SLOT_PK_COMMITTEE) return pk_agg[s];
  g1_jac acc = jac_infinity<fp_t>();
  const bool cached = (d.flags & BGV_SLOT_PK_CACHED) != 0;
  const bool tree = pk_agg != nullptr && cached && d.n_pk >= BGV_PK_TREE_MIN;
  if (tree) return pk_agg[s];
  for (uint32_t k = 0; k < d.n_pk; ++k) {
    g1_aff a;
    if (cached) {
      a = cache[pk_idx[d.pk_off + k]];
    } else {
      uint8_t b[96];
      const uint8_t* src = pk_bytes + 96ull * (d.pk_off + k);
      for (int i = 0; i < 96; ++i) b[i] = src[i];
      bool inf;
      const int rc = g1_deserialize(&a, &inf, b);
      if (rc != BGV_OK) {
        *st = rc;
        break;
      }
      if (inf) continue;
    }
    acc = jac_add_aff(acc, a);
  }
  return acc;
}

static __device__ __noinline__ bool task_pk_sum(uint32_t s, const bgv_dslot* __restrict__ slots,
                                                const uint32_t* __restrict__ pk_idx, const g1_aff* __restrict__ cache,
                                                const uint8_t* __restrict__ pk_bytes, int32_t* __restrict__ pk_status,
                                                const g1_jac* __restrict__ pk_agg, g1_jac* acc) {
  const bgv_dslot& d = slots[s];
  if (d.flags & BGV_SLOT_PAD) {
    pk_status[s] = BGV_ST_INFINITY;
    return false;
  }
  int32_t st = BGV_ST_OK;
  const g1_jac a = pk_sum(d, pk_idx, cache, pk_bytes, pk_agg, s, &st);
  if (st != BGV_OK || jac_is_inf(a)) {
    pk_status[s] = st != BGV_OK ? st : BGV_ST_INFINITY;
    return false;
  }
  *acc = a;
  return true;
}

static __device__ __noinline__ void task_pk(uint32_t s, const bgv_dslot* __restrict__ slots,
                                     const uint32_t* __restrict__ pk_idx, const g1_aff* __restrict__ cache,
                                     const uint8_t* __restrict__ pk_bytes, g1_jac* __restrict__ rpk,
                                     int32_t* __restrict__ pk_status, const g1_jac* __restrict__ pk_agg) {
  const bgv_dslot& d = slots[s];
  int32_t st = BGV_ST_OK;
  if (d.flags & BGV_SLOT_PAD) {
    pk_status[s] = BGV_ST_INFINITY;
    return;
  }
  const g1_jac acc = pk_sum(d, pk_idx, cache, pk_bytes, pk_agg, s, &st);
  if (st == BGV_OK) {
    const g1_jac rp = jac_mul_glv(acc, d.scalar);
    if (jac_is_inf(rp))
      st = BGV_ST_INFINITY;
    else
      rpk[s] = rp;
  }
  pk_status[s] = st;
}
```

### lodestar_amd/csrc/bgv_launch.h

```cpp
#pragma once
#include <hip/hip_runtime.h>
#include <stddef.h>
#include <stdint.h>

#include "bgv_layout.h"

struct fp12_t;
template <class F>
struct jac_t;
template <class F>
struct aff_t;
struct fp_t;
struct fp2_t;

struct bgv_cache_entry;

#define BGV_PATH_AUTO 0
#ifndef BGV_PATH_BULK
#define BGV_PATH_BULK 1
#define BGV_PATH_LATENCY 2
#endif

struct bgv_dev_batch {
  uint32_t nslots, ngroups;
  uint32_t max_npk;
  bool uniform;
  int path;
  const uint32_t* uniq;
  uint32_t nuniq;
  const bgv_dslot* slots;
  const bgv_dgroup* groups;
  const uint32_t* pk_idx;
  const bgv_cache_entry* cache_opaque;
  const uint8_t* pk_bytes;
  const uint32_t* com;
  uint32_t ncom_team, ncom_wave;
  const bgv_dcommittee* com_dir;
  const uint32_t* com_pool;
  jac_t<fp2_t>* rsig;
  jac_t<fp2_t>* h;
  jac_t<fp_t>* rpk;
  fp12_t* f;
  fp12_t* fsig;
  jac_t<fp_t>* pk_agg;
  int32_t* sig_status;
  int32_t* pk_status;
  jac_t<fp2_t>* gsum;
  fp12_t* gpair;
  jac_t<fp_t>* gpk;
  fp12_t* gpkp;
  const uint32_t* upk;
  uint32_t npk;
  bool weighted;
  fp12_t* gprod;
  fp12_t* gu;
  const fp12_t* gu1;
  int32_t* verdict;
  uint32_t* lines;
  uint32_t lines_cap;
#ifdef BGV_KERNEL_SIDE
  const aff_t<fp_t>* cache_ptr() const { return reinterpret_cast<const aff_t<fp_t>*>(cache_opaque); }
#endif
};

#define BGV_NKERNELS 3
#define BGV_NSETKERNELS 2
static const char* const BGV_KERNEL_NAMES[BGV_NKERNELS] = {"k_prep", "k_miller", "k_final"};
struct bgv_streams {
  hipStream_t main;
  hipEvent_t* kev;
};
hipError_t bgv_launch_sets(const bgv_dev_batch& b, const bgv_streams& s);
bool bgv_sig_pairs(const bgv_dev_batch& b);
hipError_t bgv_launch_prep(const bgv_dev_batch& b, const bgv_streams& s);
hipError_t bgv_launch_prep_bulk(const bgv_dev_batch& b, const bgv_streams& s, bool tree);
hipError_t bgv_launch_prep_wave(const bgv_dev_batch& b, hipStream_t st);
hipError_t bgv_launch_miller(const bgv_dev_batch& b, const bgv_streams& s);
hipError_t bgv_launch_miller_bulk(const bgv_dev_batch& b, uint32_t ngroups, hipStream_t st);
uint32_t bgv_lines_pairs(const bgv_dev_batch& b);
bool bgv_single_pass_miller();
size_t bgv_line_record_bytes();
hipError_t bgv_launch_groups(const bgv_dev_batch& b, const bgv_streams& s, bool pairs);
uint32_t bgv_fold_pairs_max();
hipError_t bgv_launch_gpairs(const bgv_dev_batch& b, hipStream_t st);
size_t bgv_slot_bytes();
size_t bgv_slot_mem_bytes(uint32_t cap_slots);
size_t bgv_group_bytes();
size_t bgv_cache_entry_bytes();
void bgv_carve(bgv_dev_batch* b, void* slot_mem, uint32_t cap_slots, void* group_mem, uint32_t cap_groups);
hipError_t bgv_launch_cache_put(const uint8_t* keys, uint32_t n, int fmt, bgv_cache_entry* cache, int32_t* status,
                                hipStream_t st);
hipError_t bgv_launch_aggregate(const bgv_dslot* slot, const uint32_t* idx, uint32_t n, const bgv_cache_entry* cache,
                                void* agg, uint8_t* out96, hipStream_t st);
hipError_t bgv_launch_aggregate_bits(const bgv_dslot* slot, const uint32_t* idx, const uint32_t* list, bool team,
                                     const bgv_dcommittee* dir, const uint32_t* pool, const bgv_cache_entry* cache,
                                     void* agg, uint8_t* out96, hipStream_t st);
hipError_t bgv_launch_committee_totals(bgv_dcommittee* dir, const uint32_t* handles, uint32_t nh, const uint32_t* pool,
                                       const bgv_cache_entry* cache, hipStream_t st);
size_t bgv_shuffle_scratch_words(uint32_t n, uint32_t rounds);
hipError_t bgv_launch_shuffle(const uint8_t seed[32], uint32_t n, uint32_t rounds, uint32_t* scratch, uint32_t* out,
                              hipStream_t st);
hipError_t bgv_launch_shuffle_dir(bgv_dcommittee* dir, const uint32_t* handles, uint32_t nh, uint32_t base, uint32_t n,
                                  uint32_t count, hipStream_t st);
size_t bgv_g1_point_bytes();
hipError_t bgv_launch_debug_out(const bgv_dev_batch& b, uint8_t* out_h192, uint8_t* out_f576, hipStream_t st);
hipError_t bgv_launch_hash(const uint8_t* msgs, const uint32_t* offs, const uint32_t* lens, uint32_t n,
                           uint8_t* out192, hipStream_t st);
hipError_t bgv_launch_keygen(const uint8_t* sks, uint32_t n, bgv_cache_entry* cache, uint8_t* out48, hipStream_t st);
hipError_t bgv_launch_sign(const uint8_t* sks, const uint8_t* msgs, uint32_t n, uint8_t* out96, hipStream_t st);
hipError_t bgv_launch_pk_validate(const uint8_t* keys48, uint32_t n, int32_t* status, uint8_t* out96,
                                  hipStream_t st);
hipError_t bgv_launch_sig_aggregate(const uint8_t* sigs96, const uint32_t* lens, uint32_t n, const uint32_t* first,
                                    const uint32_t* count, uint32_t naggs, void* pts, int32_t* status,
                                    uint8_t* out96, hipStream_t st);
size_t bgv_g2_point_bytes();
size_t bgv_fp12_bytes();
hipError_t bgv_launch_fp12_bytes(const fp12_t* in, uint32_t n, uint8_t* out576, hipStream_t st);
hipError_t bgv_launch_partial(const bgv_dev_batch& b, uint32_t g0, uint32_t ng, void* scratch, uint8_t* out576,
                              hipStream_t st);
hipError_t bgv_launch_final_verify(const uint8_t* in, uint32_t n, void* vals, void* one, const bgv_dgroup* group,
                                   int32_t* status, int32_t* verdict, hipStream_t st);
```

Before: 2.726 million.

## Add opt-in zero-copy prep path and parallel chunked host merge

Adds an opt-in mode (BGV_INPLACE) where the bulk prep kernel reads slots, groups, indices and key bytes directly from pinned host memory through mapped device pointers. In that mode the kernel copies those records into device buffers itself, which removes the separate host-to-device memcpys. The host-side merge of per-call layouts is refactored into a plan plus a chunked multi-threaded merge, and random scalars are now written straight into slot records. Slot records are staged through LDS with vector loads, which adds shared-memory use and extra syncs to the prep kernel. The in-place path is off by default, so the default behaviour changes mostly through the merge refactor and the kernel staging.

```diff
diff --git a/lodestar_amd/csrc/bgv_api.cpp b/lodestar_amd/csrc/bgv_api.cpp
--- a/lodestar_amd/csrc/bgv_api.cpp
+++ b/lodestar_amd/csrc/bgv_api.cpp
@@ -47,6 +47,13 @@
   static const size_t v = env_size("BGV_SPLIT_MIN", BGV_SPLIT_MIN_SETS, 0);
   return v == 1 ? 2 : v;
 }
+static bool inplace_enabled() {
+  static const bool v = [] {
+    const char* e = getenv("BGV_INPLACE");
+    return e && atoi(e) > 0;
+  }();
+  return v;
+}
 static int dispatchers_per_device() {
   static const int v = (int)env_size("BGV_DISPATCHERS", BGV_DISPATCHERS, 1);
   return v;
@@ -76,14 +83,19 @@
 template <class T>
 struct Pinned {
   T* p = nullptr;
+  T* dev = nullptr;
   size_t cap = 0;
   hipError_t reserve(size_t n) {
     if (n <= cap) return hipSuccess;
     release();
     n = std::max(n, 2 * cap);
     hipError_t e = hipHostMalloc(reinterpret_cast<void**>(&p), std::max<size_t>(n, 1) * sizeof(T), 0);
+    if (e == hipSuccess) {
+      e = hipHostGetDevicePointer(reinterpret_cast<void**>(&dev), p, 0);
+      if (e != hipSuccess) (void)hipHostFree(p);
+    }
     if (e != hipSuccess) {
-      p = nullptr;
+      p = dev = nullptr;
       return e;
     }
     cap = n;
@@ -91,7 +103,7 @@
   }
   void release() {
     if (p) (void)hipHostFree(p);
-    p = nullptr;
+    p = dev = nullptr;
     cap = 0;
   }
 };
@@ -205,6 +217,7 @@
 struct BatchState {
   std::chrono::steady_clock::time_point tb;
   double t_merge = 0, t_tok = 0, t_sets = 0, t_pass1 = 0, t_post = 0;
+  size_t h2d_bytes = 0;
   uint32_t nslots = 0, ngroups = 0;
   std::vector<uint32_t> call_gb;
   bool want_gu = false;
@@ -313,7 +326,7 @@
   return z ^ (z >> 31);
 }
 
-static void fill_scalars(bgv_ctx* c, uint64_t* out, size_t n) {
+static void fill_scalars(bgv_ctx* c, bgv_dslot* slots, size_t n) {
   {
     std::lock_guard<std::mutex> lk(c->rng_mu);
     if (c->rng_seed) {
@@ -321,20 +334,24 @@
         uint64_t v;
         do v = splitmix64(&c->rng_state);
         while (v == 0);
-        out[i] = v;
+        slots[i].scalar = v;
       }
       return;
     }
   }
-  par_ranges(n, [out](size_t lo, size_t hi) {
-    size_t got = 0;
-    uint8_t* p = reinterpret_cast<uint8_t*>(out + lo);
-    while (got < (hi - lo) * 8) {
-      const ssize_t r = getrandom(p + got, (hi - lo) * 8 - got, 0);
-      if (r > 0) got += (size_t)r;
-    }
-    for (size_t i = lo; i < hi; ++i)
-      if (out[i] == 0) out[i] = 1;
+  par_ranges(n, [slots](size_t lo, size_t hi) {
+    uint64_t buf[512];
+    for (size_t at = lo; at < hi;) {
+      const size_t m = std::min<size_t>(hi - at, sizeof(buf) / sizeof(buf[0]));
+      size_t got = 0;
+      uint8_t* p = reinterpret_cast<uint8_t*>(buf);
+      while (got < m * 8) {
+        const ssize_t r = getrandom(p + got, m * 8 - got, 0);
+        if (r > 0) got += (size_t)r;
+      }
+      for (size_t i = 0; i < m; ++i) slots[at + i].scalar = buf[i] ? buf[i] : 1;
+      at += m;
+    }
   });
 }
 
@@ -609,21 +626,14 @@
   const auto tb = std::chrono::steady_clock::now();
   bs.tb = tb;
   double t_merge = 0, t_tok = 0, t_sets = 0, t_pass1 = 0, t_post = 0;
-  uint32_t nslots = 0, ngroups = 0;
-  size_t nidx = 0, npkb = 0, nuniq = 0, ncom_team = 0, ncom_wave = 0;
-  bool any_uniform = false;
-  for (Call* call : calls) {
-    call->slot_base = nslots;
-    nslots += (uint32_t)call->L.slots.size();
-    ngroups += (uint32_t)call->L.groups.size();
-    nidx += call->L.idx.size();
-    npkb += call->L.pkb.size();
-    nuniq += call->L.uniq.size();
-    ncom_team += call->L.com_team.size();
-    ncom_wave += call->L.com_wave.size();
-    for (char u : call->L.group_uniform) any_uniform = any_uniform || u;
-  }
-  const size_t ncom = ncom_team + ncom_wave, nlist = nuniq + ncom;
+  std::vector<const Layout*> layouts;
+  for (Call* call : calls) layouts.push_back(&call->L);
+  const MergePlan P = merge_plan(layouts);
+  for (size_t k = 0; k < calls.size(); ++k) calls[k]->slot_base = P.base[k].slot;
+  const uint32_t nslots = P.nslots, ngroups = P.ngroups;
+  const size_t nidx = P.nidx, npkb = P.npkb, nuniq = P.nuniq, ncom_team = P.ncom_team, ncom_wave = P.ncom_wave;
+  const bool any_uniform = P.any_uniform;
+  const size_t nlist = P.nlist();
   const bool bulk = nslots + ngroups > bgv_fold_pairs_max();
   const bool uniform = uniform_enabled() && any_uniform && bulk && !bgv_single_pass_miller();
   HIPCHK(hipSetDevice(d.id));
@@ -634,62 +644,15 @@
     return rc;
   HIPCHK(x.h_slots.reserve(nslots));
   HIPCHK(x.h_groups.reserve(std::max<size_t>(ngroups, 1)));
-  HIPCHK(x.h_idx.reserve(nidx + nlist));
-  HIPCHK(x.h_pkb.reserve(npkb));
+  HIPCHK(x.h_idx.reserve(std::max<size_t>(nidx + nlist, 1)));
+  HIPCHK(x.h_pkb.reserve(std::max<size_t>(npkb, 1)));
   HIPCHK(x.h_ss.reserve(nslots));
   HIPCHK(x.h_ps.reserve(nslots));
   HIPCHK(x.h_verdict.reserve(std::max<size_t>(ngroups, 1)));
   bgv_dslot* slots = x.h_slots.p;
   bgv_dgroup* groups = x.h_groups.p;
-  uint32_t max_npk = 0;
-  {
-    size_t ns = 0, ng = 0, ni = 0, npb = 0;
-    for (Call* call : calls) {
-      const uint32_t ib = (uint32_t)ni, pb = (uint32_t)(npb / 96), gb = (uint32_t)ng;
-      if (ns == 0 && ib == 0 && pb == 0 && gb == 0) {
-        const bgv_dslot* src = call->L.slots.data();
-        std::atomic<uint32_t> mx{0};
-        par_ranges(call->L.slots.size(), [&](size_t lo, size_t hi) {
-          memcpy(slots + lo, src + lo, sizeof(bgv_dslot) * (hi - lo));
-          uint32_t m = 0;
-          for (size_t i = lo; i < hi; ++i)
-            if (!(src[i].flags & BGV_SLOT_PK_COMMITTEE)) m = std::max(m, src[i].n_pk);
-          uint32_t cur = mx.load();
-          while (m > cur && !mx.compare_exchange_weak(cur, m)) {
-          }
-        });
-        max_npk = std::max(max_npk, mx.load());
-        ns = call->L.slots.size();
-      } else {
-        for (const bgv_dslot& s0 : call->L.slots) {
-          const bgv_dslot s = rebase_slot(s0, call->slot_base, ib, pb, gb);
-          if (!(s.flags & BGV_SLOT_PK_COMMITTEE)) max_npk = std::max(max_npk, s.n_pk);
-          slots[ns++] = s;
-        }
-      }
-      for (size_t gi = 0; gi < call->L.groups.size(); ++gi) {
-        const bgv_dgroup& g = call->L.groups[gi];
-        groups[ng++] = bgv_dgroup{g.first_slot + call->slot_base, g.n_slots, g.mask, 0,
-                                  uniform && call->L.group_uniform[gi] ? BGV_GROUP_UNIFORM : 0u};
-      }
-      if (!call->L.idx.empty()) memcpy(x.h_idx.p + ni, call->L.idx.data(), 4 * call->L.idx.size());
-      ni += call->L.idx.size();
-      if (!call->L.pkb.empty()) memcpy(x.h_pkb.p + npb, call->L.pkb.data(), call->L.pkb.size());
-      npb += call->L.pkb.size();
-    }
-    uint32_t* u = x.h_idx.p + nidx;
-    for (Call* call : calls)
-      for (uint32_t v : call->L.uniq) *u++ = v + call->slot_base;
-    for (Call* call : calls)
-      for (uint32_t v : call->L.com_team) *u++ = v + call->slot_base;
-    for (Call* call : calls)
-      for (uint32_t v : call->L.com_wave) *u++ = v + call->slot_base;
-  }
-  std::vector<uint64_t> sc(nslots);
-  fill_scalars(c, sc.data(), nslots);
-  par_ranges(nslots, [&](size_t lo, size_t hi) {
-    for (size_t i = lo; i < hi; ++i) slots[i].scalar = sc[i];
-  });
+  const uint32_t max_npk = merge_layouts(layouts, P, uniform, slots, groups, x.h_idx.p, x.h_pkb.p);
+  fill_scalars(c, slots, nslots);
 
   bool prof;
   {
@@ -698,11 +661,22 @@
   }
   t_merge = ms_since(tb);
   if (c->fault_inject) HIPCHK(hipErrorLaunchFailure);
-  HIPCHK(hipMemcpyAsync(x.d_slots, slots, sizeof(bgv_dslot) * nslots, hipMemcpyHostToDevice, x.main));
-  HIPCHK(hipMemcpyAsync(x.d_groups, groups, sizeof(bgv_dgroup) * ngroups, hipMemcpyHostToDevice, x.main));
-  if (nidx + nlist) HIPCHK(hipMemcpyAsync(x.d_idx, x.h_idx.p, 4 * (nidx + nlist), hipMemcpyHostToDevice, x.main));
-  if (npkb) HIPCHK(hipMemcpyAsync(x.d_pkb, x.h_pkb.p, npkb, hipMemcpyHostToDevice, x.main));
   bgv_dev_batch b = make_batch(d, x, nslots, ngroups);
+  const bool in_place = inplace_enabled() && bgv_prep_is_bulk(b) && ngroups <= nslots;
+  size_t h2d_bytes = 0;
+  if (in_place) {
+    b.in_slots = x.h_slots.dev;
+    b.in_groups = x.h_groups.dev;
+    b.in_idx = x.h_idx.dev;
+    b.in_pkb = x.h_pkb.dev;
+  } else {
+    HIPCHK(hipMemcpyAsync(x.d_slots, slots, sizeof(bgv_dslot) * nslots, hipMemcpyHostToDevice, x.main));
+    HIPCHK(hipMemcpyAsync(x.d_groups, groups, sizeof(bgv_dgroup) * ngroups, hipMemcpyHostToDevice, x.main));
+    if (nidx + nlist)
+      HIPCHK(hipMemcpyAsync(x.d_idx, x.h_idx.p, 4 * (nidx + nlist), hipMemcpyHostToDevice, x.main));
+    if (npkb) HIPCHK(hipMemcpyAsync(x.d_pkb, x.h_pkb.p, npkb, hipMemcpyHostToDevice, x.main));
+    h2d_bytes = sizeof(bgv_dslot) * nslots + sizeof(bgv_dgroup) * ngroups + 4 * (nidx + nlist) + npkb;
+  }
   b.max_npk = max_npk;
   b.uniform = uniform;
   bs.uniform = uniform;
@@ -786,16 +760,17 @@
   bs.t_sets = t_sets;
   bs.t_pass1 = t_pass1;
   bs.t_post = t_post;
+  bs.h2d_bytes = h2d_bytes;
   bs.nslots = nslots;
   bs.ngroups = ngroups;
   bs.prof = prof;
   if (trace_on() && !needs_retry(calls))
     fprintf(stderr,
             "[bgv] dev %d calls %zu slots %u groups %u | submit..dispatch %.1f | merge %.1f tokwait %.1f sets %.1f "
-            "groups %.1f post %.1f total %.1f ms\n",
+            "groups %.1f post %.1f total %.1f ms | h2d %zu B\n",
             d.id, calls.size(), nslots, ngroups,
             std::chrono::duration<double, std::milli>(tb - calls.front()->t0).count(), t_merge, t_tok, t_sets,
-            t_pass1, t_post, ms_since(tb));
+            t_pass1, t_post, ms_since(tb), h2d_bytes);
   return BGV_OK;
 }
 
@@ -879,9 +854,9 @@
   const BatchState& bs = *r.job.st;
   fprintf(stderr,
           "[bgv] dev %d calls %zu slots %u groups %u | merge %.1f tokwait %.1f sets %.1f groups %.1f post %.1f "
-          "retry(%d) %.1f total %.1f ms\n",
+          "retry(%d) %.1f total %.1f ms | h2d %zu B\n",
           d.id, r.job.calls.size(), bs.nslots, bs.ngroups, bs.t_merge, bs.t_tok, bs.t_sets, bs.t_pass1, bs.t_post,
-          r.rounds, ms_since(r.tr), ms_since(bs.tb));
+          r.rounds, ms_since(r.tr), ms_since(bs.tb), bs.h2d_bytes);
 }
 
 static Exec* exec_acquire(Device& d) {
diff --git a/lodestar_amd/csrc/bgv_device.h b/lodestar_amd/csrc/bgv_device.h
--- a/lodestar_amd/csrc/bgv_device.h
+++ b/lodestar_amd/csrc/bgv_device.h
@@ -49,6 +49,15 @@
   return !(d.flags & BGV_SLOT_PAD) && (ss == BGV_ST_OK || ss == BGV_ST_INFINITY) && ps == BGV_ST_OK;
 }
 
+struct bgv_slot_head {
+  uint32_t flags, n_pk, pk_off, sig_len;
+};
+static_assert(sizeof(bgv_dslot) % 16 == 0, "slot records keep 16-byte alignment");
+__device__ __forceinline__ bgv_slot_head slot_head(const bgv_dslot* __restrict__ slots, uint32_t s) {
+  const uint4 v = *reinterpret_cast<const uint4*>(slots + s);
+  return bgv_slot_head{v.x, v.y, v.z, v.w};
+}
+
 #include "bgv_launch.h"
 
 static inline unsigned nblk(uint32_t n, unsigned t) { return (n + t - 1) / t; }
diff --git a/lodestar_amd/csrc/bgv_host_layout.h b/lodestar_amd/csrc/bgv_host_layout.h
--- a/lodestar_amd/csrc/bgv_host_layout.h
+++ b/lodestar_amd/csrc/bgv_host_layout.h
@@ -4,6 +4,7 @@
 #include <string.h>
 
 #include <algorithm>
+#include <atomic>
 #include <memory>
 #include <thread>
 #include <unordered_map>
@@ -118,6 +119,110 @@
   if (s.flags & BGV_SLOT_PK_BYTES) s.pk_off += pb;
   if (!(s.flags & BGV_SLOT_PAD)) s.group += gb;
   return s;
+}
+
+struct MergeBase {
+  uint32_t slot, group, idx, pkb;
+  size_t uniq, com_team, com_wave;
+};
+struct MergePlan {
+  std::vector<MergeBase> base;
+  uint32_t nslots = 0, ngroups = 0;
+  size_t nidx = 0, npkb = 0;
+  size_t nuniq = 0, ncom_team = 0, ncom_wave = 0;
+  bool any_uniform = false;
+  size_t nlist() const { return nuniq + ncom_team + ncom_wave; }
+};
+inline MergePlan merge_plan(const std::vector<const Layout*>& calls) {
+  MergePlan P;
+  P.base.reserve(calls.size());
+  for (const Layout* L : calls) {
+    P.base.push_back(MergeBase{P.nslots, P.ngroups, (uint32_t)P.nidx, (uint32_t)(P.npkb / 96), P.nuniq, P.ncom_team,
+                               P.ncom_wave});
+    P.nslots += (uint32_t)L->slots.size();
+    P.ngroups += (uint32_t)L->groups.size();
+    P.nidx += L->idx.size();
+    P.npkb += L->pkb.size();
+    P.nuniq += L->uniq.size();
+    P.ncom_team += L->com_team.size();
+    P.ncom_wave += L->com_wave.size();
+    for (char u : L->group_uniform) P.any_uniform = P.any_uniform || u;
+  }
+  return P;
+}
+
+static const size_t kMergeParMin = size_t(1) << 15;
+static const size_t kMergeChunk = size_t(1) << 14;
+
+inline uint32_t merge_layouts(const std::vector<const Layout*>& calls, const MergePlan& P, bool uniform,
+                              bgv_dslot* slots, bgv_dgroup* groups, uint32_t* idx, uint8_t* pkb,
+                              size_t par_min = kMergeParMin) {
+  struct Piece {
+    uint32_t call;
+    size_t lo, hi;
+  };
+  std::vector<Piece> pieces;
+  for (size_t k = 0; k < calls.size(); ++k) {
+    const size_t n = calls[k]->slots.size();
+    size_t lo = 0;
+    do {
+      const size_t hi = std::min(n, lo + kMergeChunk);
+      pieces.push_back(Piece{(uint32_t)k, lo, hi});
+      lo = hi;
+    } while (lo < n);
+  }
+  uint32_t* const uniq = idx + P.nidx;
+  uint32_t* const com_team = uniq + P.nuniq;
+  uint32_t* const com_wave = com_team + P.ncom_team;
+  std::vector<uint32_t> piece_max(pieces.size(), 0);
+  auto run_piece = [&](size_t q) {
+    const Piece& pc = pieces[q];
+    const Layout& L = *calls[pc.call];
+    const MergeBase& B = P.base[pc.call];
+    const bgv_dslot* src = L.slots.data();
+    bgv_dslot* dst = slots + B.slot;
+    uint32_t m = 0;
+    if (B.slot == 0 && B.idx == 0 && B.pkb == 0 && B.group == 0) {
+      if (pc.hi > pc.lo) memcpy(dst + pc.lo, src + pc.lo, sizeof(bgv_dslot) * (pc.hi - pc.lo));
+      for (size_t i = pc.lo; i < pc.hi; ++i)
+        if (!(src[i].flags & BGV_SLOT_PK_COMMITTEE)) m = std::max(m, src[i].n_pk);
+    } else {
+      for (size_t i = pc.lo; i < pc.hi; ++i) {
+        dst[i] = rebase_slot(src[i], B.slot, B.idx, B.pkb, B.group);
+        if (!(src[i].flags & BGV_SLOT_PK_COMMITTEE)) m = std::max(m, src[i].n_pk);
+      }
+    }
+    piece_max[q] = m;
+    if (pc.lo != 0) return;
+    for (size_t gi = 0; gi < L.groups.size(); ++gi) {
+      const bgv_dgroup& g = L.groups[gi];
+      groups[B.group + gi] = bgv_dgroup{g.first_slot + B.slot, g.n_slots, g.mask, 0,
+                                        uniform && L.group_uniform[gi] ? BGV_GROUP_UNIFORM : 0u};
+    }
+    if (!L.idx.empty()) memcpy(idx + B.idx, L.idx.data(), 4 * L.idx.size());
+    if (!L.pkb.empty()) memcpy(pkb + 96ull * B.pkb, L.pkb.data(), L.pkb.size());
+    for (size_t i = 0; i < L.uniq.size(); ++i) uniq[B.uniq + i] = L.uniq[i] + B.slot;
+    for (size_t i = 0; i < L.com_team.size(); ++i) com_team[B.com_team + i] = L.com_team[i] + B.slot;
+    for (size_t i = 0; i < L.com_wave.size(); ++i) com_wave[B.com_wave + i] = L.com_wave[i] + B.slot;
+  };
+  unsigned nt = 1;
+  if (P.nslots >= par_min && pieces.size() > 1)
+    nt = (unsigned)std::min<size_t>(pieces.size(), std::min(8u, std::max(1u, std::thread::hardware_concurrency())));
+  if (nt <= 1) {
+    for (size_t q = 0; q < pieces.size(); ++q) run_piece(q);
+  } else {
+    std::atomic<size_t> next{0};
+    auto worker = [&] {
+      for (size_t q; (q = next.fetch_add(1)) < pieces.size();) run_piece(q);
+    };
+    std::vector<std::thread> th;
+    for (unsigned t = 1; t < nt; ++t) th.emplace_back(worker);
+    worker();
+    for (auto& t : th) t.join();
+  }
+  uint32_t max_npk = 0;
+  for (uint32_t m : piece_max) max_npk = std::max(max_npk, m);
+  return max_npk;
 }
 
 struct RootIndex {
diff --git a/lodestar_amd/csrc/bgv_k_prep.hip b/lodestar_amd/csrc/bgv_k_prep.hip
--- a/lodestar_amd/csrc/bgv_k_prep.hip
+++ b/lodestar_amd/csrc/bgv_k_prep.hip
@@ -94,7 +94,7 @@
   uint32_t n = 0;
   bool comp = false;
   if (act) {
-    const bgv_dslot& d = slots[s];
+    const bgv_slot_head d = slot_head(slots, s);
     cm = dir + pk_idx[d.pk_off];
     words = pk_idx + d.pk_off + 1;
     members = pool + cm->off;
@@ -113,7 +113,7 @@
 __device__ __forceinline__ void pk_aggw_body(const bgv_dslot* __restrict__ slots, uint32_t s,
                                              const uint32_t* __restrict__ pk_idx, const g1_aff* __restrict__ cache,
                                              g1_jac* __restrict__ pk_agg) {
-  const bgv_dslot& d = slots[s];
+  const bgv_slot_head d = slot_head(slots, s);
   if ((d.flags & BGV_SLOT_PAD) || !(d.flags & BGV_SLOT_PK_CACHED) || d.n_pk <= BGV_PK_TEAM_MAX) return;
   const uint32_t l = threadIdx.x;
   g1_jac acc = jac_infinity<fp_t>();
@@ -132,13 +132,13 @@
                                               g1_jac* __restrict__ pk_agg) {
   const uint32_t s = blk * (64 / 16) + threadIdx.x / 16;
   const uint32_t l = threadIdx.x % 16;
-  const bgv_dslot* d = s < nslots ? &slots[s] : nullptr;
-  const bool act = d && !(d->flags & BGV_SLOT_PAD) && (d->flags & BGV_SLOT_PK_CACHED) &&
-                   d->n_pk >= BGV_PK_TREE_MIN && d->n_pk <= BGV_PK_TEAM_MAX;
+  const bgv_slot_head d = s < nslots ? slot_head(slots, s) : bgv_slot_head{BGV_SLOT_PAD, 0, 0, 0};
+  const bool act = !(d.flags & BGV_SLOT_PAD) && (d.flags & BGV_SLOT_PK_CACHED) && d.n_pk >= BGV_PK_TREE_MIN &&
+                   d.n_pk <= BGV_PK_TEAM_MAX;
   g1_jac acc = jac_infinity<fp_t>();
   if (act) {
-    const uint32_t* idx = pk_idx + d->pk_off;
-    const uint32_t n = d->n_pk;
+    const uint32_t* idx = pk_idx + d.pk_off;
+    const uint32_t n = d.n_pk;
     acc = jac_from_aff(cache[idx[l]]);
     uint32_t k = l + 16;
     g1_aff cur = cache[idx[k < n ? k : l]];
@@ -241,7 +241,7 @@
   else if (blockIdx.y == 2)
     task_sig_decode_t<bgv_pow_lane>(s, slots, split_sig(f, s), sig_status, true);
   else
-    task_pk(s, slots, pk_idx, cache, pk_bytes, rpk, pk_status, pk_agg);
+    task_pk(s, slots[s], pk_idx, cache, pk_bytes, rpk, pk_status, pk_agg);
 }
 
 __global__ void __launch_bounds__(64) k_prep_team(const bgv_dslot* __restrict__ slots, uint32_t nslots,
@@ -348,7 +348,7 @@
     if (pk_agg) pk_bits_one(slots, s, pk_idx, com_dir, com_pool, cache, pk_agg);
     if (threadIdx.x == 0) {
       g1_jac acc;
-      const bool go = task_pk_sum(s, slots, pk_idx, cache, pk_bytes, pk_status, pk_agg, &acc);
+      const bool go = task_pk_sum(s, slots[s], pk_idx, cache, pk_bytes, pk_status, pk_agg, &acc);
       flag = go ? 1 : 0;
       if (go) {
         S[TG1_BANK(1)] = acc.x;
@@ -460,6 +460,8 @@
 
 }
 
+bool bgv_prep_is_bulk(const bgv_dev_batch& b) { return b.nslots > 0 && !bgv_use_latency(b, b.nslots + b.ngroups); }
+
 hipError_t bgv_launch_prep(const bgv_dev_batch& b, const bgv_streams& s) {
   const uint32_t n = b.nslots;
   if (n == 0) return hipSuccess;
@@ -477,15 +479,19 @@
     BGV_MARK(1);
     return hipGetLastError();
   }
+  const bool in_place = b.in_slots != nullptr && bgv_prep_is_bulk(b);
+  const bgv_dslot* slots = in_place ? b.in_slots : b.slots;
+  const uint32_t* pk_idx = in_place ? b.in_idx : b.pk_idx;
+  const uint32_t* com = in_place ? b.in_idx + (b.com - b.pk_idx) : b.com;
   if (ncom)
-    hipLaunchKernelGGL(k_pk_agg_bits, dim3(nblk(b.ncom_team, 4) + b.ncom_wave), dim3(64), 0, s.main, b.slots, b.com,
-                       b.ncom_team, b.ncom_wave, b.pk_idx, b.com_dir, b.com_pool,
+    hipLaunchKernelGGL(k_pk_agg_bits, dim3(nblk(b.ncom_team, 4) + b.ncom_wave), dim3(64), 0, s.main, slots, com,
+                       b.ncom_team, b.ncom_wave, pk_idx, b.com_dir, b.com_pool,
                        reinterpret_cast<const g1_aff*>(b.cache_opaque), b.pk_agg);
   if (tree)
-    hipLaunchKernelGGL(k_pk_agg16, dim3(nblk(n, 4)), dim3(64), 0, s.main, b.slots, n, b.pk_idx,
+    hipLaunchKernelGGL(k_pk_agg16, dim3(nblk(n, 4)), dim3(64), 0, s.main, slots, n, pk_idx,
                        reinterpret_cast<const g1_aff*>(b.cache_opaque), b.pk_agg);
   if (b.max_npk > BGV_PK_TEAM_MAX)
-    hipLaunchKernelGGL(k_pk_agg, dim3(n), dim3(64), 0, s.main, b.slots, n, b.pk_idx,
+    hipLaunchKernelGGL(k_pk_agg, dim3(n), dim3(64), 0, s.main, slots, n, pk_idx,
                        reinterpret_cast<const g1_aff*>(b.cache_opaque), b.pk_agg);
   if (bgv_use_latency(b, n + b.ngroups)) {
     hipLaunchKernelGGL(k_prep_a, dim3(nblk(n, 64), 4), dim3(64), 0, s.main, b.slots, n, b.h, b.f, b.sig_status,
diff --git a/lodestar_amd/csrc/bgv_k_prep_bulk.hip b/lodestar_amd/csrc/bgv_k_prep_bulk.hip
--- a/lodestar_amd/csrc/bgv_k_prep_bulk.hip
+++ b/lodestar_amd/csrc/bgv_k_prep_bulk.hip
@@ -9,6 +9,16 @@
 #endif
 #define BGV_KATTR_BULK __launch_bounds__(64) __attribute__((amdgpu_waves_per_eu(BGV_WPE_BULK, BGV_WPE_BULK)))
 
+struct bgv_prep_keep {
+  bgv_dslot* slots;
+  bgv_dgroup* groups;
+  const bgv_dgroup* in_groups;
+  uint32_t ngroups;
+  uint32_t* uniq;
+};
+
+#define BGV_SLOT_Q ((uint32_t)(sizeof(bgv_dslot) / 16))
+
 extern "C" {
 
 __global__ void BGV_KATTR_BULK k_prep(const bgv_dslot* __restrict__ slots, uint32_t nslots, g2_jac* __restrict__ rsig,
@@ -16,22 +26,53 @@
                                       const uint32_t* __restrict__ pk_idx, const g1_aff* __restrict__ cache,
                                       const uint8_t* __restrict__ pk_bytes, g1_jac* __restrict__ rpk,
                                       int32_t* __restrict__ pk_status, const g1_jac* __restrict__ pk_agg,
-                                      const uint32_t* __restrict__ uniq, uint32_t nuniq, uint32_t task0) {
-  const uint32_t s = blockIdx.x * blockDim.x + threadIdx.x;
+                                      const uint32_t* __restrict__ uniq, uint32_t nuniq, uint32_t task0,
+                                      bgv_prep_keep keep) {
+  __shared__ uint4 stage[64 * BGV_SLOT_Q];
+  __shared__ uint32_t rec[64];
+  const uint32_t lane = threadIdx.x;
+  const uint32_t s = blockIdx.x * 64 + lane;
   const uint32_t task = blockIdx.y + task0;
-  if (task == 0) {
-    if (uniq) {
-      if (s < nuniq) task_hash(uniq[s], slots, h);
-    } else if (s < nslots) {
-      task_hash(s, slots, h);
+  const bool hashes = task == 0 && uniq != nullptr;
+  uint32_t r = s;
+  if (hashes) {
+    r = s < nuniq ? uniq[s] : nslots;
+    if (keep.uniq && s < nuniq) keep.uniq[s] = r;
+  }
+  const bool has = r < nslots;
+  rec[lane] = has ? r : ~0u;
+  __syncthreads();
+  BGV_UNROLL for (uint32_t i = 0; i < BGV_SLOT_Q; ++i) {
+    const uint32_t w = i * 64 + lane, src = rec[w / BGV_SLOT_Q];
+    if (src != ~0u) stage[w] = reinterpret_cast<const uint4*>(slots + src)[w % BGV_SLOT_Q];
+  }
+  __syncthreads();
+  if (task == 2) {
+    if (keep.slots) {
+      uint4* out = reinterpret_cast<uint4*>(keep.slots + blockIdx.x * 64);
+      BGV_UNROLL for (uint32_t i = 0; i < BGV_SLOT_Q; ++i) {
+        const uint32_t w = i * 64 + lane;
+        if (rec[w / BGV_SLOT_Q] != ~0u) out[w] = stage[w];
+      }
     }
-    return;
+    if (keep.groups && s < keep.ngroups) {
+      static_assert(sizeof(bgv_dgroup) == 24, "a group record is three 8-byte words");
+      const uint64_t* gi = reinterpret_cast<const uint64_t*>(keep.in_groups + s);
+      uint64_t* go = reinterpret_cast<uint64_t*>(keep.groups + s);
+      const uint64_t g0 = gi[0], g1 = gi[1], g2 = gi[2];
+      go[0] = g0;
+      go[1] = g1;
+      go[2] = g2;
+    }
   }
-  if (s >= nslots) return;
-  if (task == 1)
-    task_sig(s, slots, rsig, sig_status);
+  if (!has) return;
+  const bgv_dslot& d = *reinterpret_cast<const bgv_dslot*>(stage + lane * BGV_SLOT_Q);
+  if (task == 0)
+    task_hash(r, d, h);
+  else if (task == 1)
+    task_sig(s, d, rsig, sig_status);
   else
-    task_pk(s, slots, pk_idx, cache, pk_bytes, rpk, pk_status, pk_agg);
+    task_pk(s, d, pk_idx, cache, pk_bytes, rpk, pk_status, pk_agg);
 }
 
 }
@@ -41,10 +82,24 @@
     const char* e = getenv("BGV_PREP_SPLIT");
     return e && atoi(e) > 0;
   }();
+  const bool in_place = b.in_slots != nullptr;
+  const size_t uniq_off = b.uniq ? (size_t)(b.uniq - b.pk_idx) : 0;
+  const bgv_dslot* slots = in_place ? b.in_slots : b.slots;
+  const uint32_t* pk_idx = in_place ? b.in_idx : b.pk_idx;
+  const uint8_t* pk_bytes = in_place ? b.in_pkb : b.pk_bytes;
+  const uint32_t* uniq = in_place && b.uniq ? b.in_idx + uniq_off : b.uniq;
+  bgv_prep_keep keep{};
+  if (in_place) {
+    keep.slots = const_cast<bgv_dslot*>(b.slots);
+    keep.groups = const_cast<bgv_dgroup*>(b.groups);
+    keep.in_groups = b.in_groups;
+    keep.ngroups = b.ngroups;
+    keep.uniq = b.uniq ? const_cast<uint32_t*>(b.uniq) : nullptr;
+  }
   for (uint32_t t0 = 0; t0 < 3; t0 += split ? 1 : 3) {
-    hipLaunchKernelGGL(k_prep, dim3(nblk(b.nslots, 64), split ? 1 : 3), dim3(64), 0, s.main, b.slots, b.nslots, b.rsig,
-                       b.sig_status, b.h, b.pk_idx, reinterpret_cast<const g1_aff*>(b.cache_opaque), b.pk_bytes, b.rpk,
-                       b.pk_status, tree ? b.pk_agg : nullptr, b.uniq, b.nuniq, t0);
+    hipLaunchKernelGGL(k_prep, dim3(nblk(b.nslots, 64), split ? 1 : 3), dim3(64), 0, s.main, slots, b.nslots, b.rsig,
+                       b.sig_status, b.h, pk_idx, reinterpret_cast<const g1_aff*>(b.cache_opaque), pk_bytes, b.rpk,
+                       b.pk_status, tree ? b.pk_agg : nullptr, uniq, b.nuniq, t0, keep);
   }
   return hipGetLastError();
 }
diff --git a/lodestar_amd/csrc/bgv_k_tasks.h b/lodestar_amd/csrc/bgv_k_tasks.h
--- a/lodestar_amd/csrc/bgv_k_tasks.h
+++ b/lodestar_amd/csrc/bgv_k_tasks.h
@@ -1,9 +1,8 @@
 #pragma once
 #include "bgv_device.h"
 
-static __device__ __noinline__ void task_sig(uint32_t s, const bgv_dslot* __restrict__ slots, g2_jac* __restrict__ rsig,
+static __device__ __noinline__ void task_sig(uint32_t s, const bgv_dslot& d, g2_jac* __restrict__ rsig,
                                       int32_t* __restrict__ sig_status) {
-  const bgv_dslot& d = slots[s];
   int32_t st = BGV_ST_OK;
   if (d.flags & BGV_SLOT_PAD) {
     st = BGV_ST_INFINITY;
@@ -30,8 +29,7 @@
   sig_status[s] = st;
 }
 
-static __device__ __noinline__ void task_hash(uint32_t s, const bgv_dslot* __restrict__ slots, g2_jac* __restrict__ h) {
-  const bgv_dslot& d = slots[s];
+static __device__ __noinline__ void task_hash(uint32_t s, const bgv_dslot& d, g2_jac* __restrict__ h) {
   if (d.flags & BGV_SLOT_PAD) return;
   uint8_t msg[32];
   for (int i = 0; i < 32; ++i) msg[i] = d.msg[i];
@@ -51,9 +49,9 @@
     if (cached) {
       a = cache[pk_idx[d.pk_off + k]];
     } else {
-      uint8_t b[96];
-      const uint8_t* src = pk_bytes + 96ull * (d.pk_off + k);
-      for (int i = 0; i < 96; ++i) b[i] = src[i];
+      alignas(16) uint8_t b[96];
+      const uint4* src = reinterpret_cast<const uint4*>(pk_bytes + 96ull * (d.pk_off + k));
+      for (int i = 0; i < 6; ++i) reinterpret_cast<uint4*>(b)[i] = src[i];
       bool inf;
       const int rc = g1_deserialize(&a, &inf, b);
       if (rc != BGV_OK) {
@@ -67,11 +65,10 @@
   return acc;
 }
 
-static __device__ __noinline__ bool task_pk_sum(uint32_t s, const bgv_dslot* __restrict__ slots,
+static __device__ __noinline__ bool task_pk_sum(uint32_t s, const bgv_dslot& d,
                                                 const uint32_t* __restrict__ pk_idx, const g1_aff* __restrict__ cache,
                                                 const uint8_t* __restrict__ pk_bytes, int32_t* __restrict__ pk_status,
                                                 const g1_jac* __restrict__ pk_agg, g1_jac* acc) {
-  const bgv_dslot& d = slots[s];
   if (d.flags & BGV_SLOT_PAD) {
     pk_status[s] = BGV_ST_INFINITY;
     return false;
@@ -86,11 +83,10 @@
   return true;
 }
 
-static __device__ __noinline__ void task_pk(uint32_t s, const bgv_dslot* __restrict__ slots,
+static __device__ __noinline__ void task_pk(uint32_t s, const bgv_dslot& d,
                                      const uint32_t* __restrict__ pk_idx, const g1_aff* __restrict__ cache,
                                      const uint8_t* __restrict__ pk_bytes, g1_jac* __restrict__ rpk,
                                      int32_t* __restrict__ pk_status, const g1_jac* __restrict__ pk_agg) {
-  const bgv_dslot& d = slots[s];
   int32_t st = BGV_ST_OK;
   if (d.flags & BGV_SLOT_PAD) {
     pk_status[s] = BGV_ST_INFINITY;
diff --git a/lodestar_amd/csrc/bgv_launch.h b/lodestar_amd/csrc/bgv_launch.h
--- a/lodestar_amd/csrc/bgv_launch.h
+++ b/lodestar_amd/csrc/bgv_launch.h
@@ -37,6 +37,10 @@
   uint32_t ncom_team, ncom_wave;
   const bgv_dcommittee* com_dir;
   const uint32_t* com_pool;
+  const bgv_dslot* in_slots;
+  const uint32_t* in_idx;
+  const uint8_t* in_pkb;
+  const bgv_dgroup* in_groups;
   jac_t<fp2_t>* rsig;
   jac_t<fp2_t>* h;
   jac_t<fp_t>* rpk;
@@ -73,6 +77,7 @@
 hipError_t bgv_launch_sets(const bgv_dev_batch& b, const bgv_streams& s);
 bool bgv_sig_pairs(const bgv_dev_batch& b);
 hipError_t bgv_launch_prep(const bgv_dev_batch& b, const bgv_streams& s);
+bool bgv_prep_is_bulk(const bgv_dev_batch& b);
 hipError_t bgv_launch_prep_bulk(const bgv_dev_batch& b, const bgv_streams& s, bool tree);
 hipError_t bgv_launch_prep_wave(const bgv_dev_batch& b, hipStream_t st);
 hipError_t bgv_launch_miller(const bgv_dev_batch& b, const bgv_streams& s);
```

Result: no change. 2.716 million (-0.4%).
